# wzf2000/GAMER

Hardware: AMD Instinct MI355X
Metric: train-step sequences/sec, Qwen3Multi SMB decoder, his_len=100 (higher is better)
Workload: dtype f32 tensors/accumulators, products = 3 x fp16 pieces (split3)

## Files before the change

### gamer_amd/_lib.py

```python
from __future__ import annotations

import ctypes as C
import os
import re
from typing import Optional

import torch

_HERE = os.path.dirname(os.path.abspath(__file__))
LIB_PATH = os.path.join(_HERE, "lib", "libgamer_hip.so")
if os.environ.get("GAMER_LIB_PATH"):
    LIB_PATH = os.path.abspath(os.environ["GAMER_LIB_PATH"])
HEADER_PATH = os.path.join(os.path.dirname(_HERE), "include", "gamer_hip.h")

_lib: Optional[C.CDLL] = None

c_void_p, c_int, c_float, c_int64, c_uint64 = C.c_void_p, C.c_int, C.c_float, C.c_int64, C.c_uint64


class GemmDesc(C.Structure):
    _fields_ = [
        ("A", c_void_p), ("a_rs", c_int64), ("a_ks", c_int64),
        ("B", c_void_p), ("b_rs", c_int64), ("b_ks", c_int64),
        ("C", c_void_p), ("ldc", c_int64),
        ("M", c_int), ("N", c_int), ("K", c_int),
        ("alpha", c_float),
        ("accumulate", c_int),
        ("groups", c_int),
        ("group_mode", c_int),
        ("group_offsets", c_void_p),
        ("strideB", c_int64), ("strideC", c_int64),
        ("kchunk", c_int),
        ("resid", c_void_p),
        ("row_map", c_void_p),
        ("p_drop", c_float),
        ("seed", c_uint64),
        ("rowdot_other", c_void_p),
        ("rowdot_out", c_void_p),
        ("rowdot_S", c_int),
        ("qk_wq", c_void_p), ("qk_wk", c_void_p),
        ("qk_eps", c_float),
        ("qk_cos", c_void_p), ("qk_sin", c_void_p),
        ("qk_bias_q", c_void_p), ("qk_bias_k", c_void_p), ("qk_bias_v", c_void_p),
        ("qk_act_idx", c_void_p),
        ("qk_pos_ids", c_void_p),
        ("qk_q_rot", c_void_p), ("qk_k_rot", c_void_p),
        ("qk_S", c_int), ("qk_nq", c_int), ("qk_nkv", c_int),
        ("b_planes", c_void_p), ("b_plane_stride", c_int64),
        ("amax_a", c_void_p), ("amax_b", c_void_p),
        ("amax_c", c_void_p), ("amax_c_col0", c_int),
        ("wgrad_ws", c_void_p), ("wgrad_ws_floats", c_int64),
        ("sw_gu", c_void_p), ("sw_ld", c_int64),
        ("group_div", c_int), ("sw_tbl", c_void_p), ("b_planes_t", c_void_p),
        ("sw_hm", c_void_p), ("sw_row_group", c_void_p),
        ("norm_x", c_void_p), ("norm_w", c_void_p), ("norm_eps", c_float),
        ("norm_dst_rows", c_void_p), ("norm_src_rows", c_void_p),
        ("bias_idx", c_void_p), ("bias_q", c_void_p), ("bias_k", c_void_p), ("bias_v", c_void_p),
        ("bias_rows", c_int), ("bias_nq", c_int), ("bias_nkv", c_int),
    ]


class GemmBf16Desc(C.Structure):
    _fields_ = [
        ("A", c_void_p), ("lda", c_int64),
        ("B", c_void_p), ("ldb", c_int64),
        ("C", c_void_p), ("ldc", c_int64),
        ("M", c_int), ("N", c_int), ("K", c_int),
        ("accumulate", c_int),
        ("groups", c_int),
        ("group_mode", c_int),
        ("group_offsets", c_void_p),
        ("strideB", c_int64), ("strideC", c_int64),
        ("kchunk", c_int),
        ("resid", c_void_p),
        ("row_map", c_void_p),
        ("p_drop", c_float),
        ("seed", c_uint64),
        ("rowdot_other", c_void_p),
        ("rowdot_out", c_void_p),
        ("rowdot_S", c_int),
        ("qk_wq", c_void_p), ("qk_wk", c_void_p), ("qk_eps", c_float),
        ("qk_cos", c_void_p), ("qk_sin", c_void_p),
        ("qk_bias_q", c_void_p), ("qk_bias_k", c_void_p), ("qk_bias_v", c_void_p),
        ("qk_act_idx", c_void_p), ("qk_pos_ids", c_void_p),
        ("qk_q_rot", c_void_p), ("qk_k_rot", c_void_p),
        ("qk_S", c_int), ("qk_nq", c_int), ("qk_nkv", c_int),
        ("sw_gu", c_void_p), ("sw_ld", c_int64),
        ("wgrad_ws", c_void_p), ("wgrad_ws_floats", c_int64),
    ]


P, I, F, L, U = c_void_p, c_int, c_float, c_int64, c_uint64

_SIGNATURES = {
    "gamer_router_fwd": [P, P, P, P, I, I, I, I, I, I, P, P, P, P, P, P, P, P, P, P, P, P],
    "gamer_expert_lists": [P, I, I, I, P, P, P, P, P],
    "gamer_causal_prep": [P, I, I, P, P, P, P, P, P],
    "gamer_session_prep": [P, P, P, I, I, I, I, P, P, P, P, P, P, P],
    "gamer_moe_router_prep": [P, P, P, I, P, I, I, I, I, I, I, I, P, P, P, P, P, P, P, P, P],
    "gamer_moe_action_router_prep": [P, P, P, I, P, I, I, I, I, I, I, I, I, I, P, P, P, P, P, P, P, P, P, P],
    "gamer_session_moe_prep": [P, P, P, P, P, I, P, I, I, I, I, I, I, I, I, P, P, P, P, P, P, P, P, P, P],
    "gamer_embedding_fwd": [P, P, I, I, I, P, P],
    "gamer_embedding_bwd": [P, P, I, I, I, I, P, P],
    "gamer_embedding_bwd_ordered": [P, P, I, I, I, I, P, P, L, P],
    "gamer_embedding_bwd_ordered_ws_bytes": [I, I, I],
    "gamer_rmsnorm_fwd": [P, P, I, I, F, P, P, I, P],
    "gamer_rmsnorm_bwd": [P, P, P, I, P, I, I, F, I, P, P, I, P, P, F, U, P],
    "gamer_colsum_reduce": [P, I, I, I, P, P],
    "gamer_colsum_reduce_batched": [P, L, I, I, I, P, I, P],
    "gamer_rowtable_fwd": [P, P, P, I, I, P, I, I, P],
    "gamer_rowtable_bwd": [P, I, I, P, P, I, I, I, P, P, L, P],
    "gamer_gemm_f32": [C.POINTER(GemmDesc), P],
    "gamer_gemm_f32_split": [C.POINTER(GemmDesc), c_int, P],
    "gamer_split3_guard": [I],
    "gamer_gemm_bf16": [C.POINTER(GemmBf16Desc), P],
    "gamer_cast_params_bf16": [P, P, P, P, I, I, P],
    "gamer_attn_fwd_bf16": [P, I, P, I, P, I, P, P, I, I, I, I, F, F, U, P, P, P, P, P, P, P],
    "gamer_attn_bwd_bf16": [P, I, P, I, P, I, P, P, P, P, P, I, I, I, I, F, F, U, P, P, I, P, I, P, I, P, I, P, P, P, P],
    "gamer_session_spans": [P, P, P, P, P, I, I, I, I, P, P, P, P, P, P, P, P, P],
    "gamer_qknorm_rope_fwd": [P, I, I, I, I, P, P, F, P, P, P, P, P, P, P, P, P, P],
    "gamer_qknorm_rope_bwd": [P, P, P, I, I, I, I, P, P, F, P, P, P, P, P, I, P, P, P, P, P, P, P, P, L, P],
    "gamer_attn_row_order": [P, I, I, P, P, P, P],
    "gamer_attn_fwd": [P, I, P, I, P, I, P, P, P, P, I, I, I, I, F, F, U, P, P, P, P, P, I, P, P],
    "gamer_attn_bwd": [P, I, P, I, P, I, P, P, P, P, P, P, P, I, I, I, I, F, F, U, P, P, I, P, I, P, I, P, P, P, P, P, I, P],
    "gamer_split3_planes": [P, P, L, L, P],
    "gamer_absmax_f32": [P, I, L, I, I, L, P, P],
    "gamer_absmax_multi_f32": [P, P, I, P, P],
    "gamer_split2h_planes_multi": [P, P, I, P, P, P],
    "gamer_amax_sink": [P, P],
    "gamer_amax_sink3": [P, P, P],
    "gamer_attn_split_amax": [P, P, P, P],
    "gamer_attn_fwd_split": [P, I, P, I, P, I, P, P, P, I, I, I, I, F, F, U, P, P, P, P, P, I, P, P],
    "gamer_attn_bwd_split": [P, I, P, I, P, I, P, P, P, P, P, P, P, I, I, I, I, F, F, U, P, P, I, P, I, P, I, P, P, P, I, P, P, P],
    "gamer_residual_dropout_fwd": [P, P, P, I, I, F, U, P, P],
    "gamer_residual_dropout_bwd": [P, P, I, I, F, U, P, P],
    "gamer_swiglu_fwd": [P, P, L, F, U, P, P],
    "gamer_swiglu_bwd": [P, P, P, L, F, U, P],
    "gamer_swiglu_fwd_ld": [P, L, I, I, F, U, P, P],
    "gamer_swiglu_bwd_ld": [P, L, I, I, P, F, U, P],
    "gamer_swiglu_fwd_ld_tbl": [P, L, I, I, F, U, P, P, P, P],
    "gamer_pba_router": [P, I, I, I, I, I, I, I, P, I, I, I, I, I, P, P, P, P, P],
# ... 158 lines not shown
```

### gamer_amd/csrc/common.h

```cpp
#pragma once
#include <hip/hip_runtime.h>
#include <stdint.h>
#include <stdio.h>
#include <stdarg.h>
#include <stdlib.h>
#include <atomic>
#include <type_traits>

#include "../../include/gamer_hip.h"

namespace gamer {

void set_error(const char* fmt, ...);

#define GAMER_CHECK_ARG(cond, ...)                       \
    do {                                                 \
        if (!(cond)) {                                   \
            gamer::set_error(__VA_ARGS__);               \
            return -1;                                   \
        }                                                \
    } while (0)

#define GAMER_CHECK_LAUNCH(name)                                                        \
    do {                                                                                \
// ... 222 lines not shown
    __device__ __forceinline__ float mult(uint64_t idx) const {
        if (!on) return 1.f;
        uint32_t h = mix32((uint32_t)idx ^ k0);
        h = mix32(h + (uint32_t)(idx >> 32) * 0x9e3779b1U + k1);
        return h >= thr ? scale : 0.f;
    }
};

struct AttnDropout {
    uint32_t k0, k1, thr;
    float scale;
    __device__ __forceinline__ AttnDropout(float p, uint64_t seed) {
        k0 = mix32((uint32_t)seed ^ 0x9e3779b9U) ^ mix32((uint32_t)(seed >> 32) + 0x7f4a7c15U);
        k1 = mix32(k0 + 0x632be5abU);
        const float t = p * 4294967296.f;
        thr = t >= 4294967040.f ? 0xffffffffU : (uint32_t)t;
        scale = p > 0.f ? 1.f / (1.f - p) : 1.f;
    }
    __device__ __forceinline__ uint32_t row_word(uint32_t row) const {
        return (mix32(row * 0x9e3779b1U + k0) & 0xffffffU) | 0x800001U;
    }
    __device__ __forceinline__ uint32_t key_word(uint32_t j) const { return mix32(j * 0x85ebca6bU + k1) & 0xffffffU; }
    __device__ __forceinline__ bool keep(uint32_t a, uint32_t b) const { return __umul24(a, b) >= thr; }
};

__device__ __forceinline__ float xor32_max(float v) {
    const auto sw = __builtin_amdgcn_permlane32_swap(__float_as_uint(v), __float_as_uint(v), false, false);
    return fmaxf(__uint_as_float(sw[0]), __uint_as_float(sw[1]));
}
__device__ __forceinline__ float xor32_sum(float v) {
    const auto sw = __builtin_amdgcn_permlane32_swap(__float_as_uint(v), __float_as_uint(v), false, false);
    return __uint_as_float(sw[0]) + __uint_as_float(sw[1]);
}

__device__ __forceinline__ int wave_sum_i32(int v) {
#pragma unroll
    for (int o = 32; o > 0; o >>= 1) v += __shfl_xor(v, o, 64);
    return v;
}
__device__ __forceinline__ int wave_max_i32(int v) {
#pragma unroll
    for (int o = 32; o > 0; o >>= 1) v = max(v, __shfl_xor(v, o, 64));
    return v;
}
__device__ __forceinline__ int wave_min_i32(int v) {
#pragma unroll
    for (int o = 32; o > 0; o >>= 1) v = min(v, __shfl_xor(v, o, 64));
    return v;
}

#define GAMER_DPP_ROW_REDUCE(OP, v)                                                                   \
    v = OP(v, __builtin_amdgcn_update_dpp(v, v, 0xB1, 0xf, 0xf, false));      \
    v = OP(v, __builtin_amdgcn_update_dpp(v, v, 0x4E, 0xf, 0xf, false));      \
    v = OP(v, __builtin_amdgcn_update_dpp(v, v, 0x141, 0xf, 0xf, false));         \
    v = OP(v, __builtin_amdgcn_update_dpp(v, v, 0x140, 0xf, 0xf, false));
__device__ __forceinline__ int wave_min_i32_dpp(int v) {
    GAMER_DPP_ROW_REDUCE(min, v)
    return min(min(__builtin_amdgcn_readlane(v, 0), __builtin_amdgcn_readlane(v, 16)),
               min(__builtin_amdgcn_readlane(v, 32), __builtin_amdgcn_readlane(v, 48)));
}
__device__ __forceinline__ int wave_max_i32_dpp(int v) {
    GAMER_DPP_ROW_REDUCE(max, v)
    return max(max(__builtin_amdgcn_readlane(v, 0), __builtin_amdgcn_readlane(v, 16)),
               max(__builtin_amdgcn_readlane(v, 32), __builtin_amdgcn_readlane(v, 48)));
}

__device__ __forceinline__ float row16_sum_dpp(float v) {
#define GAMER_DPP_F(ctrl) __int_as_float(__builtin_amdgcn_update_dpp(__float_as_int(v), __float_as_int(v), ctrl, 0xf, 0xf, false))
    v += GAMER_DPP_F(0xB1);
    v += GAMER_DPP_F(0x4E);
    v += GAMER_DPP_F(0x141);
    v += GAMER_DPP_F(0x140);
#undef GAMER_DPP_F
    return v;
}

__device__ __forceinline__ float sigmoid_f(float x) { return __builtin_amdgcn_rcpf(1.f + __expf(-x)); }
__device__ __forceinline__ float silu_f(float x) { return x * sigmoid_f(x); }
__device__ __forceinline__ float dsilu_f(float x) {
    const float s = sigmoid_f(x);
    return s * (1.f + x * (1.f - s));
}

struct SwigluRule {
    static constexpr int NIN = 2;
    static __device__ __forceinline__ float fwd(float a, float b, float m) { return m * (silu_f(a) * b); }
    static __device__ __forceinline__ float bwd_a(float a, float b, float d) { return d * b * dsilu_f(a); }
    static __device__ __forceinline__ float bwd_b(float a, float, float d) { return d * silu_f(a); }
};
struct SiluRule {
    static constexpr int NIN = 1;
    static __device__ __forceinline__ float fwd(float a, float, float m) { return m * silu_f(a); }
    static __device__ __forceinline__ float bwd_a(float a, float, float d) { return d * dsilu_f(a); }
};
struct ReluRule {
    static constexpr int NIN = 1;
    static __device__ __forceinline__ float fwd(float a, float, float m) { return a > 0.f ? m * a : 0.f; }
    static __device__ __forceinline__ float bwd_a(float a, float, float d) { return a > 0.f ? d : 0.f; }
};
template <class R>
__device__ __forceinline__ float4 act_fwd4(const float4 a, const float4 b, const float (&m)[4]) {
    return make_float4(R::fwd(a.x, b.x, m[0]), R::fwd(a.y, b.y, m[1]), R::fwd(a.z, b.z, m[2]), R::fwd(a.w, b.w, m[3]));
}
template <class R>
__device__ __forceinline__ void act_bwd4(const float4 a, const float4 b, const float4 dout, const float (&m)[4], float4& da, float4& db) {
    const float d0 = m[0] * dout.x, d1 = m[1] * dout.y, d2 = m[2] * dout.z, d3 = m[3] * dout.w;
    da = make_float4(R::bwd_a(a.x, b.x, d0), R::bwd_a(a.y, b.y, d1), R::bwd_a(a.z, b.z, d2), R::bwd_a(a.w, b.w, d3));
    if constexpr (R::NIN == 2) db = make_float4(R::bwd_b(a.x, b.x, d0), R::bwd_b(a.y, b.y, d1), R::bwd_b(a.z, b.z, d2), R::bwd_b(a.w, b.w, d3));
}

bool gemm_as_eligible(const gamer_gemm_desc* d, bool a_kc, bool b_kc, const uint16_t* b_planes);
int launch_gemm_as(const gamer_gemm_desc* d, const uint16_t* b_planes, bool b_kc, hipStream_t st);
int launch_gemm_bias_rows(const gamer_gemm_desc* d, hipStream_t st);
bool gemm_os_eligible(const gamer_gemm_desc* d, bool a_kc, bool b_kc, const uint16_t* b_planes);
int launch_gemm_os(const gamer_gemm_desc* d, const uint16_t* b_planes, int guard, hipStream_t st, bool fwd_t = false);
bool gemm_os_fwd_eligible(const gamer_gemm_desc* d, bool a_kc, bool b_kc);
bool gemm_wg_eligible(const gamer_gemm_desc* d, bool a_kc, bool b_kc);
int launch_gemm_wg(const gamer_gemm_desc* d, hipStream_t st);

int launch_wgrad_reduce(const float* ws, float* C, int64_t ldc, int M, int N, int groups, const int32_t* group_offsets, int K,
                        int kchunk, int64_t strideC, hipStream_t st);

}
```

### gamer_amd/csrc/elementwise.hip

```cpp
#include "common.h"

namespace gamer {

__global__ void __launch_bounds__(EW_THREADS)
embedding_fwd_kernel(const int64_t* __restrict__ ids, const float4* __restrict__ W, int V, int T, int H4,
                     float4* __restrict__ x) {
    const int lane = threadIdx.x & 63;
    const int wave = (blockIdx.x * EW_THREADS + threadIdx.x) >> 6;
    const int nwaves = (gridDim.x * EW_THREADS) >> 6;
    for (int t = wave; t < T; t += nwaves) {
        const int64_t id = ids[t];
        const bool ok = id >= 0 && id < V;
        for (int c = lane; c < H4; c += 64) {
            float4 v = ok ? W[id * H4 + c] : make_float4(0.f, 0.f, 0.f, 0.f);
            x[(int64_t)t * H4 + c] = v;
        }
    }
}

constexpr int EMB_CACHE = 8;
constexpr int EMB_CHUNK = 1024;
__global__ void __launch_bounds__(EW_THREADS)
embedding_bwd_kernel(const int64_t* __restrict__ ids, const float* __restrict__ dx, int V, int T, int H,
                     int pad_id, float* __restrict__ dW, const int chunk) {
// ... 436 lines not shown
    for (int a = 0; a < TBL_MAXROWS; ++a) acc[a] = make_float4(0.f, 0.f, 0.f, 0.f);
    if (rl < rows_per_block) {
        for (int64_t t = (int64_t)blockIdx.x * rows_per_block + rl; t < T; t += (int64_t)gridDim.x * rows_per_block) {
            const int64_t r = dy_rows ? dy_rows[t] : t;
            const float4 g = ld4(dy + r * lddy + col0 + 4 * c);
            const int a_t = idx[t];
#pragma unroll
            for (int a = 0; a < TBL_MAXROWS; ++a) {
                const float m = (a_t == a) ? 1.f : 0.f;
                acc[a].x += m * g.x; acc[a].y += m * g.y; acc[a].z += m * g.z; acc[a].w += m * g.w;
            }
        }
#pragma unroll
        for (int a = 0; a < TBL_MAXROWS; ++a) {
            if (a < nrows) {
                if (DET) {
                    *reinterpret_cast<float4*>(&lds_tbl[(rl * nrows + a) * E + c * 4]) = acc[a];
                } else {
                    atomicAdd(&lds_tbl[a * E + c * 4 + 0], acc[a].x);
                    atomicAdd(&lds_tbl[a * E + c * 4 + 1], acc[a].y);
                    atomicAdd(&lds_tbl[a * E + c * 4 + 2], acc[a].z);
                    atomicAdd(&lds_tbl[a * E + c * 4 + 3], acc[a].w);
                }
            }
        }
    }
    __syncthreads();
    if (DET) {
        for (int i = threadIdx.x; i < nrows * E; i += EW_THREADS) {
            float t = 0.f;
            for (int g = 0; g < rows_per_block; ++g) t += lds_tbl[g * nrows * E + i];
            partial[(int64_t)blockIdx.x * nrows * E + i] = t;
        }
    } else {
        for (int i = threadIdx.x; i < nrows * E; i += EW_THREADS) atomicAdd(&dtable[i], lds_tbl[i]);
    }
}

__global__ void __launch_bounds__(EW_THREADS)
residual_dropout_fwd_kernel(const float4* x_in, const float4* __restrict__ delta,
                            const int32_t* __restrict__ src_rows, int T, int H4, float p, uint64_t seed,
                            float4* x_out) {
    const DropoutRng rng(p, seed);
    const int64_t total = (int64_t)T * H4;
    for (int64_t i = (int64_t)blockIdx.x * EW_THREADS + threadIdx.x; i < total; i += (int64_t)gridDim.x * EW_THREADS) {
        const int t = (int)(i / H4);
        const int c = (int)(i % H4);
        const int64_t r = src_rows ? src_rows[t] : t;
        const float4 d = delta[r * H4 + c];
        float4 v = x_in[i];
        float m[4];
        rng.mult4((uint32_t)i, m);
        v.x += m[0] * d.x; v.y += m[1] * d.y; v.z += m[2] * d.z; v.w += m[3] * d.w;
        x_out[i] = v;
    }
}

__global__ void __launch_bounds__(EW_THREADS)
residual_dropout_bwd_kernel(const float4* __restrict__ dx, const int32_t* __restrict__ src_rows, int T, int H4,
                            float p, uint64_t seed, float4* __restrict__ ddelta) {
    const DropoutRng rng(p, seed);
    const int64_t total = (int64_t)T * H4;
    for (int64_t i = (int64_t)blockIdx.x * EW_THREADS + threadIdx.x; i < total; i += (int64_t)gridDim.x * EW_THREADS) {
        const int t = (int)(i / H4);
        const int c = (int)(i % H4);
        const int64_t r = src_rows ? src_rows[t] : t;
        const float4 g = dx[i];
        float m[4];
        rng.mult4((uint32_t)i, m);
        float4 o;
        o.x = m[0] * g.x; o.y = m[1] * g.y; o.z = m[2] * g.z; o.w = m[3] * g.w;
        ddelta[r * H4 + c] = o;
    }
}

template <typename TA, typename TO>
__global__ void __launch_bounds__(EW_THREADS)
silu_gate_fwd_kernel(const TA* __restrict__ a, const TA* __restrict__ gate, int64_t n4,
                     TO* __restrict__ out, const float4* __restrict__ resid, float p, uint64_t seed) {
    const DropoutRng rng(resid ? p : 0.f, seed);
    for (int64_t i = (int64_t)blockIdx.x * EW_THREADS + threadIdx.x; i < n4; i += (int64_t)gridDim.x * EW_THREADS) {
        const float4 x = ld4(a + 4 * i), g = ld4(gate + 4 * i);
        float4 o;
        o.x = x.x * silu_f(g.x); o.y = x.y * silu_f(g.y); o.z = x.z * silu_f(g.z); o.w = x.w * silu_f(g.w);
        if (resid) {
            const float4 r = resid[i];
            float m[4];
            rng.mult4((uint32_t)i, m);
            o.x = r.x + m[0] * o.x; o.y = r.y + m[1] * o.y; o.z = r.z + m[2] * o.z; o.w = r.w + m[3] * o.w;
        }
        st4(out + 4 * i, o);
    }
}

template <typename TA>
__global__ void __launch_bounds__(EW_THREADS)
silu_gate_bwd_kernel(const TA* __restrict__ a, const TA* __restrict__ gate, const float4* __restrict__ dout,
                     int64_t n4, TA* __restrict__ da, TA* __restrict__ dgate, float p, uint64_t seed,
                     uint32_t* __restrict__ amax_a, uint32_t* __restrict__ amax_gate) {
    __shared__ uint32_t amax_lds[2][4];
    uint32_t ama = 0, amg = 0;
    const DropoutRng rng(p, seed);
    for (int64_t i = (int64_t)blockIdx.x * EW_THREADS + threadIdx.x; i < n4; i += (int64_t)gridDim.x * EW_THREADS) {
        const float4 x = ld4(a + 4 * i), g = ld4(gate + 4 * i);
        float4 d = dout[i];
        float m[4];
        rng.mult4((uint32_t)i, m);
        d.x *= m[0]; d.y *= m[1]; d.z *= m[2]; d.w *= m[3];
        float4 oa, og;
        oa.x = d.x * silu_f(g.x); og.x = d.x * x.x * dsilu_f(g.x);
        oa.y = d.y * silu_f(g.y); og.y = d.y * x.y * dsilu_f(g.y);
        oa.z = d.z * silu_f(g.z); og.z = d.z * x.z * dsilu_f(g.z);
        oa.w = d.w * silu_f(g.w); og.w = d.w * x.w * dsilu_f(g.w);
        st4(da + 4 * i, oa);
        st4(dgate + 4 * i, og);
        ama = amax_f4(ama, oa);
        amg = amax_f4(amg, og);
    }
    amax_block_commit(ama, amax_a, amax_lds[0]);
    amax_block_commit(amg, amax_gate, amax_lds[1]);
}

constexpr int CE_MAXC = 20;
template <typename T> constexpr int CE_EPL = 16 / (int)sizeof(T);
template <typename T> constexpr int CE_MAXQ = sizeof(T) == 2 ? 3 : 5;
__device__ __forceinline__ void ce_load16(const float* p, float (&x)[4]) {
    const float4 v = *reinterpret_cast<const float4*>(p);
    x[0] = v.x; x[1] = v.y; x[2] = v.z; x[3] = v.w;
}
__device__ __forceinline__ void ce_store16(float* p, const float (&x)[4]) { *reinterpret_cast<float4*>(p) = make_float4(x[0], x[1], x[2], x[3]); }
__device__ __forceinline__ void ce_load16(const bf16_t* p, float (&x)[8]) {
    const bf16x8 v = *reinterpret_cast<const bf16x8*>(p);
#pragma unroll
    for (int e = 0; e < 8; ++e) x[e] = (float)v[e];
}
__device__ __forceinline__ void ce_store16(bf16_t* p, const float (&x)[8]) {
    bf16x8 v;
#pragma unroll
    for (int e = 0; e < 8; ++e) v[e] = (bf16_t)x[e];
    *reinterpret_cast<bf16x8*>(p) = v;
}
template <typename TL>
__global__ void __launch_bounds__(EW_THREADS)
ce_fwd_kernel(TL* __restrict__ logits, int ldl, const int64_t* __restrict__ labels, int T, int S, int V,
              float inv_temp, int ignore_index, float* __restrict__ lse_out, float* __restrict__ row_loss, int vec4) {
    const int lane = threadIdx.x & 63;
    const int wave = (blockIdx.x * EW_THREADS + threadIdx.x) >> 6;
    const int nwaves = (gridDim.x * EW_THREADS) >> 6;
    for (int t = wave; t < T; t += nwaves) {
        TL* row = logits + (int64_t)t * ldl;
        const int s = t % S;
        const int64_t tgt = (s + 1 < S) ? labels[t + 1] : (int64_t)ignore_index;
        const bool valid = tgt != ignore_index && tgt >= 0 && tgt < V;
        float mx = -INFINITY;
        float zt = 0.f;
        if (vec4 && V <= 64 * CE_EPL<TL> * CE_MAXQ<TL>) {
            constexpr int EPL = CE_EPL<TL>;
            float z[CE_MAXQ<TL>][EPL];
            const int c_last = ((V - 1) / EPL) * EPL;
#pragma unroll
            for (int i = 0; i < CE_MAXQ<TL>; ++i) {
                const int c = EPL * (lane + 64 * i);
                float x[EPL];
                ce_load16(row + min(c, c_last), x);
#pragma unroll
                for (int e = 0; e < EPL; ++e) z[i][e] = c + e < V ? round_as<TL>(x[e] * inv_temp) : -INFINITY;
            }
#pragma unroll
            for (int i = 0; i < CE_MAXQ<TL>; ++i) {
                const int c = EPL * (lane + 64 * i);
                if (inv_temp == 1.f) {
                } else if (c + EPL <= V) {
// ... 551 lines not shown
```

### gamer_amd/csrc/gemm.hip

```cpp
#include "common.h"
#include <stdlib.h>

namespace gamer {

constexpr int BM = 128, BN = 128, BK = 32;
constexpr int GEMM_THREADS = 256;
constexpr int KC_LD = BK + 4;
constexpr int TILE_FLOATS = BM * KC_LD;
constexpr int GEMM_LDS_BYTES = 4 * TILE_FLOATS * (int)sizeof(float);

typedef float f32x16 __attribute__((ext_vector_type(16)));

constexpr int SP_KC_ROW = 80;
constexpr int SP_KC_IMG = BM * SP_KC_ROW;
constexpr int SP_RC_IMG = BK * 256;
constexpr int SP_OPERAND = 3 * SP_KC_IMG;
constexpr int SP_LDS_BYTES = 2 * SP_OPERAND;

#ifndef SP_ABLATE
#define SP_ABLATE 0
#endif
__device__ __forceinline__ uint32_t pack_hi16(uint32_t w0, uint32_t w1) { return __builtin_amdgcn_perm(w1, w0, 0x07060302u); }
__device__ __forceinline__ void split3(float x, uint32_t (&w)[3]) {
    if (SP_ABLATE & 1) { w[0] = w[1] = w[2] = __float_as_uint(x); return; }
    w[0] = __float_as_uint(x);
    const float r1 = x - __uint_as_float(w[0] & 0xffff0000u);
    w[1] = __float_as_uint(r1);
    const float r2 = r1 - __uint_as_float(w[1] & 0xffff0000u);
    w[2] = __float_as_uint(r2);
}
__device__ __forceinline__ void split3_quad(const float4& v, uint2 (&img)[3]) {
    uint32_t a[3], b[3], c[3], d[3];
    split3(v.x, a); split3(v.y, b); split3(v.z, c); split3(v.w, d);
#pragma unroll
    for (int s = 0; s < 3; ++s) img[s] = make_uint2(pack_hi16(a[s], b[s]), pack_hi16(c[s], d[s]));
}
__device__ __forceinline__ int sp_rc_off(int k, int row) { return k * 256 + ((((row >> 3) ^ ((k & 3) << 2))) << 4) + ((row & 7) << 1); }
__device__ __forceinline__ void store_kc_split(unsigned char* __restrict__ lds, int tid, const float4 (&r)[4]) {
#pragma unroll
    for (int j = 0; j < 4; ++j) {
        const int f = tid + GEMM_THREADS * j;
        uint2 img[3];
        split3_quad(r[j], img);
        unsigned char* dst = lds + (f >> 3) * SP_KC_ROW + ((f & 7) << 3);
        if (SP_ABLATE & 2) { asm volatile("" :: "v"(img[0].x), "v"(img[1].x), "v"(img[2].x), "v"(img[0].y), "v"(img[1].y), "v"(img[2].y)); continue; }
#pragma unroll
        for (int s = 0; s < 3; ++s) *reinterpret_cast<uint2*>(dst + s * SP_KC_IMG) = img[s];
    }
}
__device__ __forceinline__ void store_rc_split(unsigned char* __restrict__ lds, int tid, const float4 (&r)[4]) {
#pragma unroll
    for (int j = 0; j < 4; ++j) {
        const int f = tid + GEMM_THREADS * j;
        uint2 img[3];
        split3_quad(r[j], img);
        unsigned char* dst = lds + sp_rc_off(f >> 5, (f & 31) << 2);
        if (SP_ABLATE & 2) { asm volatile("" :: "v"(img[0].x), "v"(img[1].x), "v"(img[2].x), "v"(img[0].y), "v"(img[1].y), "v"(img[2].y)); continue; }
#pragma unroll
        for (int s = 0; s < 3; ++s) *reinterpret_cast<uint2*>(dst + s * SP_RC_IMG) = img[s];
    }
}
__device__ __forceinline__ void split2h_quad(const float4& v, float s, uint2 (&img)[2]) {
    uint32_t a0, a1, b0, b1;
    cut2h_quad(v.x, v.y, v.z, v.w, s, a0, a1, b0, b1);
    img[0] = make_uint2(a0, b0);
    img[1] = make_uint2(a1, b1);
}
__device__ __forceinline__ void store_kc_h2(unsigned char* __restrict__ lds, int tid, const float4 (&r)[4], float s) {
#pragma unroll
    for (int j = 0; j < 4; ++j) {
        const int f = tid + GEMM_THREADS * j;
        uint2 img[2];
        split2h_quad(r[j], s, img);
        unsigned char* dst = lds + (f >> 3) * SP_KC_ROW + ((f & 7) << 3);
#pragma unroll
        for (int q = 0; q < 2; ++q) *reinterpret_cast<uint2*>(dst + q * SP_KC_IMG) = img[q];
    }
}
__device__ __forceinline__ void store_rc_h2(unsigned char* __restrict__ lds, int tid, const float4 (&r)[4], float s) {
#pragma unroll
    for (int j = 0; j < 4; ++j) {
        const int f = tid + GEMM_THREADS * j;
        uint2 img[2];
        split2h_quad(r[j], s, img);
// ... 45 lines not shown
__device__ __forceinline__ bf16x8 read_frag_half(const unsigned char* __restrict__ img, int rbase, int lane) {
    const int r32 = lane & 31, h = lane >> 5;
    if (KC) {
        return *reinterpret_cast<const bf16x8*>(img + (rbase + r32) * SPH_KC_ROW + (h << 4));
    } else {
        const int q = (lane >> 2) & 3, pp = lane & 3, gsel = (lane >> 4) & 1;
        const int row = rbase + 16 * gsel + 4 * pp;
        bf16x8 out;
#pragma unroll
        for (int c = 0; c < 2; ++c) {
            const int k = 8 * h + 4 * c + q;
            const bf16x4 v = __builtin_amdgcn_ds_read_tr16_b64_v4bf16(
                (bf16x4 __attribute__((address_space(3)))*)(img + sp_rc_off(k, row)));
            out[4 * c + 0] = v[0]; out[4 * c + 1] = v[1]; out[4 * c + 2] = v[2]; out[4 * c + 3] = v[3];
        }
        return out;
    }
}

template <bool KC>
__device__ __forceinline__ bf16x8 read_frag_split(const unsigned char* __restrict__ img, int rbase, int sub, int lane) {
    const int r32 = lane & 31, h = lane >> 5;
    if (KC) {
        return *reinterpret_cast<const bf16x8*>(img + (rbase + r32) * SP_KC_ROW + ((2 * sub + h) << 4));
    } else {
        const int q = (lane >> 2) & 3, pp = lane & 3, gsel = (lane >> 4) & 1;
        const int row = rbase + 16 * gsel + 4 * pp;
        bf16x8 out;
#pragma unroll
        for (int c = 0; c < 2; ++c) {
            const int k = 16 * sub + 8 * h + 4 * c + q;
            const bf16x4 v = __builtin_amdgcn_ds_read_tr16_b64_v4bf16(
                (bf16x4 __attribute__((address_space(3)))*)(img + sp_rc_off(k, row)));
            out[4 * c + 0] = v[0]; out[4 * c + 1] = v[1]; out[4 * c + 2] = v[2]; out[4 * c + 3] = v[3];
        }
        return out;
    }
}

__device__ unsigned long long* g_gemm_stamp = nullptr;
__device__ __forceinline__ unsigned long long stamp_now() {
    unsigned long long t;
    asm volatile("s_memtime %0\n\ts_waitcnt lgkmcnt(0)" : "=s"(t) :: "memory");
    return t;
}

struct GemmParams {
    const float* A; int64_t a_rs, a_ks;
    const float* B; int64_t b_rs, b_ks;
    float* C; int64_t ldc;
    int M, N, K;
    float alpha;
    int accumulate;
    int groups;
    const int32_t* group_offsets;
    int64_t strideB, strideC;
    int kchunk;
    int m_tiles, n_tiles;
    const float* resid;
    const int32_t* row_map;
    float p_drop;
    uint64_t seed;
    const float* rowdot_other;
    float* rowdot_out;
    int rowdot_S;
    const float* qk_wq; const float* qk_wk;
    float qk_eps;
    const float* qk_cos; const float* qk_sin;
    const float* qk_bias_q; const float* qk_bias_k; const float* qk_bias_v;
    const int32_t* qk_act_idx;
    const int32_t* qk_pos_ids;
    float* qk_q_rot; float* qk_k_rot;
    int qk_S, qk_nq, qk_nkv;
    const uint32_t* amax_a; const uint32_t* amax_b;
    const uint16_t* b_planes;
    int64_t b_plane_stride;
    int guard;
    uint32_t* amax_c;
    int amax_c_col0;
    float* wgrad_ws;
    float* sw_gu; int64_t sw_ld;
    int group_div;
    const float* sw_tbl;
};

constexpr float SPLIT3_GUARD_RATIO = 1.f / 65536.f;
#ifndef GAMER_GEMM_CAMAX_BUILD
#define GAMER_GEMM_CAMAX_BUILD 1
#endif
#ifndef GAMER_SPLIT3_GUARD_BUILD
#define GAMER_SPLIT3_GUARD_BUILD 1
#endif
static int g_split3_guard = 1;

__device__ __forceinline__ int xcd_remap(int id, int n) {
    const int q = n >> 3, r = n & 7;
    const int xcd = id & 7, idx = id >> 3;
    const int base = xcd < r ? xcd * (q + 1) : r * (q + 1) + (xcd - r) * q;
    return base + idx;
}

template <bool INTERIOR>
__device__ __forceinline__ void load_kc(const float* __restrict__ p, int64_t rs, int row0, int row_end, int k0,
                                        int k_end, int tid, float4 (&r)[4]) {
#pragma unroll
    for (int j = 0; j < 4; ++j) {
        const int f = tid + GEMM_THREADS * j;
        const int row = row0 + (f >> 3);
        const int k = k0 + ((f & 7) << 2);
        if (INTERIOR) {
            r[j] = *reinterpret_cast<const float4*>(p + (int64_t)row * rs + k);
            continue;
        }
        float4 v = make_float4(0.f, 0.f, 0.f, 0.f);
        if (row < row_end && k < k_end) {
            v = *reinterpret_cast<const float4*>(p + (int64_t)row * rs + k);
            if (k + 3 >= k_end) {
                if (k + 1 >= k_end) v.y = 0.f;
                if (k + 2 >= k_end) v.z = 0.f;
                v.w = 0.f;
            }
        }
        r[j] = v;
    }
}
template <bool INTERIOR>
__device__ __forceinline__ void load_rc(const float* __restrict__ p, int64_t ks, int row0, int row_end, int k0,
                                        int k_end, int tid, float4 (&r)[4]) {
#pragma unroll
    for (int j = 0; j < 4; ++j) {
        const int f = tid + GEMM_THREADS * j;
        const int k = k0 + (f >> 5);
        const int row = row0 + ((f & 31) << 2);
        if (INTERIOR) {
            r[j] = *reinterpret_cast<const float4*>(p + (int64_t)k * ks + row);
            continue;
        }
        float4 v = make_float4(0.f, 0.f, 0.f, 0.f);
        if (k < k_end && row < row_end) {
            v = *reinterpret_cast<const float4*>(p + (int64_t)k * ks + row);
            if (row + 3 >= row_end) {
                if (row + 1 >= row_end) v.y = 0.f;
                if (row + 2 >= row_end) v.z = 0.f;
                v.w = 0.f;
            }
        }
        r[j] = v;
    }
}
__device__ __forceinline__ void store_kc(float* __restrict__ lds, int tid, const float4 (&r)[4]) {
#pragma unroll
    for (int j = 0; j < 4; ++j) {
        const int f = tid + GEMM_THREADS * j;
        *reinterpret_cast<float4*>(lds + (f >> 3) * KC_LD + ((f & 7) << 2)) = r[j];
    }
}
__device__ __forceinline__ void store_rc(float* __restrict__ lds, int tid, const float4 (&r)[4]) {
#pragma unroll
    for (int j = 0; j < 4; ++j) {
        const int f = tid + GEMM_THREADS * j;
        *reinterpret_cast<float4*>(lds + (f >> 5) * BM + ((f & 31) << 2)) = r[j];
    }
}

template <bool KC>
__device__ __forceinline__ void read_frag(const float* __restrict__ lds, int row, int kk, int h, float (&f)[4]) {
// ... 510 lines not shown
        }
    }
    if (PP && grp == 0) __syncthreads();
    const unsigned long long t_loop_end = STAMP ? stamp_now() : 0;

    bool redo = false;
    if (GUARD && p.guard) {
        const float thr = __uint_as_float(amax_a_bits) * SPLIT3_GUARD_RATIO;
        bool bad = false;
#pragma unroll
        for (int j = 0; j < 4; ++j) {
            float m = rmax[j];
            m = fmaxf(m, __shfl_xor(m, 1, 64)); m = fmaxf(m, __shfl_xor(m, 2, 64)); m = fmaxf(m, __shfl_xor(m, 4, 64));
            bad |= (m > 0.f) & !(m >= thr);
        }
        int* flags = reinterpret_cast<int*>(smem + 4 * 64 * 68);
        const bool wave_bad = __any(bad ? 1 : 0) != 0;
        if (lane == 0) flags[wid] = wave_bad ? 1 : 0;
        __syncthreads();
        redo = (flags[0] | flags[1] | flags[2] | flags[3]) != 0;
        if (redo) {
#pragma unroll
            for (int i = 0; i < 2; ++i)
#pragma unroll
                for (int j = 0; j < 2; ++j)
#pragma unroll
                    for (int r = 0; r < 16; ++r) acc[i][j][r] = 0.f;
            if (wave_live) {
                const int ar0 = row0 + wm * 64 + r32, bc0 = col0 + wn * 64 + r32;
#pragma unroll 1
                for (int k = kbeg; k < kend; k += 2) {
                    const int kk = k + h;
                    const bool kin = kk < kend;
                    float av[2], bv[2];
#pragma unroll
                    for (int i = 0; i < 2; ++i) {
                        const int row = ar0 + i * 32;
                        av[i] = (kin && row < row_end) ? p.A[(int64_t)row * p.a_rs + kk] : 0.f;
                    }
#pragma unroll
                    for (int j = 0; j < 2; ++j) {
                        const int col = bc0 + j * 32;
                        bv[j] = (kin && col < col_end) ? (B_KC ? Bsrc[(int64_t)col * p.b_rs + kk] : Bsrc[(int64_t)kk * p.b_ks + col]) : 0.f;
                    }
#pragma unroll
                    for (int i = 0; i < 2; ++i)
#pragma unroll
                        for (int j = 0; j < 2; ++j)
                            acc[i][j] = __builtin_amdgcn_mfma_f32_32x32x2f32(av[i], bv[j], acc[i][j], 0, 0, 0);
                }
            }
        }
    }

    const bool interior = a_in && b_in;
    const float alpha_eff = (SPLIT == 3 && !redo) ? p.alpha * unscale : p.alpha;
    if (MODE == 0 && (NBUF == 2 || SPLIT) && interior && (p.ldc & 3) == 0) {
        float* patch = smem + wid * (64 * 68);
        float4 oth[EPI == 2 ? 16 : 1];
        if (EPI == 2) {
            const float* ob = p.rowdot_other + (int64_t)(row0 + wm * 64 + (lane >> 4)) * p.ldc + col0 + wn * 64 + ((lane & 15) << 2);
#pragma unroll
            for (int it = 0; it < 16; ++it) oth[it] = *reinterpret_cast<const float4*>(ob + (int64_t)it * 4 * p.ldc);
        }
        if (SPLIT != 3 && p.alpha == 1.f) {
#pragma unroll
            for (int i = 0; i < 2; ++i)
#pragma unroll
                for (int j = 0; j < 2; ++j)
#pragma unroll
                    for (int r = 0; r < 16; ++r)
                        patch[(i * 32 + (r & 3) + 8 * (r >> 2) + 4 * h) * 68 + j * 32 + r32] = acc[i][j][r];
        } else {
#pragma unroll
            for (int i = 0; i < 2; ++i)
#pragma unroll
                for (int j = 0; j < 2; ++j)
#pragma unroll
                    for (int r = 0; r < 16; ++r)
                        patch[(i * 32 + (r & 3) + 8 * (r >> 2) + 4 * h) * 68 + j * 32 + r32] = alpha_eff * acc[i][j][r];
        }
        __builtin_amdgcn_s_waitcnt(0xc07f);
        const int c4 = (lane & 15) << 2;
        const DropoutRng rng((EPI == 1 || EPI == 4) ? p.p_drop : 0.f, p.seed);
        const int row_first = row0 + wm * 64 + (lane >> 4);
        const int col = col0 + wn * 64 + c4;
        float* dst0 = Cp + (int64_t)row_first * p.ldc + col;
        const int64_t step = 4 * p.ldc;
        const int qk_pos0 = EPI == 3 ? row_first % max(p.qk_S, 1) : 0;
        const bool amax_on = GAMER_GEMM_CAMAX_BUILD && p.amax_c != nullptr && !ACCUM && col0 + wn * 64 >= p.amax_c_col0;
        float cmax = 0.f;
        int pre_rc[EPI == 1 ? 16 : 1];
        float4 pre_x[EPI == 1 ? 16 : (EPI == 4 ? 8 : 1)], pre_b[EPI == 4 ? 8 : 1];
        if (EPI == 1) {
            if (p.row_map) {
#pragma unroll
                for (int it = 0; it < 16; ++it) pre_rc[it] = p.row_map[row_first + 4 * it];
            } else {
#pragma unroll
                for (int it = 0; it < 16; ++it) pre_rc[it] = row_first + 4 * it;
            }
#pragma unroll
            for (int it = 0; it < 16; ++it) pre_x[it] = *reinterpret_cast<const float4*>(p.resid + (int64_t)pre_rc[it] * p.ldc + col);
        }
        float4 tb_g = make_float4(0.f, 0.f, 0.f, 0.f), tb_u = tb_g;
        if (EPI == 4 && p.sw_tbl) {
            const float* tb = p.sw_tbl + (int64_t)tile_group * 2 * p.N + col;
            tb_g = *reinterpret_cast<const float4*>(tb);
            tb_u = *reinterpret_cast<const float4*>(tb + p.N);
        }
        auto pre_sw = [&](int it0) {
#pragma unroll
            for (int it = 0; it < 8; ++it) {
                const float* ga = p.sw_gu + (int64_t)(row_first + 4 * (it0 + it)) * p.sw_ld + col;
                pre_x[EPI == 4 ? it : 0] = *reinterpret_cast<const float4*>(ga);
                pre_b[EPI == 4 ? it : 0] = *reinterpret_cast<const float4*>(ga + p.N);
            }
        };
        if (EPI == 4) pre_sw(0);
#pragma unroll
        for (int it = 0; it < 16; ++it) {
            if (EPI == 4 && it == 8) pre_sw(8);
            const int lr = (lane >> 4) + 4 * it;
            const float4 v = *reinterpret_cast<const float4*>(patch + lr * 68 + c4);
            if (EPI == 3) {
                const int row = row_first + 4 * it;
                const int hd = (col0 + wn * 64) >> 6;
                const int g = lane & 15;
                float4 x = v;
                const bool cross = p.qk_bias_q != nullptr;
                const int a = cross ? p.qk_act_idx[row] : 0;
                if (hd < p.qk_nq + p.qk_nkv) {
                    const bool isq = hd < p.qk_nq;
                    if (cross) {
                        const float4 b4 = isq ? reinterpret_cast<const float4*>(p.qk_bias_q + (int64_t)a * p.qk_nq * 64 + hd * 64)[g]
                                              : reinterpret_cast<const float4*>(p.qk_bias_k + (int64_t)a * p.qk_nkv * 64 + (hd - p.qk_nq) * 64)[g];
                        x.x += b4.x; x.y += b4.y; x.z += b4.z; x.w += b4.w;
                    }
                    *reinterpret_cast<float4*>(dst0 + it * step) = x;
                    float ss = x.x * x.x + x.y * x.y + x.z * x.z + x.w * x.w;
                    ss = row16_sum_dpp(ss);
                    const float rstd = rsqrtf(ss * (1.f / 64.f) + p.qk_eps);
                    const float4 w4 = reinterpret_cast<const float4*>(isq ? p.qk_wq : p.qk_wk)[g];
                    float4 y;
                    y.x = w4.x * (x.x * rstd); y.y = w4.y * (x.y * rstd); y.z = w4.z * (x.z * rstd); y.w = w4.w * (x.w * rstd);
                    float4 pr;
                    pr.x = __shfl_xor(y.x, 8, 64); pr.y = __shfl_xor(y.y, 8, 64); pr.z = __shfl_xor(y.z, 8, 64); pr.w = __shfl_xor(y.w, 8, 64);
                    int pos = qk_pos0 + 4 * it;
                    if (p.qk_S >= 64) pos = pos >= p.qk_S ? pos - p.qk_S : pos;
                    else pos %= p.qk_S;
                    if (p.qk_pos_ids) pos = p.qk_pos_ids[row];
                    const float4 cc = reinterpret_cast<const float4*>(p.qk_cos + pos * 64)[g];
                    const float4 sn = reinterpret_cast<const float4*>(p.qk_sin + pos * 64)[g];
                    const float sgn = g < 8 ? -1.f : 1.f;
                    float4 o;
                    o.x = y.x * cc.x + sgn * pr.x * sn.x; o.y = y.y * cc.y + sgn * pr.y * sn.y;
                    o.z = y.z * cc.z + sgn * pr.z * sn.z; o.w = y.w * cc.w + sgn * pr.w * sn.w;
                    float* rot = isq ? p.qk_q_rot + (int64_t)row * p.qk_nq * 64 + hd * 64
                                     : p.qk_k_rot + (int64_t)row * p.qk_nkv * 64 + (hd - p.qk_nq) * 64;
                    *reinterpret_cast<float4*>(rot + 4 * g) = o;
                } else {
                    if (cross) {
                        const float4 b4 = reinterpret_cast<const float4*>(p.qk_bias_v + (int64_t)a * p.qk_nkv * 64 +
                                                                          (hd - p.qk_nq - p.qk_nkv) * 64)[g];
                        x.x += b4.x; x.y += b4.y; x.z += b4.z; x.w += b4.w;
                    }
                    *reinterpret_cast<float4*>(dst0 + it * step) = x;
                }
            } else if (EPI == 4) {
                const int row = row_first + 4 * it;
                float* ga = p.sw_gu + (int64_t)row * p.sw_ld + col;
                float* ua = ga + p.N;
                float4 a = pre_x[EPI == 4 ? (it & 7) : 0], b = pre_b[EPI == 4 ? (it & 7) : 0];
                a.x += tb_g.x; a.y += tb_g.y; a.z += tb_g.z; a.w += tb_g.w;
                b.x += tb_u.x; b.y += tb_u.y; b.z += tb_u.z; b.w += tb_u.w;
                float m[4];
                rng.mult4((uint32_t)(((int64_t)row * p.N + col) >> 2), m);
                const float d0 = m[0] * v.x, d1 = m[1] * v.y, d2 = m[2] * v.z, d3 = m[3] * v.w;
                float4 dg, du;
                dg.x = SwigluRule::bwd_a(a.x, b.x, d0); du.x = SwigluRule::bwd_b(a.x, b.x, d0);
                dg.y = SwigluRule::bwd_a(a.y, b.y, d1); du.y = SwigluRule::bwd_b(a.y, b.y, d1);
                dg.z = SwigluRule::bwd_a(a.z, b.z, d2); du.z = SwigluRule::bwd_b(a.z, b.z, d2);
                dg.w = SwigluRule::bwd_a(a.w, b.w, d3); du.w = SwigluRule::bwd_b(a.w, b.w, d3);
                *reinterpret_cast<float4*>(ga) = dg;
                *reinterpret_cast<float4*>(ua) = du;
                if (amax_on) {
                    asm("v_max3_f32 %0, %0, |%1|, |%2|\n\tv_max3_f32 %0, %0, |%3|, |%4|" : "+v"(cmax) : "v"(dg.x), "v"(dg.y), "v"(dg.z), "v"(dg.w));
                    asm("v_max3_f32 %0, %0, |%1|, |%2|\n\tv_max3_f32 %0, %0, |%3|, |%4|" : "+v"(cmax) : "v"(du.x), "v"(du.y), "v"(du.z), "v"(du.w));
                }
            } else if (EPI == 1) {
                const int64_t e = (int64_t)pre_rc[EPI == 1 ? it : 0] * p.ldc + col;
                float* dst = Cp + e;
                const float4 x = pre_x[EPI == 1 ? it : 0];
                float m[4];
                rng.mult4((uint32_t)(e >> 2), m);
                float4 o;
                o.x = x.x + m[0] * v.x; o.y = x.y + m[1] * v.y; o.z = x.z + m[2] * v.z; o.w = x.w + m[3] * v.w;
                *reinterpret_cast<float4*>(dst) = o;
            } else {
                float* dst = dst0 + it * step;
                if (EPI != 1 && EPI != 3 && amax_on)
                    asm("v_max3_f32 %0, %0, |%1|, |%2|\n\tv_max3_f32 %0, %0, |%3|, |%4|" : "+v"(cmax) : "v"(v.x), "v"(v.y), "v"(v.z), "v"(v.w));
                if (EPI == 2) {
                    const float4 o4 = oth[EPI == 2 ? it : 0];
                    float d = v.x * o4.x + v.y * o4.y + v.z * o4.z + v.w * o4.w;
                    d = row16_sum_dpp(d);
                    if ((lane & 15) == 0) {
                        const int row = row_first + 4 * it;
                        const int heads = p.N >> 6, head = (col0 + wn * 64) >> 6;
                        p.rowdot_out[((int64_t)(row / p.rowdot_S) * heads + head) * p.rowdot_S + row % p.rowdot_S] = d;
                    }
                }
                if (ACCUM) {
                    float4 o = *reinterpret_cast<const float4*>(dst);
                    o.x += v.x; o.y += v.y; o.z += v.z; o.w += v.w;
                    *reinterpret_cast<float4*>(dst) = o;
                } else {
                    *reinterpret_cast<float4*>(dst) = v;
                }
            }
        }
        if (EPI != 1 && EPI != 3 && amax_on) {
            uint32_t mw = __float_as_uint(cmax);
#pragma unroll
            for (int o2 = 32; o2 > 0; o2 >>= 1) mw = max(mw, (uint32_t)__shfl_xor((int)mw, o2, 64));
            if (lane == 0 && mw) amax_publish(mw, p.amax_c, (uint32_t)(vblock * 4 + wid));
        }
    } else if (MODE == 1 && p.wgrad_ws != nullptr) {
        float* blk = p.wgrad_ws + ws_block * (int64_t)(BM * BN);
#pragma unroll
        for (int i = 0; i < 2; ++i)
#pragma unroll
            for (int j = 0; j < 2; ++j) {
                const int lc = wn * 64 + j * 32 + r32;
                const int lr0 = wm * 64 + i * 32 + 4 * h;
#pragma unroll
                for (int r = 0; r < 16; ++r) blk[(lr0 + (r & 3) + 8 * (r >> 2)) * BN + lc] = alpha_eff * acc[i][j][r];
            }
    } else {
        float emax = 0.f;
        if (EPI == 4 && p.sw_tbl != nullptr) {
            const float* tb0 = p.sw_tbl + (int64_t)tile_group * 2 * p.N;
            const int nr = min(BM, row_end - row0), nc = min(BN, p.N - col0);
            for (int i = threadIdx.x; i < nr * nc; i += GEMM_THREADS) {
                const int rr = row0 + i / nc, cc = col0 + i % nc;
                float* ga = p.sw_gu + (int64_t)rr * p.sw_ld + cc;
                ga[0] += tb0[cc];
                ga[p.N] += tb0[p.N + cc];
            }
            __syncthreads();
        }
        auto emit = [&](int row, int col, float v) {
            if (EPI == 4) {
                float* ga = p.sw_gu + (int64_t)row * p.sw_ld + col;
                float a = ga[0], b = ga[p.N];
                const int64_t e = (int64_t)row * p.N + col;
                const DropoutRng rng(p.p_drop, p.seed);
                float m[4];
                rng.mult4((uint32_t)(e >> 2), m);
                const float d = m[e & 3] * v;
                const float dg = SwigluRule::bwd_a(a, b, d), du = SwigluRule::bwd_b(a, b, d);
                ga[0] = dg; ga[p.N] = du;
                if (GAMER_GEMM_CAMAX_BUILD && p.amax_c != nullptr) emax = fmaxf(emax, fmaxf(fabsf(dg), fabsf(du)));
                return;
            }
            if (GAMER_GEMM_CAMAX_BUILD && EPI != 1 && MODE == 0 && !ACCUM && p.amax_c != nullptr && col >= p.amax_c_col0) emax = fmaxf(emax, fabsf(v));
            if (EPI == 1) {
                const int64_t rc = p.row_map ? p.row_map[row] : row;
                const int64_t e = rc * p.ldc + col;
                const DropoutRng rng(p.p_drop, p.seed);
                float m[4];
                rng.mult4((uint32_t)(e >> 2), m);
                Cp[e] = p.resid[e] + m[e & 3] * v;
            } else {
                float* dst = Cp + (int64_t)row * p.ldc + col;
                if (MODE == 1) atomicAdd(dst, v);
                else if (ACCUM) *dst += v;
                else *dst = v;
            }
        };
#pragma unroll
        for (int i = 0; i < 2; ++i) {
#pragma unroll
            for (int j = 0; j < 2; ++j) {
                const int col = col0 + wn * 64 + j * 32 + r32;
                const int rbase = row0 + wm * 64 + i * 32 + 4 * h;
                if (interior) {
#pragma unroll
                    for (int r = 0; r < 16; ++r) emit(rbase + (r & 3) + 8 * (r >> 2), col, alpha_eff * acc[i][j][r]);
                } else {
#pragma unroll
                    for (int r = 0; r < 16; ++r) {
                        const int rr = (r & 3) + 8 * (r >> 2);
                        if (rbase + rr < row_end && col < col_end) emit(rbase + rr, col, alpha_eff * acc[i][j][r]);
                    }
                }
            }
        }
        if (GAMER_GEMM_CAMAX_BUILD && MODE == 0 && !ACCUM && p.amax_c != nullptr) {
            uint32_t mw = __float_as_uint(emax);
#pragma unroll
            for (int o2 = 32; o2 > 0; o2 >>= 1) mw = max(mw, (uint32_t)__shfl_xor((int)mw, o2, 64));
            if (lane == 0 && mw) amax_publish(mw, p.amax_c, (uint32_t)(vblock * 4 + wid));
        }
    }
    if (STAMP) {
        unsigned long long* st = g_gemm_stamp;
        if (st && threadIdx.x == 0) {
            const unsigned long long t_end = stamp_now();
            unsigned long long* rec = st + 8ull * vblock;
            rec[0] = t_ph[0]; rec[1] = t_ph[1]; rec[2] = t_ph[2]; rec[3] = t_ph[3];
            rec[4] = t_loop_end - t_begin;
            rec[5] = t_end - t_loop_end;
            rec[6] = t_begin;
            rec[7] = t_end;
        }
    }
}

template <bool A_KC, bool B_KC, int MODE, bool ACCUM, bool STAMP, int NBUF, int EPI, int SPLIT = 0, bool PP = false>
__global__ void __launch_bounds__(PP ? 2 * GEMM_THREADS : GEMM_THREADS, (NBUF == 1 && SPLIT == 0) ? 3 : 2)
gemm_f32_kernel(const GemmParams p, const int vgrid) {
    extern __shared__ __attribute__((aligned(16))) float smem_all[];
    for (int v = blockIdx.x; v < vgrid; v += gridDim.x) {
        gemm_f32_tile<A_KC, B_KC, MODE, ACCUM, STAMP, NBUF, EPI, SPLIT, PP>(p, smem_all, v, vgrid);
        if (v + (int)gridDim.x < vgrid) __syncthreads();
    }
}

template <bool A_KC, bool B_KC, int MODE, bool ACCUM, bool STAMP, int NBUF, int EPI = 0, int SPLIT = 0, bool PP = false>
static int launch_gemm_t(const GemmParams& p, int blocks, hipStream_t st, int lds) {
    static int persist = -1;
    if (persist < 0) { const char* e = getenv("GAMER_GEMM_PERSIST"); persist = e ? atoi(e) : 0; }
    const int grid = (persist > 0 && SPLIT != 0 && !PP && !STAMP && blocks > persist) ? persist : blocks;
    return launch<gemm_f32_kernel<A_KC, B_KC, MODE, ACCUM, STAMP, NBUF, EPI, SPLIT, PP>>("gamer_gemm_f32", dim3(grid), dim3(PP ? 2 * GEMM_THREADS : GEMM_THREADS),
                                                                                        lds, st, p, blocks);
}

template <bool A_KC, bool B_KC, int MODE, int SPLIT>
static int launch_gemm_split(const GemmParams& p, int blocks, hipStream_t st) {
    constexpr int h2_stage = 2 * ((A_KC ? SP_KC_IMG : SP_RC_IMG) + (B_KC ? SP_KC_IMG : SP_RC_IMG));
    const int lds = (SPLIT == 3 && SP_WIDE3 && A_KC && B_KC && 2 * h2_stage > GEMM_LDS_BYTES) ? 2 * h2_stage : GEMM_LDS_BYTES;
    static_assert(SP_LDS_BYTES <= GEMM_LDS_BYTES, "split images must fit the fp32 kernel's LDS allocation");
    const bool acc = MODE == 0 && p.accumulate;
    static int stamp = -1, pp = 0;
    if (stamp < 0) {
        const char* e = getenv("GAMER_GEMM_STAMP");
        stamp = (e && e[0] == '1') ? 1 : 0;
        const char* e2 = getenv("GAMER_GEMM_PP");
        pp = (SP_PINGPONG && e2 && e2[0] == '1') ? 1 : 0;
    }
    (void)pp;
#if SP_PINGPONG
    if ((SPLIT == 6 || SPLIT == 3) && pp && !(MODE == 0 && p.b_planes)) {
        int pblocks;
        if (MODE == 0) pblocks = (blocks + 1) / 2;
        else {
            const int tiles_mn = p.m_tiles * p.n_tiles;
            pblocks = blocks / tiles_mn * ((tiles_mn + 1) / 2);
        }
        const int plds = 2 * GEMM_LDS_BYTES;
        if (stamp) return launch_gemm_t<A_KC, B_KC, MODE, false, true, 2, 0, SPLIT, true>(p, pblocks, st, plds);
        if (MODE == 0 && p.resid) return launch_gemm_t<A_KC, B_KC, MODE, false, false, 2, 1, SPLIT, true>(p, pblocks, st, plds);
        if (MODE == 0 && p.rowdot_out) return launch_gemm_t<A_KC, B_KC, MODE, false, false, 2, 2, SPLIT, true>(p, pblocks, st, plds);
        if (MODE == 0 && A_KC && B_KC && p.qk_q_rot) return launch_gemm_t<A_KC, B_KC, MODE, false, false, 2, 3, SPLIT, true>(p, pblocks, st, plds);
        if (acc) return launch_gemm_t<A_KC, B_KC, MODE, true, false, 2, 0, SPLIT, true>(p, pblocks, st, plds);
        return launch_gemm_t<A_KC, B_KC, MODE, false, false, 2, 0, SPLIT, true>(p, pblocks, st, plds);
    }
#endif
    if (stamp && SPLIT == 6) return launch_gemm_t<A_KC, B_KC, MODE, false, true, 2, 0, SPLIT>(p, blocks, st, lds);
    if constexpr (SPLIT == 3 && MODE == 0 && A_KC) {
        if (p.sw_gu) return launch_gemm_t<A_KC, B_KC, MODE, false, false, 2, 4, SPLIT>(p, blocks, st, lds);
    }
    if (MODE == 0 && p.resid) return launch_gemm_t<A_KC, B_KC, MODE, false, false, 2, 1, SPLIT>(p, blocks, st, lds);
    if (MODE == 0 && p.rowdot_out) return launch_gemm_t<A_KC, B_KC, MODE, false, false, 2, 2, SPLIT>(p, blocks, st, lds);
    if (MODE == 0 && A_KC && B_KC && p.qk_q_rot) return launch_gemm_t<A_KC, B_KC, MODE, false, false, 2, 3, SPLIT>(p, blocks, st, lds);
    if (acc) return launch_gemm_t<A_KC, B_KC, MODE, true, false, 2, 0, SPLIT>(p, blocks, st, lds);
    return launch_gemm_t<A_KC, B_KC, MODE, false, false, 2, 0, SPLIT>(p, blocks, st, lds);
}

template <bool A_KC, bool B_KC, int MODE>
static int launch_gemm(const GemmParams& p, int blocks, hipStream_t st, int split = 0) {
    if (split == 6) return launch_gemm_split<A_KC, B_KC, MODE, 6>(p, blocks, st);
    if (split == 9) return launch_gemm_split<A_KC, B_KC, MODE, 9>(p, blocks, st);
    if (split == 3) return launch_gemm_split<A_KC, B_KC, MODE, 3>(p, blocks, st);
    static int stamp = -1, solo = 0, nbuf = 2;
    if (stamp < 0) {
        const char* e = getenv("GAMER_GEMM_STAMP");
        stamp = (e && e[0] == '1') ? 1 : 0;
        const char* s2 = getenv("GAMER_GEMM_SOLO");
        solo = (s2 && s2[0] == '1') ? 1 : 0;
        const char* s3 = getenv("GAMER_GEMM_NBUF");
        nbuf = (s3 && s3[0] == '1') ? 1 : 2;
    }
    const int lds = solo ? 150 * 1024 : GEMM_LDS_BYTES;
    const bool acc = MODE == 0 && p.accumulate;
    if (stamp) return launch_gemm_t<A_KC, B_KC, MODE, false, true, 2>(p, blocks, st, lds);
    if (MODE == 0 && p.resid) return launch_gemm_t<A_KC, B_KC, MODE, false, false, 2, 1>(p, blocks, st, lds);
    if (MODE == 0 && p.rowdot_out) return launch_gemm_t<A_KC, B_KC, MODE, false, false, 2, 2>(p, blocks, st, lds);
    if (MODE == 0 && A_KC && B_KC && p.qk_q_rot) return launch_gemm_t<A_KC, B_KC, MODE, false, false, 2, 3>(p, blocks, st, lds);
    if (nbuf == 1) {
        const int lds1 = 2 * TILE_FLOATS * (int)sizeof(float);
        if (acc) return launch_gemm_t<A_KC, B_KC, MODE, true, false, 1>(p, blocks, st, lds1);
        return launch_gemm_t<A_KC, B_KC, MODE, false, false, 1>(p, blocks, st, lds1);
    }
    if (acc) return launch_gemm_t<A_KC, B_KC, MODE, true, false, 2>(p, blocks, st, lds);
    return launch_gemm_t<A_KC, B_KC, MODE, false, false, 2>(p, blocks, st, lds);
}

__global__ void __launch_bounds__(256)
wgrad_reduce_kernel(const float* __restrict__ ws, float* __restrict__ C, int64_t ldc, int M, int N, int m_tiles, int n_tiles,
                    int groups, const int32_t* __restrict__ group_offsets, int K, int kchunk, int64_t strideC) {
    const int tiles_mn = m_tiles * n_tiles;
    int id = blockIdx.x;
    const int strip = id & 15; id >>= 4;
    const int tile = id % tiles_mn, g = id / tiles_mn;
    int c_beg = 0, c_n;
    if (group_offsets) {
        int prev = group_offsets[0];
        c_n = 0;
        for (int gi = 0; gi <= g; ++gi) {
            const int nxt = group_offsets[gi + 1];
            const int chunks = (nxt - prev + kchunk - 1) / kchunk;
            if (gi < g) c_beg += chunks; else c_n = chunks;
            prev = nxt;
        }
    } else {
        c_n = (K + kchunk - 1) / kchunk;
    }
    const int lr = strip * 8 + (threadIdx.x >> 5), lc = (threadIdx.x & 31) << 2;
    const float4* src = reinterpret_cast<const float4*>(ws + ((int64_t)c_beg * tiles_mn + tile) * (int64_t)(BM * BN) + lr * BN + lc);
    const int64_t step4 = (int64_t)tiles_mn * (BM * BN) / 4;
    float4 s = make_float4(0.f, 0.f, 0.f, 0.f);
    int c = 0;
    for (; c + 4 <= c_n; c += 4) {
        const float4 a0 = src[(int64_t)c * step4], a1 = src[(int64_t)(c + 1) * step4], a2 = src[(int64_t)(c + 2) * step4],
                     a3 = src[(int64_t)(c + 3) * step4];
        s.x = (((s.x + a0.x) + a1.x) + a2.x) + a3.x; s.y = (((s.y + a0.y) + a1.y) + a2.y) + a3.y;
        s.z = (((s.z + a0.z) + a1.z) + a2.z) + a3.z; s.w = (((s.w + a0.w) + a1.w) + a2.w) + a3.w;
    }
    for (; c < c_n; ++c) {
        const float4 a0 = src[(int64_t)c * step4];
        s.x += a0.x; s.y += a0.y; s.z += a0.z; s.w += a0.w;
    }
    const int row = (tile / n_tiles) * BM + lr, col = (tile % n_tiles) * BN + lc;
    if (row < M && c_n > 0) {
        float* dst = C + (int64_t)g * strideC + (int64_t)row * ldc + col;
        const float v[4] = {s.x, s.y, s.z, s.w};
#pragma unroll
        for (int e = 0; e < 4; ++e)
            if (col + e < N) dst[e] += v[e];
    }
}

int launch_wgrad_reduce(const float* ws, float* C, int64_t ldc, int M, int N, int groups, const int32_t* group_offsets, int K,
                        int kchunk, int64_t strideC, hipStream_t st) {
    const int m_tiles = (M + BM - 1) / BM, n_tiles = (N + BN - 1) / BN;
    const int64_t rblocks = (int64_t)groups * m_tiles * n_tiles * 16;
    hipLaunchKernelGGL(wgrad_reduce_kernel, dim3((int)rblocks), dim3(256), 0, st, ws, C, ldc, M, N, m_tiles, n_tiles, groups,
                       group_offsets, K, kchunk, strideC);
    return (int)hipGetLastError();
}

__global__ void __launch_bounds__(256)
split3_planes_kernel(const float4* __restrict__ x, uint16_t* __restrict__ planes, int64_t n4, int64_t stride) {
    for (int64_t i = (int64_t)blockIdx.x * 256 + threadIdx.x; i < n4; i += (int64_t)gridDim.x * 256) {
        uint2 img[3];
        split3_quad(x[i], img);
#pragma unroll
        for (int s = 0; s < 3; ++s) *reinterpret_cast<uint2*>(planes + s * stride + 4 * i) = img[s];
    }
}

}

using namespace gamer;

extern "C" int gamer_split3_planes(const float* x, gamer_bf16* planes, int64_t n, int64_t plane_stride, void* stream) {
    GAMER_CHECK_ARG(x && planes && n > 0 && n % 4 == 0 && plane_stride >= n && plane_stride % 4 == 0 && aligned16(x) &&
                    (reinterpret_cast<uintptr_t>(planes) & 7u) == 0,
                    "gamer_split3_planes: n=%lld and plane_stride=%lld must be multiples of 4 (stride >= n), x 16-byte and planes 8-byte aligned",
                    (long long)n, (long long)plane_stride);
    const int64_t n4 = n / 4;
    int blocks = (int)((n4 + 255) / 256);
    if (blocks > 4096) blocks = 4096;
    hipLaunchKernelGGL(split3_planes_kernel, dim3(blocks), dim3(256), 0, (hipStream_t)stream, reinterpret_cast<const float4*>(x),
                       reinterpret_cast<uint16_t*>(planes), n4, plane_stride);
    GAMER_CHECK_LAUNCH("gamer_split3_planes");
    return 0;
}

extern "C" int gamer_debug_gemm_stamp(void* p) {
    unsigned long long* v = (unsigned long long*)p;
    return (int)hipMemcpyToSymbol(HIP_SYMBOL(g_gemm_stamp), &v, sizeof(v));
}

static inline bool diag_build_switches() {
    static EnvSwitch stamp("GAMER_GEMM_STAMP"), nbuf("GAMER_GEMM_NBUF");
    return stamp.is_set() || nbuf.is_set();
}
static inline bool diag_pp_switch() { static EnvSwitch pp("GAMER_GEMM_PP"); return pp.is_set(); }
static int gemm_entry(const gamer_gemm_desc* d, void* stream, int split) {
    GAMER_CHECK_ARG(d, "gamer_gemm_f32: null descriptor");
    GAMER_CHECK_ARG(d->A && d->B && d->C, "gamer_gemm_f32: null matrix pointer");
    GAMER_CHECK_ARG(d->M > 0 && d->N > 0 && d->K > 0, "gamer_gemm_f32: bad shape M=%d N=%d K=%d", d->M, d->N, d->K);
    GAMER_CHECK_ARG((d->a_rs == 1) != (d->a_ks == 1) || (d->a_rs == 1 && d->a_ks == 1 && (d->M == 1 || d->K == 1)),
                    "gamer_gemm_f32: exactly one of a_rs/a_ks must be 1 (rs=%lld ks=%lld)", (long long)d->a_rs, (long long)d->a_ks);
    GAMER_CHECK_ARG((d->b_rs == 1) != (d->b_ks == 1) || (d->b_rs == 1 && d->b_ks == 1 && (d->N == 1 || d->K == 1)),
                    "gamer_gemm_f32: exactly one of b_rs/b_ks must be 1 (rs=%lld ks=%lld)", (long long)d->b_rs, (long long)d->b_ks);
    const bool a_kc = d->a_ks == 1, b_kc = d->b_ks == 1;
    const int64_t a_ld = a_kc ? d->a_rs : d->a_ks, b_ld = b_kc ? d->b_rs : d->b_ks;
    GAMER_CHECK_ARG(a_ld % 4 == 0 && b_ld % 4 == 0 && d->ldc >= d->N,
                    "gamer_gemm_f32: leading dims must be multiples of 4 (lda=%lld ldb=%lld ldc=%lld)",
                    (long long)a_ld, (long long)b_ld, (long long)d->ldc);
    GAMER_CHECK_ARG(aligned16(d->A) && aligned16(d->B), "gamer_gemm_f32: A and B must be 16-byte aligned");
    GAMER_CHECK_ARG(d->groups >= 1 && (d->groups == 1 || d->group_offsets), "gamer_gemm_f32: groups=%d needs group_offsets", d->groups);
    GAMER_CHECK_ARG(d->strideB % 4 == 0, "gamer_gemm_f32: strideB must be a multiple of 4");
    GAMER_CHECK_ARG(d->group_mode == 0 || d->group_mode == 1, "gamer_gemm_f32: group_mode=%d", d->group_mode);

    GemmParams p;
    p.A = d->A; p.a_rs = d->a_rs; p.a_ks = d->a_ks;
    p.B = d->B; p.b_rs = d->b_rs; p.b_ks = d->b_ks;
    p.C = d->C; p.ldc = d->ldc;
    p.M = d->M; p.N = d->N; p.K = d->K;
    p.alpha = d->alpha; p.accumulate = d->accumulate;
    p.groups = d->groups; p.group_offsets = d->group_offsets;
    p.strideB = d->strideB; p.strideC = d->strideC;
    p.kchunk = d->kchunk;
    p.resid = d->resid; p.row_map = d->row_map; p.p_drop = d->p_drop; p.seed = d->seed;
    p.rowdot_other = d->rowdot_other; p.rowdot_out = d->rowdot_out; p.rowdot_S = d->rowdot_S;
    p.qk_wq = d->qk_wq; p.qk_wk = d->qk_wk; p.qk_eps = d->qk_eps; p.qk_cos = d->qk_cos; p.qk_sin = d->qk_sin;
    p.qk_bias_q = d->qk_bias_q; p.qk_bias_k = d->qk_bias_k; p.qk_bias_v = d->qk_bias_v;
    p.qk_act_idx = d->qk_act_idx; p.qk_pos_ids = d->qk_pos_ids; p.qk_q_rot = d->qk_q_rot; p.qk_k_rot = d->qk_k_rot;
    p.qk_S = d->qk_S; p.qk_nq = d->qk_nq; p.qk_nkv = d->qk_nkv;
    p.amax_a = d->amax_a; p.amax_b = d->amax_b;
    p.guard = g_split3_guard;
    p.amax_c = d->amax_c; p.amax_c_col0 = d->amax_c_col0;
    p.wgrad_ws = nullptr;
    p.sw_gu = d->sw_gu; p.sw_ld = d->sw_ld;
    p.group_div = d->group_div > 1 ? d->group_div : 1; p.sw_tbl = d->sw_tbl;
    GAMER_CHECK_ARG(d->group_div <= 1 || (d->group_mode == 0 && d->group_offsets && d->groups % d->group_div == 0),
                    "gamer_gemm_f32: group_div = %d needs group_mode 0, group_offsets and groups (%d) a multiple of it", d->group_div, d->groups);
    GAMER_CHECK_ARG(!d->sw_tbl || ((d->sw_gu || d->sw_hm) && aligned16(d->sw_tbl)),
                    "gamer_gemm_f32: sw_tbl is an option of the SwiGLU epilogues (sw_gu, sw_hm)");
    GAMER_CHECK_ARG(!d->sw_gu || (split == 3 && d->group_mode == 0 && !d->accumulate && !d->resid && !d->rowdot_out && !d->qk_q_rot &&
                                  d->alpha == 1.f && d->N % 4 == 0 && d->sw_ld >= 2 * (int64_t)d->N && d->sw_ld % 4 == 0 &&
                                  aligned16(d->sw_gu) && d->p_drop >= 0.f && d->p_drop < 1.f),
                    "gamer_gemm_f32: the SwiGLU-backward epilogue (sw_gu) is built for gamer_gemm_f32_split(terms = 3), a plain input-"
                    "gradient GEMM with alpha = 1, N %% 4 == 0, sw_ld >= 2 N (N=%d sw_ld=%lld)", d->N, (long long)d->sw_ld);
    GAMER_CHECK_ARG(!d->amax_c || (d->group_mode == 0 && !d->accumulate && !d->resid && !d->qk_q_rot && d->amax_c_col0 >= 0 &&
                                   d->amax_c_col0 % 64 == 0),
                    "gamer_gemm_f32: amax_c needs a plain or row-dot Linear-forward / input-gradient GEMM (no accumulate, residual or "
                    "q|k|v epilogue) and amax_c_col0 a multiple of 64 (amax_c_col0=%d)", d->amax_c_col0);
    GAMER_CHECK_ARG(split != 3 || (d->amax_a && d->amax_b), "gamer_gemm_f32_split: terms = 3 needs amax_a and amax_b (gamer_absmax_f32)");
    p.b_planes = (split && d->group_mode == 0) ? (const uint16_t*)d->b_planes : nullptr;
    p.b_plane_stride = d->b_plane_stride;
    GAMER_CHECK_ARG(!p.b_planes || split == 3 || ((reinterpret_cast<uintptr_t>(p.b_planes) & 7u) == 0 && d->b_plane_stride % 4 == 0 && d->b_plane_stride > 0),
                    "gamer_gemm_f32_split: b_planes must be 8-byte aligned with b_plane_stride %% 4 == 0");
    GAMER_CHECK_ARG(!p.b_planes || split != 3 || (reinterpret_cast<uintptr_t>(p.b_planes) & 15u) == 0,
                    "gamer_gemm_f32_split: terms = 3 takes b_planes as packed pieces at B's offsets (16-byte aligned)");
    if (split == 3 && p.b_planes && ((b_kc ? d->K : d->N) % 4) != 0) p.b_planes = nullptr;
    GAMER_CHECK_ARG(!d->qk_q_rot || (d->qk_k_rot && d->qk_wq && d->qk_wk && d->qk_cos && d->qk_sin && d->group_mode == 0 &&
                                     d->groups == 1 && a_kc && b_kc && !d->resid && !d->rowdot_out && !d->accumulate &&
                                     d->alpha == 1.f && d->M % BM == 0 && d->qk_nq > 0 && d->qk_nkv > 0 && d->qk_S > 0 &&
                                     d->N == (d->qk_nq + 2 * d->qk_nkv) * 64 && d->N % BN == 0 && d->ldc % 4 == 0 &&
                                     aligned16(d->C) && aligned16(d->qk_q_rot) && aligned16(d->qk_k_rot) &&
                                     (!d->qk_bias_q || (d->qk_bias_k && d->qk_bias_v && d->qk_act_idx)) &&
                                     !diag_build_switches()),
                    "gamer_gemm_f32: the q|k|v epilogue needs a Linear-forward layout, one group, M %% 128 == 0 (M=%d), "
                    "N = (nq + 2 nkv) * 64 a multiple of 128 (N=%d), alpha = 1 and no other epilogue", d->M, d->N);
    GAMER_CHECK_ARG(!d->rowdot_out || (d->rowdot_other && d->rowdot_S > 0 && d->group_mode == 0 && d->groups == 1 &&
                                       !d->resid && !d->accumulate && d->M % BM == 0 && d->N % BN == 0 &&
                                       d->M % d->rowdot_S == 0 && d->ldc % 4 == 0 && aligned16(d->rowdot_other) &&
                                       aligned16(d->C) && !diag_build_switches()),
                    "gamer_gemm_f32: the row-dot epilogue needs full 128 x 128 tiles (M=%d N=%d), one group, ldc %% 4 == 0",
                    d->M, d->N);
    GAMER_CHECK_ARG(!d->resid || (d->group_mode == 0 && !d->accumulate && a_kc && b_kc && d->ldc % 4 == 0 &&
                                  aligned16(d->resid) && aligned16(d->C) && d->p_drop >= 0.f && d->p_drop < 1.f),
                    "gamer_gemm_f32: the fused residual epilogue needs a Linear-forward layout, ldc %% 4 == 0, no accumulate");
    GAMER_CHECK_ARG(!d->sw_hm || (d->group_mode == 0 && a_kc && b_kc && !d->accumulate && !d->resid && !d->rowdot_out && !d->qk_q_rot &&
                                  !d->sw_gu && d->alpha == 1.f && d->N % 8 == 0 && d->ldc >= d->N && d->ldc % 4 == 0 && aligned16(d->sw_hm) &&
                                  aligned16(d->C) && (!d->sw_tbl || d->sw_row_group) && d->p_drop >= 0.f && d->p_drop < 1.f),
                    "gamer_gemm_f32: the SwiGLU-forward epilogue (sw_hm) needs a Linear-forward layout with N = 2 I (N=%d), alpha = 1, no other "
                    "epilogue, and sw_row_group with sw_tbl", d->N);
    GAMER_CHECK_ARG(!d->norm_x || (d->norm_w && d->group_mode == 0 && a_kc && b_kc && d->norm_eps > 0.f && d->K % 4 == 0 && d->K <= 1024 &&
                                   aligned16(d->norm_x) && aligned16(d->norm_w) &&
                                   (d->norm_dst_rows != nullptr) == (d->norm_src_rows != nullptr)),
                    "gamer_gemm_f32: the RMSNorm prologue (norm_x) needs a Linear-forward layout, norm_w, norm_eps > 0, K %% 4 == 0 (K=%d) "
                    "and norm_dst_rows / norm_src_rows both or neither", d->K);
    GAMER_CHECK_ARG(!d->bias_idx || (d->bias_q && d->bias_k && d->bias_v && d->group_mode == 0 && d->groups == 1 && a_kc && b_kc &&
                                     !d->accumulate && !d->resid && !d->rowdot_out && !d->qk_q_rot && !d->sw_gu && !d->sw_hm &&
                                     d->bias_rows >= 1 && d->bias_nq > 0 && d->bias_nkv > 0 && d->bias_nq % 4 == 0 && d->bias_nkv % 4 == 0 &&
                                     d->N == d->bias_nq + 2 * d->bias_nkv && d->ldc % 4 == 0 && aligned16(d->C) && aligned16(d->bias_q) &&
                                     aligned16(d->bias_k) && aligned16(d->bias_v)),
                    "gamer_gemm_f32: the bias-row epilogue (bias_idx) needs a plain Linear-forward GEMM with one group, three tables and "
                    "N = bias_nq + 2 bias_nkv in multiples of 4 (N=%d)", d->N);
    if (split == 3 && gemm_as_eligible(d, a_kc, b_kc, p.b_planes)) return launch_gemm_as(d, p.b_planes, b_kc, (hipStream_t)stream);
    if (d->norm_x || d->bias_idx) {
        gamer_gemm_desc d2 = *d;
        if (d->norm_x) {
            if (d->amax_a) gamer_amax_sink(const_cast<uint32_t*>(d->amax_a), nullptr);
            GAMER_TRY(gamer_rmsnorm_fwd(d->norm_x, d->norm_w, d->M, d->K, d->norm_eps, d->norm_dst_rows, const_cast<float*>(d->A), (int)d->a_rs,
                                        stream));
            d2.norm_x = nullptr; d2.norm_w = nullptr; d2.norm_dst_rows = nullptr; d2.norm_src_rows = nullptr;
        }
        if (d->bias_idx) { d2.bias_idx = nullptr; d2.amax_c = nullptr; }
        GAMER_TRY(gemm_entry(&d2, stream, split));
        return d->bias_idx ? launch_gemm_bias_rows(d, (hipStream_t)stream) : 0;
    }
    if (d->sw_hm) {
        gamer_gemm_desc d2 = *d;
        d2.sw_hm = nullptr; d2.sw_row_group = nullptr; d2.sw_tbl = nullptr; d2.amax_c = nullptr;
        const int rc = gemm_entry(&d2, stream, split);
        if (rc) return rc;
        if (d->amax_c) gamer_amax_sink(d->amax_c, nullptr);
        return d->sw_tbl ? gamer_swiglu_fwd_ld_tbl(d->C, d->ldc, d->M, d->N / 2, d->p_drop, d->seed, d->sw_hm, d->sw_tbl, d->sw_row_group, stream)
                         : gamer_swiglu_fwd_ld(d->C, d->ldc, d->M, d->N / 2, d->p_drop, d->seed, d->sw_hm, stream);
    }
    if (split == 3 && gemm_os_eligible(d, a_kc, b_kc, p.b_planes)) return launch_gemm_os(d, p.b_planes, g_split3_guard, (hipStream_t)stream);
    if (split == 3 && gemm_os_fwd_eligible(d, a_kc, b_kc))
        return launch_gemm_os(d, reinterpret_cast<const uint16_t*>(d->b_planes_t), g_split3_guard, (hipStream_t)stream, true);
    p.n_tiles = (d->N + BN - 1) / BN;
    hipStream_t st = (hipStream_t)stream;

    if (d->group_mode == 0) {
        p.m_tiles = (d->M + BM - 1) / BM + (d->group_offsets ? d->groups : 0);
        const int64_t blocks = (int64_t)p.m_tiles * p.n_tiles;
        GAMER_CHECK_ARG(blocks < (1LL << 31), "gamer_gemm_f32: grid too large");
        if (a_kc && b_kc) return launch_gemm<true, true, 0>(p, (int)blocks, st, split);
        if (a_kc && !b_kc) return launch_gemm<true, false, 0>(p, (int)blocks, st, split);
        if (!a_kc && !b_kc) return launch_gemm<false, false, 0>(p, (int)blocks, st, split);
        GAMER_CHECK_ARG(false, "gamer_gemm_f32: layout (A row-contiguous, B k-contiguous) is not built");
    } else {
        GAMER_CHECK_ARG(!a_kc && !b_kc, "gamer_gemm_f32: group_mode 1 (wgrad) needs row-contiguous A and B");
        GAMER_CHECK_ARG(d->kchunk >= BK && d->kchunk % BK == 0, "gamer_gemm_f32: kchunk=%d must be a positive multiple of 32", d->kchunk);
        p.m_tiles = (d->M + BM - 1) / BM;
        const int64_t chunks = (d->K + d->kchunk - 1) / d->kchunk + (d->group_offsets ? d->groups : 0);
        const int64_t blocks = chunks * p.m_tiles * p.n_tiles;
        GAMER_CHECK_ARG(blocks < (1LL << 31), "gamer_gemm_f32: grid too large");
        p.wgrad_ws = d->wgrad_ws;
        if (p.wgrad_ws) {
            const int64_t need = chunks * p.m_tiles * p.n_tiles * (int64_t)(BM * BN);
            GAMER_CHECK_ARG(d->wgrad_ws_floats >= need && aligned16(d->wgrad_ws),
                            "gamer_gemm_f32: wgrad_ws holds %lld floats, this weight gradient needs %lld (chunks x tiles x 16384)",
                            (long long)d->wgrad_ws_floats, (long long)need);
            GAMER_CHECK_ARG(!diag_pp_switch(), "gamer_gemm_f32: the deterministic weight gradient is not built for the ping-pong form");
        }
        const int rc = (split == 3 && p.wgrad_ws && gemm_wg_eligible(d, a_kc, b_kc)) ? launch_gemm_wg(d, st)
                                                                                     : launch_gemm<false, false, 1>(p, (int)blocks, st, split);
        if (rc || !p.wgrad_ws) return rc;
        const int64_t rblocks = (int64_t)d->groups * p.m_tiles * p.n_tiles * 16;
        hipLaunchKernelGGL(wgrad_reduce_kernel, dim3((int)rblocks), dim3(256), 0, st, p.wgrad_ws, d->C, d->ldc, d->M, d->N, p.m_tiles,
                           p.n_tiles, d->groups, d->group_offsets, d->K, d->kchunk, d->strideC);
        GAMER_CHECK_LAUNCH("gamer_gemm_f32/wgrad_reduce");
        return 0;
    }
    return 0;
}

__device__ __forceinline__ uint32_t amax4(uint32_t m, const uint4 v) {
    return max(max(m, v.x & 0x7fffffffu), max(max(v.y & 0x7fffffffu, v.z & 0x7fffffffu), v.w & 0x7fffffffu));
}
__device__ __forceinline__ void amax_commit(uint32_t m, uint32_t* __restrict__ out) {
    __shared__ uint32_t part[4];
#pragma unroll
    for (int o = 32; o > 0; o >>= 1) m = max(m, (uint32_t)__shfl_xor((int)m, o, 64));
    if ((threadIdx.x & 63) == 0) part[threadIdx.x >> 6] = m;
    __syncthreads();
    if (threadIdx.x == 0) {
        m = max(max(part[0], part[1]), max(part[2], part[3]));
        if (m) amax_publish(m, out, blockIdx.x);
    }
}
__global__ void __launch_bounds__(256)
absmax_flat_kernel(const uint4* __restrict__ x, int64_t n4, uint32_t* __restrict__ out) {
    uint32_t m = 0;
    const int64_t step = (int64_t)gridDim.x * 256;
    int64_t i = (int64_t)blockIdx.x * 256 + threadIdx.x;
    for (; i + step < n4; i += 2 * step) {
        const uint4 a = x[i], b = x[i + step];
        m = amax4(amax4(m, a), b);
    }
    if (i < n4) m = amax4(m, x[i]);
    amax_commit(m, out);
}
__global__ void __launch_bounds__(256)
absmax_rows_kernel(const float* __restrict__ x, int batch, int64_t stride, int rows, int cols, int64_t ld, uint32_t* __restrict__ out) {
    const int lane = threadIdx.x & 63;
    const int64_t waves = (int64_t)gridDim.x * 4, nrows = (int64_t)batch * rows;
    uint32_t m = 0;
    for (int64_t w = (int64_t)blockIdx.x * 4 + (threadIdx.x >> 6); w < nrows; w += waves) {
        const int64_t b = w / rows, r = w - b * rows;
        const float* src = x + b * stride + r * ld;
        for (int c = lane << 2; c < cols; c += 256) {
            if (c + 3 < cols) m = amax4(m, *reinterpret_cast<const uint4*>(src + c));
            else for (int q = 0; c + q < cols; ++q) m = max(m, __float_as_uint(src[c + q]) & 0x7fffffffu);
        }
    }
    amax_commit(m, out);
}
extern "C" int gamer_absmax_f32(const float* x, int batch, int64_t stride, int rows, int cols, int64_t ld, uint32_t* out, void* stream) {
    GAMER_CHECK_ARG(x && out && batch >= 1 && rows >= 1 && cols >= 1 && ld >= cols && ld % 4 == 0 && stride % 4 == 0 &&
                    (reinterpret_cast<uintptr_t>(x) & 15u) == 0, "gamer_absmax_f32: bad arguments (rows=%d cols=%d ld=%lld)",
// ... 14 lines not shown
    return 0;
}

__global__ void __launch_bounds__(256)
absmax_multi_kernel(const float* __restrict__ base, const int64_t* __restrict__ table, int bpe, uint32_t* __restrict__ out) {
    const int e = blockIdx.x / bpe, part = blockIdx.x % bpe;
    const uint4* x = reinterpret_cast<const uint4*>(base + table[2 * e]);
    const int64_t n4 = table[2 * e + 1] >> 2;
    uint32_t m = 0;
    for (int64_t i = (int64_t)part * 256 + threadIdx.x; i < n4; i += (int64_t)bpe * 256) m = amax4(m, x[i]);
    __shared__ uint32_t part4[4];
#pragma unroll
    for (int o = 32; o > 0; o >>= 1) m = max(m, (uint32_t)__shfl_xor((int)m, o, 64));
    if ((threadIdx.x & 63) == 0) part4[threadIdx.x >> 6] = m;
    __syncthreads();
    if (threadIdx.x == 0) {
        m = max(max(part4[0], part4[1]), max(part4[2], part4[3]));
        if (m) amax_publish(m, out + (int64_t)e * 256, (uint32_t)part);
    }
}
extern "C" int gamer_absmax_multi_f32(const float* base, const int64_t* table, int n, uint32_t* out, void* stream) {
    GAMER_CHECK_ARG(base && table && out && n >= 1 && (reinterpret_cast<uintptr_t>(base) & 15u) == 0, "gamer_absmax_multi_f32: bad arguments");
    const int bpe = 16;
    hipLaunchKernelGGL(absmax_multi_kernel, dim3(n * bpe), dim3(256), 0, (hipStream_t)stream, base, table, bpe, out);
    GAMER_CHECK_LAUNCH("gamer_absmax_multi_f32");
    return 0;
}

__global__ void __launch_bounds__(256)
split2h_planes_multi_kernel(const float* __restrict__ base, const int64_t* __restrict__ table, int bpe,
                            const uint32_t* __restrict__ slots, uint16_t* __restrict__ planes) {
    const int e = blockIdx.x / bpe, part = blockIdx.x % bpe;
    const int64_t off = table[2 * e], n4 = table[2 * e + 1] >> 2;
    float s, inv;
    scale_from_amax(amax_read(slots + (int64_t)e * 256), s, inv);
    const float4* x = reinterpret_cast<const float4*>(base + off);
    for (int64_t i = (int64_t)part * 256 + threadIdx.x; i < n4; i += (int64_t)bpe * 256) {
        uint2 img[2];
        split2h_quad(x[i], s, img);
        reinterpret_cast<uint4*>(planes)[(off >> 2) + i] = make_uint4(img[0].x, img[0].y, img[1].x, img[1].y);
    }
}
extern "C" int gamer_split2h_planes_multi(const float* base, const int64_t* table, int n, const uint32_t* slots, gamer_bf16* planes,
                                          void* stream) {
    GAMER_CHECK_ARG(base && table && slots && planes && n >= 1 && (reinterpret_cast<uintptr_t>(base) & 15u) == 0 &&
                    (reinterpret_cast<uintptr_t>(planes) & 15u) == 0, "gamer_split2h_planes_multi: bad arguments");
    const int bpe = 16;
    hipLaunchKernelGGL(split2h_planes_multi_kernel, dim3(n * bpe), dim3(256), 0, (hipStream_t)stream, base, table, bpe, slots,
                       reinterpret_cast<uint16_t*>(planes));
    GAMER_CHECK_LAUNCH("gamer_split2h_planes_multi");
    return 0;
}

__global__ void __launch_bounds__(256)
split2h_transpose_multi_kernel(const uint4* __restrict__ planes, const int64_t* __restrict__ table, int bpe, uint4* __restrict__ planes_t) {
    const int e = blockIdx.x / bpe, part = blockIdx.x % bpe;
    const int64_t off4 = table[3 * e] >> 2;
    const int rows = (int)table[3 * e + 1], cols = (int)table[3 * e + 2];
    const int r4n = rows >> 2, c4n = cols >> 2;
    const int64_t units = (int64_t)r4n * cols;
    for (int64_t u = (int64_t)part * 256 + threadIdx.x; u < units; u += (int64_t)bpe * 256) {
        const int r4 = (int)(u / cols), c = (int)(u % cols);
        uint32_t h0[4], h1[4];
#pragma unroll
        for (int i = 0; i < 4; ++i) {
            const uint4 s = planes[off4 + (int64_t)(4 * r4 + i) * c4n + (c >> 2)];
            const uint32_t w0 = (c & 2) ? s.y : s.x, w1 = (c & 2) ? s.w : s.z;
            h0[i] = (c & 1) ? (w0 >> 16) : (w0 & 0xffffu);
            h1[i] = (c & 1) ? (w1 >> 16) : (w1 & 0xffffu);
        }
        planes_t[off4 + (int64_t)c * r4n + r4] = make_uint4(h0[0] | (h0[1] << 16), h0[2] | (h0[3] << 16), h1[0] | (h1[1] << 16), h1[2] | (h1[3] << 16));
    }
}
extern "C" int gamer_split2h_transpose_multi(const gamer_bf16* planes, const int64_t* table, int n, gamer_bf16* planes_t, void* stream) {
    GAMER_CHECK_ARG(planes && table && planes_t && n >= 1 && aligned16(planes) && aligned16(planes_t), "gamer_split2h_transpose_multi: bad arguments");
    const int bpe = 16;
    hipLaunchKernelGGL(split2h_transpose_multi_kernel, dim3(n * bpe), dim3(256), 0, (hipStream_t)stream, reinterpret_cast<const uint4*>(planes),
                       table, bpe, reinterpret_cast<uint4*>(planes_t));
    GAMER_CHECK_LAUNCH("gamer_split2h_transpose_multi");
    return 0;
}

extern "C" int gamer_gemm_f32(const gamer_gemm_desc* d, void* stream) { return gemm_entry(d, stream, 0); }

extern "C" int gamer_split3_guard(int on) {
    const int prev = g_split3_guard;
    if (on >= 0) g_split3_guard = on ? 1 : 0;
    return prev;
}

extern "C" int gamer_gemm_f32_split(const gamer_gemm_desc* d, int terms, void* stream) {
    GAMER_CHECK_ARG(terms == 3 || terms == 6 || terms == 9, "gamer_gemm_f32_split: terms=%d (3, 6 or 9)", terms);
    return gemm_entry(d, stream, terms);
}
```

### gamer_amd/csrc/qknorm_rope.hip

```cpp
#include "common.h"

#pragma clang fp contract(off)

namespace gamer {

__device__ __forceinline__ void ld8(const bf16_t* p, float (&f)[8]) {
    const bf16x8 v = *reinterpret_cast<const bf16x8*>(p);
#pragma unroll
    for (int e = 0; e < 8; ++e) f[e] = (float)v[e];
}
__device__ __forceinline__ void st8(bf16_t* p, const float (&f)[8]) {
    f32x8v v;
#pragma unroll
    for (int e = 0; e < 8; ++e) v[e] = f[e];
    *reinterpret_cast<bf16x8*>(p) = __builtin_convertvector(v, bf16x8);
}
template <typename TA> struct RowLanes;
template <> struct RowLanes<float> {
    static constexpr int LANES = 16, E = 4;
    static __device__ __forceinline__ void ld(const float* p, float (&f)[4]) {
        const float4 v = ld4(p);
        f[0] = v.x; f[1] = v.y; f[2] = v.z; f[3] = v.w;
    }
    static __device__ __forceinline__ void st(float* p, const float (&f)[4]) { st4(p, make_float4(f[0], f[1], f[2], f[3])); }
// ... 326 lines not shown
    if (cross) {
#pragma unroll
        for (int a = 0; a < NBR; ++a) {
#pragma unroll
            for (int e = 0; e < E; ++e) dbacc[a][e] = rows_sum<L>(dbacc[a][e]);
            if (a < nb1 && sub == 0) st_f32(prow + (1 + a) * 64, dbacc[a]);
        }
    }
}

template <typename TA>
__global__ void __launch_bounds__(EW_THREADS)
qknorm_rope_bwd_tok_kernel(const TA* __restrict__ qkv, const TA* __restrict__ dq_rot, const TA* __restrict__ dk_rot,
                           int T, int S, int nq, int nkv, const float* __restrict__ wq, const float* __restrict__ wk, float eps,
                           const float* __restrict__ cos_t, const float* __restrict__ sin_t, TA* __restrict__ dqkv,
                           float* __restrict__ partial, int n_waves, const int32_t* __restrict__ pos_ids,
                           uint32_t* __restrict__ amax_out) {
    using L = RowLanes<TA>;
    constexpr int E = L::E, ROWS = 64 / L::LANES;
    constexpr bool F32 = sizeof(TA) == 4;
    const int lane = threadIdx.x & 63;
    const int g = lane % L::LANES, sub = lane / L::LANES;
    const int wave = (int)(((int64_t)blockIdx.x * EW_THREADS + threadIdx.x) >> 6);
    if (wave >= n_waves) return;
    float am = 0.f;
    const int nqk = nq + nkv;
    const int ldqkv = (nq + 2 * nkv) * 64;
    float wqv[E], wkv[E], dwq[E], dwk[E];
    ld_f32(wq + E * g, wqv);
    ld_f32(wk + E * g, wkv);
#pragma unroll
    for (int e = 0; e < E; ++e) { dwq[e] = 0.f; dwk[e] = 0.f; }
    const float sgn = g < L::LANES / 2 ? 1.f : -1.f;
    for (int tb = wave * ROWS; tb < T; tb += n_waves * ROWS) {
        const int t = tb + sub;
        const bool live = t < T;
        const int tc = live ? t : T - 1;
        const int pos = pos_ids ? pos_ids[tc] : tc % S;
        float cs[E], sn[E];
        ld_f32(cos_t + pos * 64 + E * g, cs);
        ld_f32(sin_t + pos * 64 + E * g, sn);
        const TA* xrow = qkv + (int64_t)tc * ldqkv + E * g;
        const TA* dqrow = dq_rot + (int64_t)tc * nq * 64 + E * g;
        const TA* dkrow = dk_rot + (int64_t)tc * nkv * 64 + E * g;
        for (int h0 = 0; h0 < nqk; h0 += 3) {
            float xs[3][E], ds[3][E];
#pragma unroll
            for (int u = 0; u < 3; ++u) {
                const int hd = min(h0 + u, nqk - 1);
                L::ld(xrow + hd * 64, xs[u]);
                L::ld(hd < nq ? dqrow + hd * 64 : dkrow + (hd - nq) * 64, ds[u]);
            }
#pragma unroll
            for (int u = 0; u < 3; ++u) {
                const int hd = h0 + u;
                if (hd >= nqk) break;
                const bool isq = hd < nq;
                float dx[E], dwr[E];
#pragma unroll
                for (int e = 0; e < E; ++e) dwr[e] = F32 ? -0.f : (isq ? dwq[e] : dwk[e]);
                bwd_row<TA>(xs[u], ds[u], isq ? wqv : wkv, cs, sn, eps, sgn, false, live ? 1.f : 0.f, dx, dwr);
#pragma unroll
                for (int e = 0; e < E; ++e) {
                    if (isq) dwq[e] = F32 ? dwq[e] + dwr[e] : dwr[e];
                    else dwk[e] = F32 ? dwk[e] + dwr[e] : dwr[e];
                }
                if (live) {
                    L::st(dqkv + (int64_t)t * ldqkv + hd * 64 + E * g, dx);
                    if (F32) am = amax_row(am, dx);
                }
            }
        }
    }
    if (F32) bwd_amax_commit(am, amax_out, lane, (uint32_t)wave);
    float* prow = partial + (int64_t)wave * 128 + E * g;
#pragma unroll
    for (int e = 0; e < E; ++e) { dwq[e] = rows_sum<L>(dwq[e]); dwk[e] = rows_sum<L>(dwk[e]); }
    if (sub == 0) {
        st_f32(prow, dwq);
        st_f32(prow + 64, dwk);
    }
}

constexpr int QKR_CW = 8;
constexpr int QKR_RG = 1024 / QKR_CW;
__global__ void __launch_bounds__(1024)
qknorm_partial_reduce_kernel(const float* __restrict__ partial, int n_rows, int nq, int nkv, int cross, int nb1,
                             float* __restrict__ dwq, float* __restrict__ dwk, float* __restrict__ dbias_q,
                             float* __restrict__ dbias_k, float* __restrict__ dbias_v) {
    __shared__ float sh[16][QKR_CW];
    const int cl = threadIdx.x & (QKR_CW - 1), rg = threadIdx.x / QKR_CW;
    const int NH = nq + nkv + (cross ? nkv : 0);
    const int SL = 1 + (cross ? nb1 : 0);
    const int64_t row_stride = (int64_t)NH * SL * 64;
    const int col = blockIdx.x * QKR_CW + cl;
    int h0, h1, slot, c;
    float* dst;
    if (col < 64) { h0 = 0; h1 = nq; slot = 0; c = col; dst = dwq + c; }
    else if (col < 128) { h0 = nq; h1 = nq + nkv; slot = 0; c = col - 64; dst = dwk + c; }
    else {
        const int b = col - 128;
        const int hd = b / (nb1 * 64), a = (b / 64) % nb1;
        c = b % 64; h0 = hd; h1 = hd + 1; slot = 1 + a;
        if (hd < nq) dst = dbias_q + (int64_t)a * nq * 64 + hd * 64 + c;
        else if (hd < nq + nkv) dst = dbias_k + (int64_t)a * nkv * 64 + (hd - nq) * 64 + c;
        else dst = dbias_v + (int64_t)a * nkv * 64 + (hd - nq - nkv) * 64 + c;
    }
    const int nh = h1 - h0;
    const int64_t n_items = (int64_t)n_rows * nh;
    float s0 = 0.f, s1 = 0.f, s2 = 0.f, s3 = 0.f;
    auto at = [&](int64_t it) { return partial[(it / nh) * row_stride + ((int64_t)(h0 + it % nh) * SL + slot) * 64 + c]; };
    int64_t it = rg;
    for (; it + 3 * QKR_RG < n_items; it += 4 * QKR_RG) {
        s0 += at(it); s1 += at(it + QKR_RG); s2 += at(it + 2 * QKR_RG); s3 += at(it + 3 * QKR_RG);
    }
    for (; it < n_items; it += QKR_RG) s0 += at(it);
    float t = (s0 + s1) + (s2 + s3);
    t += __shfl_xor(t, 8, 64); t += __shfl_xor(t, 16, 64); t += __shfl_xor(t, 32, 64);
    const int lane = threadIdx.x & 63, w = threadIdx.x >> 6;
    if (lane < QKR_CW) sh[w][lane] = t;
    __syncthreads();
    if (threadIdx.x < QKR_CW) {
        float tot = 0.f;
#pragma unroll
        for (int gi = 0; gi < 16; ++gi) tot += sh[gi][threadIdx.x];
        *dst += tot;
    }
}

static bool qknorm_row_major() {
    static EnvSwitch sw("GAMER_QKNORM_ROW_MAJOR");
    return sw.is_set();
}

template <typename TA>
static int qknorm_rope_fwd_impl(const char* name, TA* qkv, int T, int S, int nq, int nkv, const float* wq,
                                const float* wk, float eps, const float* cos_t, const float* sin_t, const float* bias_q,
                                const float* bias_k, const float* bias_v, const int32_t* act_idx, TA* q_rot, TA* k_rot,
                                const int32_t* pos_ids, void* stream) {
    GAMER_CHECK_ARG(qkv && wq && wk && cos_t && sin_t && q_rot && k_rot, "%s: null pointer", name);
    GAMER_CHECK_ARG(T > 0 && S > 0 && nq > 0 && nkv > 0 && T % S == 0, "%s: bad shape T=%d S=%d nq=%d nkv=%d", name, T, S, nq, nkv);
    const bool cross = bias_q != nullptr;
    GAMER_CHECK_ARG(!cross || (bias_k && bias_v && act_idx), "%s: cross needs bias_k, bias_v, act_idx", name);
    const int NH = nq + nkv + (cross ? nkv : 0);
    constexpr int ROWS = 64 / RowLanes<TA>::LANES;
    AmaxSink sink = {};
    if constexpr (sizeof(TA) == 4) sink = take_amax_sink();
    const bool row_major = qknorm_row_major();
    const dim3 grid(grid_for_waves(((int64_t)T * (row_major ? NH : 1) + ROWS - 1) / ROWS));
    return with_flags([&](auto rm) {
        return launch<rm() ? qknorm_rope_fwd_row_kernel<TA> : qknorm_rope_fwd_tok_kernel<TA>>(
            name, grid, dim3(EW_THREADS), 0, ST(stream), qkv, T, S, nq, nkv, wq, wk, eps, cos_t, sin_t, bias_q, bias_k, bias_v, act_idx, q_rot,
            k_rot, pos_ids, sink.out[0], sink.out[1], sink.out[2]);
    }, row_major);
}
extern "C" int gamer_qknorm_rope_fwd(float* qkv, int T, int S, int nq, int nkv, const float* wq, const float* wk,
                                     float eps, const float* cos_t, const float* sin_t, const float* bias_q,
                                     const float* bias_k, const float* bias_v, const int32_t* act_idx, float* q_rot,
                                     float* k_rot, const int32_t* pos_ids, void* stream) {
    return qknorm_rope_fwd_impl<float>("gamer_qknorm_rope_fwd", qkv, T, S, nq, nkv, wq, wk, eps, cos_t, sin_t, bias_q,
                                       bias_k, bias_v, act_idx, q_rot, k_rot, pos_ids, stream);
}
extern "C" int gamer_qknorm_rope_fwd_bf16(gamer_bf16* qkv, int T, int S, int nq, int nkv, const float* wq,
                                          const float* wk, float eps, const float* cos_t, const float* sin_t,
                                          const float* bias_q, const float* bias_k, const float* bias_v,
                                          const int32_t* act_idx, gamer_bf16* q_rot, gamer_bf16* k_rot,
                                          const int32_t* pos_ids, void* stream) {
    return qknorm_rope_fwd_impl<bf16_t>("gamer_qknorm_rope_fwd_bf16", (bf16_t*)qkv, T, S, nq, nkv, wq, wk, eps, cos_t,
                                        sin_t, bias_q, bias_k, bias_v, act_idx, (bf16_t*)q_rot, (bf16_t*)k_rot, pos_ids,
                                        stream);
}

template <typename TA>
static int qknorm_rope_bwd_impl(const char* name, const TA* qkv, const TA* dq_rot, const TA* dk_rot, int T, int S,
                                int nq, int nkv, const float* wq, const float* wk, float eps, const float* cos_t,
                                const float* sin_t, const float* bias_q, const float* bias_k, const int32_t* act_idx,
                                int nb1, TA* dqkv, float* dwq, float* dwk, float* dbias_q, float* dbias_k,
                                float* dbias_v, const int32_t* pos_ids, float* partial, int64_t partial_numel,
                                void* stream) {
    GAMER_CHECK_ARG(qkv && dq_rot && dk_rot && wq && wk && cos_t && sin_t && dqkv && dwq && dwk && partial,
                    "%s: null pointer", name);
    GAMER_CHECK_ARG(T > 0 && S > 0 && nq > 0 && nkv > 0 && T % S == 0, "%s: bad shape", name);
    const int cross = bias_q != nullptr ? 1 : 0;
    GAMER_CHECK_ARG(!cross || (bias_k && act_idx && dbias_q && dbias_k && dbias_v && nb1 > 0 && nb1 <= TBL_MAXROWS),
                    "%s: cross needs bias_k, act_idx, dbias_*, 0<nb1<=8 (nb1=%d)", name, nb1);
    const int NH = nq + nkv + (cross ? nkv : 0);
    const int SL = 1 + (cross ? nb1 : 0);
    constexpr bool F32 = sizeof(TA) == 4;
    constexpr int ROWS = 64 / RowLanes<TA>::LANES;
    int waves_per_head = 8192 / NH;
    if (waves_per_head > (T + ROWS - 1) / ROWS) waves_per_head = (T + ROWS - 1) / ROWS;
    const int64_t cap = partial_numel / ((int64_t)NH * SL * 64);
    if (waves_per_head > cap) waves_per_head = (int)cap;
    GAMER_CHECK_ARG(waves_per_head >= 1 && aligned16(partial),
                    "%s: partial needs at least %d floats, 16-byte aligned (got %lld)", name, NH * SL * 64,
                    (long long)partial_numel);
    int n_waves = (T + ROWS - 1) / ROWS;
    if (n_waves > 8192) n_waves = 8192;
    if ((int64_t)n_waves * 128 > partial_numel) n_waves = (int)(partial_numel / 128);
    auto reduce = [&](int n_rows, int rq, int rkv, int rcross, int rnb1, int cols) {
        return launch<qknorm_partial_reduce_kernel>(name, dim3(cols / QKR_CW), dim3(1024), 0, ST(stream), (const float*)partial, n_rows, rq, rkv,
                                                    rcross, rnb1, dwq, dwk, dbias_q, dbias_k, dbias_v);
    };
    uint32_t* amax_out = nullptr;
    if (!cross && !qknorm_row_major() && n_waves >= 1) {
        if constexpr (F32) amax_out = take_amax_sink().out[0];
        GAMER_TRY(launch<qknorm_rope_bwd_tok_kernel<TA>>(name, dim3((n_waves + EW_WAVES - 1) / EW_WAVES), dim3(EW_THREADS), 0, ST(stream), qkv,
                                                         dq_rot, dk_rot, T, S, nq, nkv, wq, wk, eps, cos_t, sin_t, dqkv, partial, n_waves,
                                                         pos_ids, amax_out));
        return reduce(n_waves, 1, 1, 0, 0, 128);
    }
    const int64_t total_waves = (int64_t)NH * waves_per_head;
    const dim3 grid((int)((total_waves + EW_WAVES - 1) / EW_WAVES));
    if constexpr (F32) amax_out = take_amax_sink().out[0];
    GAMER_TRY(with_flags([&](auto four) {
        return launch<qknorm_rope_bwd_head_kernel<TA, (!F32 && four()) ? 4 : TBL_MAXROWS>>(
            name, grid, dim3(EW_THREADS), 0, ST(stream), qkv, dq_rot, dk_rot, T, S, nq, nkv, wq, wk, eps, cos_t, sin_t, cross, bias_q, bias_k,
            act_idx, nb1, dqkv, partial, waves_per_head, pos_ids, amax_out);
    }, !cross || nb1 <= 4));
    return reduce(waves_per_head, nq, nkv, cross, nb1, 128 + (cross ? NH * nb1 * 64 : 0));
}
extern "C" int gamer_qknorm_rope_bwd(const float* qkv, const float* dq_rot, const float* dk_rot, int T, int S, int nq,
                                     int nkv, const float* wq, const float* wk, float eps, const float* cos_t,
                                     const float* sin_t, const float* bias_q, const float* bias_k,
                                     const int32_t* act_idx, int nb1, float* dqkv, float* dwq, float* dwk,
                                     float* dbias_q, float* dbias_k, float* dbias_v, const int32_t* pos_ids,
                                     float* partial, int64_t partial_numel, void* stream) {
    return qknorm_rope_bwd_impl<float>("gamer_qknorm_rope_bwd", qkv, dq_rot, dk_rot, T, S, nq, nkv, wq, wk, eps, cos_t,
                                       sin_t, bias_q, bias_k, act_idx, nb1, dqkv, dwq, dwk, dbias_q, dbias_k, dbias_v,
                                       pos_ids, partial, partial_numel, stream);
}
extern "C" int gamer_qknorm_rope_bwd_bf16(const gamer_bf16* qkv, const gamer_bf16* dq_rot, const gamer_bf16* dk_rot,
                                          int T, int S, int nq, int nkv, const float* wq, const float* wk, float eps,
                                          const float* cos_t, const float* sin_t, const float* bias_q,
                                          const float* bias_k, const int32_t* act_idx, int nb1, gamer_bf16* dqkv,
                                          float* dwq, float* dwk, float* dbias_q, float* dbias_k, float* dbias_v,
                                          const int32_t* pos_ids, float* partial, int64_t partial_numel, void* stream) {
    return qknorm_rope_bwd_impl<bf16_t>("gamer_qknorm_rope_bwd_bf16", (const bf16_t*)qkv, (const bf16_t*)dq_rot,
                                        (const bf16_t*)dk_rot, T, S, nq, nkv, wq, wk, eps, cos_t, sin_t, bias_q, bias_k,
                                        act_idx, nb1, (bf16_t*)dqkv, dwq, dwk, dbias_q, dbias_k, dbias_v, pos_ids,
                                        partial, partial_numel, stream);
}

}
```

### gamer_amd/engine.py

```python
from __future__ import annotations

import contextlib
import functools
import math
import os
from types import SimpleNamespace
from typing import Dict, List, Optional, Tuple

import torch

from . import ops
from .config import Qwen3MultiConfig

IGNORE_INDEX = -100


def _round_up(x: int, m: int) -> int:
    return (x + m - 1) // m * m


class _FlatLayout:

    def __init__(self, decay: List[Tuple[str, tuple]], nodecay: List[Tuple[str, tuple]]):
        self.entries: Dict[str, Tuple[int, tuple]] = {}
# ... 515 lines not shown
                    self._amax.register_transposed(Wl.cross_attn["o"], 1, H, NQ)
        span_self = span_cross = None
        if self.variant == "session":
            if session_ids is None:
                raise ValueError("Session IDs must be provided to generate session-wise causal mask.")
            sid = session_ids.to(self.device, torch.int64).contiguous()
            ext = (extended_session_ids.to(self.device, torch.int64).contiguous()
                   if extended_session_ids is not None else None)
            if ws.session is None:
                i32 = torch.int32
                if "s_violations" not in ws._store:
                    ws._store["s_violations"] = torch.zeros(1, dtype=i32, device=self.device)
                ws.session = {"span_self": ws._buf("s_span_self", (B, S, 4), i32),
                              "span_cross": ws._buf("s_span_cross", (B, S, 4), i32),
                              "pos_ids": ws._buf("s_pos_ids", (B, S), i32), "violations": ws._store["s_violations"]}
            ws.session["violations"].zero_()
            ops.session_spans(sid, ext, am, cfg.num_positions, S, r, ws.session)
            span_self, span_cross, pos_ids = (ws.session["span_self"], ws.session["span_cross"],
                                              ws.session["pos_ids"])
        elif self.key_spans:
            span_self = ws.session["span_self"]
        if cfg.cross_attention_decoder:
            ops.attn_row_order(r["empty_cross"], *ws.cross_order)
        ops.embedding_fwd(ids, self.params["model.embed_tokens.weight"], ws.x[0][0])

        fuse_qkv = ((self.fuse_qkv_bf16 if bf16 else self.fuse_qkv) and ops.qkv_fused_ok(ws.layers[0]["h1"], T, QKV)
                    and cfg.head_dim == 64)
        attention = functools.partial(self._attention, c)

        for l in range(cfg.num_hidden_layers):
            W, A, xs = self.W[l], ws.layers[l], ws.x[l]
            Wm = self.Wm[l]
            if hidden_sink is not None:
                hidden_sink.append(xs[0].view(B, S, H).clone())
            self._self_attention(c, l, r, span_self, pos_ids, fuse_qkv, kv_dest, kv_sink)
            xcur = xs[1]
            if W.cross:
                C, Cm = W.cross_attn, Wm.cross_attn
                nrm = dict(norm=dict(x=xs[1], w=W.ln2, eps=eps)) if (c.fuse_norm and not fuse_qkv) else {}
                fuse_bias = c.fuse_bias and not fuse_qkv
                if not nrm:
                    ops.rmsnorm_fwd(xs[1], W.ln2, eps, A["h2"])
                qkv_x, k_x = kv_dest(l, "cross") if kv_dest is not None else (A["qkv_c"], A["k_c"])
                h2_hold = self._amax.hold(A["h2"]) if (self._amax is not None and not train) else None
                if h2_hold is not None:
                    h2_hold.__enter__()
                if fuse_qkv:
                    ops.gemm(A["h2"], H, 1, Cm["qkv"], H, 1, qkv_x, QKV, T, QKV, H,
                             qknorm=dict(wq=C["qn"], wk=C["kn"], eps=eps, cos=cos, sin=sin, q_rot=A["q_c"], k_rot=k_x,
                                         bias_q=C["bq"], bias_k=C["bk"], bias_v=C["bv"], act_idx=r["act_idx"],
                                         pos_ids=pos_ids, S=S, nq=nq, nkv=nkv))
                elif fuse_bias:
                    ops.linear_fwd(A["h2"], H, Cm["qkv"], H, qkv_x, QKV, T, QKV, H,
                                   bias=dict(idx=r["act_idx"], q=C["bq"], k=C["bk"], v=C["bv"]),
                                   c_amax=(qkv_x[:, NQ + NKV:], NQ + NKV), **nrm)
                    ops.qknorm_rope_fwd(qkv_x, S, nq, nkv, C["qn"], C["kn"], eps, cos, sin, A["q_c"], k_x, pos_ids=pos_ids)
                else:
                    ops.linear_fwd(A["h2"], H, Cm["qkv"], H, qkv_x, QKV, T, QKV, H, **nrm)
                    ops.qknorm_rope_fwd(qkv_x, S, nq, nkv, C["qn"], C["kn"], eps, cos, sin, A["q_c"], k_x,
                                        bias_q=C["bq"], bias_k=C["bk"], bias_v=C["bv"], act_idx=r["act_idx"],
                                        pos_ids=pos_ids)
                if kv_sink is not None:
                    kv_sink(l, "cross", k_x, qkv_x[:, NQ + NKV:])
                if (last_row_logits and l == cfg.num_hidden_layers - 1 and span_cross is None and not bf16 and
                        os.environ.get("GAMER_PREFILL_LAST_ROW", "1") != "0"):
                    rows = torch.arange(B, device=self.device) * S + (S - 1)
                    f32 = dict(dtype=torch.float32, device=self.device)
                    q_l = A["q_c"].index_select(0, rows).contiguous()
                    key_ok = (r["kl_cross"].view(B, S) < r["ql_cross"].view(B, S)[:, S - 1:S]).to(torch.int32).contiguous()
                    uni = (r["empty_cross"].view(B, S)[:, S - 1] != 0).to(torch.int32).contiguous()
                    kg0 = torch.zeros(B, 1, NKV, **f32)
                    ao_l = torch.empty(B, NQ, **f32)
                    ops.attn_decode(q_l, k_x, qkv_x[:, NQ + NKV:], key_ok, kg0, kg0, 0, False, uni, B, 1, S, nq, nkv, scale, ao_l)
                    op_l, gate_l, x_cross_last = torch.empty(B, H, **f32), torch.empty(B, H, **f32), torch.empty(B, H, **f32)
                    ops.linear_fwd(ao_l, NQ, Cm["o"], NQ, op_l, H, B, H, NQ)
                    ops.linear_fwd(A["h2"].index_select(0, rows).contiguous(), H, Cm["gate"], H, gate_l, H, B, H, H)
                    ops.silu_gate_fwd(op_l, gate_l, x_cross_last, resid=xs[1].index_select(0, rows).contiguous())
                    xcur = None
                else:
                    x_cross_last = None
                    attention(A["q_c"], k_x, qkv_x[:, NQ + NKV:], r["kl_cross"], r["ql_cross"], r["empty_cross"],
                              r["tile_empty_cross"], self._seed(l, 2), A["ao_c"], A["lse_c"], ws.cross_order, span_cross)
                if x_cross_last is None:
                    ops.linear_fwd(A["ao_c"], NQ, Cm["o"], NQ, A["op_c"], H, T, H, NQ)
                    ops.linear_fwd(A["h2"], H, Cm["gate"], H, A["gate_c"], H, T, H, H)
                if h2_hold is not None:
                    h2_hold.__exit__(None, None, None)
                if x_cross_last is None:
                    ops.silu_gate_fwd(A["op_c"], A["gate_c"], xs[2], resid=xs[1], p=p_res, seed=self._seed(l, 3))
                    xcur = xs[2]
            din = W.din
            if last_row_logits and l == cfg.num_hidden_layers - 1:
                rows = torch.arange(B, device=self.device) * S + (S - 1)
                xl = x_cross_last if (W.cross and x_cross_last is not None) else xcur.index_select(0, rows).contiguous()
                f32 = dict(dtype=torch.float32, device=self.device)
                beh = r["beh_idx"].view(-1).index_select(0, rows).contiguous() if W.inject else None
                x_last = torch.empty(B, H, **f32)
                self._ffn_last_rows(W, S, rows, xl, beh, x_last, Wm)
                break
            xnext = ws.x[l + 1][0] if l + 1 < cfg.num_hidden_layers else ws.x_final
            if not self._shipped_ffn_layer(W):
                self._ffn_fwd_plain(c, l, xcur, xnext)
                continue
            grp = dict(groups=E, group_offsets=ws.offsets)
            nrm = dict(norm=dict(x=xcur, w=W.ln3, eps=eps, dst_rows=ws.slot, src_rows=ws.perm)) if c.fuse_norm else {}
            if W.inject and self.split_inject:
                hin = A["hin"].view(-1)[:T * H].view(T, H)
                if not nrm:
                    ops.rmsnorm_fwd(xcur, W.ln3, eps, hin, H, ws.slot)
                tb = ws._buf((f"l{l}_" if train else "l_") + "inject_tbl", (E * NB1, 2 * I))
                ops.inject_table_fwd(W.beh, W.gu, din, H, E, 2 * I, tb)
                if c.fuse_swiglu_fwd:
                    ops.gemm(hin, H, 1, Wm.gu, din, 1, A["gu"], 2 * I, T, 2 * I, H, strideB=2 * I * din, groups=E * NB1,
                             group_offsets=ws.grp_offsets, group_div=NB1, p_drop=p_res, seed=self._seed(l, 4),
                             swiglu_fwd=(A["hm"], tb, ws.row_group), **nrm)
                else:
                    ops.linear_fwd(hin, H, Wm.gu, din, A["gu"], 2 * I, T, 2 * I, H, strideB=2 * I * din, **grp, **nrm)
                    ops.swiglu_fwd_ld_tbl(A["gu"], 2 * I, T, I, p_res, self._seed(l, 4), A["hm"], tb, ws.row_group)
            else:
                if din != H:
                    nrm = {}
                if not nrm:
                    ops.rmsnorm_fwd(xcur, W.ln3, eps, A["hin"], din, ws.slot)
                if W.inject:
                    ops.rowtable_fwd(W.beh, r["beh_idx"], A["hin"], din, H, ws.slot)
                if c.fuse_swiglu_fwd and din == H:
                    ops.gemm(A["hin"], din, 1, Wm.gu, din, 1, A["gu"], 2 * I, T, 2 * I, din, strideB=2 * I * din, p_drop=p_res,
                             seed=self._seed(l, 4), swiglu_fwd=(A["hm"], None, None), **grp, **nrm)
                else:
                    ops.linear_fwd(A["hin"], din, Wm.gu, din, A["gu"], 2 * I, T, 2 * I, din, strideB=2 * I * din, **grp, **nrm)
                    ops.swiglu_fwd_ld(A["gu"], 2 * I, T, I, p_res, self._seed(l, 4), A["hm"])
            ops.gemm(A["hm"], I, 1, Wm.down, I, 1, xnext, H, T, H, I, strideB=H * I, resid=xcur, row_map=ws.perm,
                     p_drop=p_res, seed=self._seed(l, 5), **grp)
        return self._head(c, x_last if last_row_logits else None, num_items_in_batch, hidden_sink)

    def _route(self, c, actions, act_zero_col, rope_from_mask: bool):
        if rope_from_mask:
            raise ValueError("rope_from_mask is an option of the models without behaviour levels")
        cfg, r, S = self.cfg, c.ws.router, c.S
        act = actions.to(self.device, torch.int64).contiguous() if actions is not None else None
        ops.router_fwd(c.ids, c.am, act, self.lut, cfg.num_positions, cfg.pad_token_id, cfg.eos_token_id, r)
        if self.position_table is not None:
            ops.router_position_table(r["expert"], self.position_table)
        if act_zero_col is None and S % cfg.num_positions == 1:
            act_zero_col = S - 1
        if act_zero_col is not None:
            r["act_idx"][:, act_zero_col] = 0
        return None

    def _bf16_refusal(self, kv_dest, generation: bool) -> Optional[str]:
        if kv_dest is not None:
            return "kv_dest is built for dtype='f32' only (a bf16 generation copies its caches through kv_sink)"
        if generation and self.variant != "multi":
            return f"generation on a dtype='bf16' engine is built for the default variant (Qwen3Multi), not for variant {self.variant!r}"
        return None

    def _shipped_ffn_layer(self, W) -> bool:
        return W.sparse and W.gated and not self.cfg.Moe_behavior_only

    def _ffn_rows(self, l: int):
        return self.ws.slot if self.W[l].sparse else None

    def _ffn_fwd_plain(self, c, l: int, xcur, xnext):
        ws, W, Wm, A = c.ws, self.W[l], self.Wm[l], c.ws.layers[l]
        T, H, I, din, nI = c.T, c.H, c.I, W.din, W.nI
        slot = ws.slot if W.sparse else None
        grp = dict(groups=W.ne, group_offsets=ws.offsets) if W.sparse else {}
        phantom = W.sparse and self.cfg.Moe_behavior_only
        ops.rmsnorm_fwd(xcur, W.ln3, c.eps, A["hin"], din, slot)
        if W.inject:
            ops.rowtable_fwd(W.beh, ws.router["beh_idx"], A["hin"], din, H, slot)
        gu = A["gu"].view(-1)[:T * nI].view(T, nI)
        if phantom:
            gu.zero_()
        ops.linear_fwd(A["hin"], din, Wm.gu, din, gu, nI, T, nI, din, **(dict(strideB=nI * din) if W.sparse else {}), **grp)
        if W.gated:
            ops.swiglu_fwd_ld(gu, nI, T, I, c.p_res, self._seed(l, 4), A["hm"])
        else:
            ops.silu_fwd_ld(gu, nI, T, I, c.p_res, self._seed(l, 4), A["hm"])
        if phantom:
            xnext.copy_(xcur)
        ops.gemm(A["hm"], I, 1, Wm.down, I, 1, xnext, H, T, H, I, resid=xcur, p_drop=c.p_res, seed=self._seed(l, 5),
                 **(dict(strideB=H * I, row_map=ws.perm) if W.sparse else {}), **grp)

    def _ffn_bwd_plain(self, c, l: int, xlast):
        ws, W, G, A = c.ws, self.W[l], self.G[l], c.ws.layers[l]
        WT = self.WT[l] if c.bf16 else None
        T, H, I, din, nI = c.T, c.H, c.I, W.din, W.nI
        t0 = ws.tmpH[0]
        slot = ws.slot if W.sparse else None
        grp = dict(groups=W.ne, group_offsets=ws.offsets) if W.sparse else {}
        sB = (lambda n: dict(strideB=n)) if W.sparse else (lambda n: {})
        sC = (lambda n: dict(strideC=n)) if W.sparse else (lambda n: {})
        if W.sparse and self.cfg.Moe_behavior_only:
            ws.dhm.zero_()
            ws.dhin.zero_()
        with c.hold(t0):
            ops.linear_wgrad(t0, H, A["hm"], I, G.down, I, T, H, I, **sC(H * I), **grp)
            self._dgrad(c, t0, H, W.down, WT.down if c.bf16 else None, I, ws.dhm, I, H, I, **sB(H * I), **grp)
        gu = A["gu"].view(-1)[:T * nI].view(T, nI)
        if W.gated:
            ops.swiglu_bwd_ld(gu, nI, T, I, ws.dhm, c.p_res, self._seed(l, 4))
        else:
            ops.silu_bwd_ld(gu, nI, T, I, ws.dhm, c.p_res, self._seed(l, 4))
        with c.hold(gu):
            ops.linear_wgrad(gu, nI, A["hin"], din, G.gu, din, T, nI, din, **sC(nI * din), **grp)
            self._dgrad(c, gu, nI, W.gu, WT.gu if c.bf16 else None, din, ws.dhin, din, nI, din, **sB(nI * din), **grp)
        if W.inject:
            ops.rowtable_bwd(ws.dhin, din, H, ws.router["beh_idx"], G.beh, slot, partial=ws.norm_partial[-1])
        self._norm_bwd(c, xlast, W.ln3, ws.dhin, din, G.ln3, True, slot,
                       branch=None if W.cross else (self._seed(l, 1), None))

    def ffn_rows(self, W, pos: int, x, beh, out, Wm=None):
        cfg = self.cfg
        Wm = W if Wm is None else Wm
        B, H, I, din, nI = x.shape[0], cfg.hidden_size, cfg.intermediate_size, W.din, W.nI
        e = cfg.position_experts()[pos] if W.sparse else 0
        if e >= W.ne:
            out.copy_(x)
            return
        act = dict(dtype=Wm.gu.dtype, device=self.device)
        hin = torch.empty(B, din, **act)
        ops.rmsnorm_fwd(x, W.ln3, float(cfg.rms_norm_eps), hin, din)
        if W.inject:
            ops.rowtable_fwd(W.beh, beh, hin, din, H)
        gu, hm = torch.empty(B, nI, **act), torch.empty(B, I, **act)
        ops.linear_fwd(hin, din, Wm.gu[e * nI:(e + 1) * nI], din, gu, nI, B, nI, din)
        if W.gated:
            ops.swiglu_fwd_ld(gu, nI, B, I, 0.0, 0, hm)
        else:
            ops.silu_fwd_ld(gu, nI, B, I, 0.0, 0, hm)
        ops.gemm(hm, I, 1, Wm.down[e * H:(e + 1) * H], I, 1, out, H, B, H, I, resid=x)

    def _ffn_last_rows(self, W, S: int, rows, x, beh, out, Wm):
        self.ffn_rows(W, (S - 1) % self.cfg.num_positions, x, beh, out, Wm)

    def _pass(self, B: int, S: int, p_res: float, p_att: float) -> SimpleNamespace:
        cfg = self.cfg
        c = SimpleNamespace(B=B, S=S, T=B * S, H=cfg.hidden_size, nq=cfg.num_attention_heads, nkv=cfg.num_key_value_heads,
                            dh=cfg.head_dim, I=cfg.intermediate_size, eps=float(cfg.rms_norm_eps), p_res=p_res, p_att=p_att,
                            bf16=self.dtype == "bf16")
        c.NQ, c.NKV = c.nq * c.dh, c.nkv * c.dh
        c.QKV = c.NQ + 2 * c.NKV
        c.scale = float(c.dh) ** -0.5
        c.cos, c.sin = self.rope(S)
        c.split_attn = self.split_attention and self.matmul != "f32" and not c.bf16
        c.h2 = c.split_attn and self.h2_attention and self.matmul == "split3" and p_att < 0.75
        c.fuse_swiglu_fwd = not c.bf16 and self.matmul == "split3" and os.environ.get("GAMER_FUSE_SWIGLU_FWD", "1") != "0"
        c.fuse_swiglu_bwd = (c.bf16 or self.matmul == "split3") and self.fuse_swiglu_bwd
        c.fuse_norm = not c.bf16 and self.matmul == "split3" and os.environ.get("GAMER_GEMM_AS_NORM", "1") != "0"
        c.fuse_bias = not c.bf16 and self.matmul == "split3" and os.environ.get("GAMER_GEMM_AS_BIAS", "1") != "0"
        return c

    def _prologue(self, input_ids, attention_mask, labels, train, dropout, dropout_rate, kv_dest, hidden_sink,
                  last_row_logits, uniform_len, eval_only: Optional[str], f32_only: Optional[str]) -> SimpleNamespace:
        B, S = input_ids.shape
        if kv_dest is not None and train:
            raise ValueError("kv_dest is an evaluation-only option (the backward reads the workspace's q|k|v and keys)")
        if eval_only and (train or labels is not None):
            raise ValueError(eval_only)
        if hidden_sink is not None and last_row_logits:
            raise ValueError("hidden_sink needs the full-sequence forward")
        if self.dtype == "bf16":
            if f32_only:
                raise NotImplementedError(f32_only)
            self.shadow.refresh()
        if self.weight_planes is not None:
            ops.split3_planes(self.flat_p, self.weight_planes)
        use_drop = train if dropout is None else dropout
        c = self._pass(B, S, float(dropout_rate) if use_drop else 0.0,
                       float(self.cfg.attention_dropout) if use_drop else 0.0)
        if use_drop:
            self.dropout_step += 1
        ws = c.ws = self.ws = self.workspace(B, S, train)
        if self._amax is not None:
            self._amax.reset()
            if train:
                self._amax.stable(ws.xn, *[A[k] for A in ws.layers for k in ("h1", "h2", "ao", "ao_c", "hin", "hm") if k in A])
                if self.h2_attention:
                    self._amax.stable(*[A[k] for A in ws.layers for k in ("q", "k", "q_c", "k_c") if k in A],
                                      *[A[k][:, c.NQ + c.NKV:] for A in ws.layers for k in ("qkv", "qkv_c") if k in A])
        c.ids = input_ids.to(self.device, torch.int64).contiguous()
        c.am = attention_mask.to(self.device, torch.int64).contiguous() if attention_mask is not None else None
        c.lab = labels.to(self.device, torch.int64).contiguous() if labels is not None else None
        c.uniform_len, c.train = uniform_len, train
        if c.lab is not None:
            ws.bad_label.zero_()
            ops.check_labels(c.lab, self.cfg.vocab_size, IGNORE_INDEX, ws.bad_label)
        return c

    def _attention(self, c, qb, kb, vb, kl_, ql_, empty_, tile_empty_, seed_, ob, lseb, order_, span_):
        B, S, nq, nkv, NQ, NKV, QKV = c.B, c.S, c.nq, c.nkv, c.NQ, c.NKV, c.QKV
        if c.split_attn and (span_ is None or c.h2):
            ops.attn_fwd_split(qb, NQ, kb, NKV, vb, QKV, kl_, ql_, empty_, B, S, nq, nkv, c.scale, c.p_att, seed_, ob, lseb,
                               order=order_, h2=c.h2, uniform_len=c.uniform_len, q_span=span_)
        elif c.bf16:
            ord16 = (order_[0], order_[2], empty_) if (order_ is not None and span_ is None) else None
            ops.attn_fwd_bf16(qb, NQ, kb, NKV, vb, QKV, kl_, ql_, B, S, nq, nkv, c.scale, c.p_att, seed_, ob, lseb,
                              q_span=span_, order=ord16)
        else:
            ops.attn_fwd(qb, NQ, kb, NKV, vb, QKV, kl_, ql_, empty_, tile_empty_, B, S, nq, nkv, c.scale, c.p_att, seed_,
                         ob, lseb, order=order_, uniform_len=c.uniform_len, q_span=span_)

    def _self_attention(self, c, l: int, masks: dict, span, pos_ids, fuse_qkv: bool, kv_dest, kv_sink):
        W, Wm, A, xs = self.W[l], self.Wm[l], c.ws.layers[l], c.ws.x[l]
        T, H, NQ, NKV, QKV, eps = c.T, c.H, c.NQ, c.NKV, c.QKV, c.eps
        nrm = dict(norm=dict(x=xs[0], w=W.ln1, eps=eps)) if (c.fuse_norm and not fuse_qkv) else {}
        if not nrm:
            ops.rmsnorm_fwd(xs[0], W.ln1, eps, A["h1"])
        qkv_s, k_s = kv_dest(l, "self") if kv_dest is not None else (A["qkv"], A["k"])
        if fuse_qkv:
            ops.gemm(A["h1"], H, 1, Wm.self_attn["qkv"], H, 1, qkv_s, QKV, T, QKV, H,
                     qknorm=dict(wq=W.self_attn["qn"], wk=W.self_attn["kn"], eps=eps, cos=c.cos, sin=c.sin, q_rot=A["q"],
                                 k_rot=k_s, pos_ids=pos_ids, S=c.S, nq=c.nq, nkv=c.nkv))
        else:
            v_amax = dict(c_amax=(qkv_s[:, NQ + NKV:], NQ + NKV)) if (c.h2 and self.gemm_c_amax) else {}
            ops.linear_fwd(A["h1"], H, Wm.self_attn["qkv"], H, qkv_s, QKV, T, QKV, H, **v_amax, **nrm)
            ops.qknorm_rope_fwd(qkv_s, c.S, c.nq, c.nkv, W.self_attn["qn"], W.self_attn["kn"], eps, c.cos, c.sin, A["q"], k_s,
                                pos_ids=pos_ids)
        if kv_sink is not None:
            kv_sink(l, "self", k_s, qkv_s[:, NQ + NKV:])
        self._attention(c, A["q"], k_s, qkv_s[:, NQ + NKV:], masks["kl_self"], None, masks["empty_self"],
                        masks["tile_empty_self"], self._seed(l, 0), A["ao"], A["lse"], None, span)
        ops.gemm(A["ao"], NQ, 1, Wm.self_attn["o"], NQ, 1, xs[1], H, T, H, NQ, resid=xs[0], p_drop=c.p_res,
                 seed=self._seed(l, 1))

    def _head(self, c, x_last: Optional[torch.Tensor], num_items_in_batch, hidden_sink):
        ws, B, S, H, eps = c.ws, c.B, c.S, c.H, c.eps
        V = self.cfg.vocab_size
        if x_last is not None:
            xn = torch.empty_like(x_last, dtype=self.act_dtype)
            ops.rmsnorm_fwd(x_last, self.params["model.norm.weight"], eps, xn)
            small = torch.empty(B, ws.ldl, dtype=torch.float32, device=self.device)
            if c.bf16:
# ... 57 lines not shown
        with ops.deterministic(True if self.deterministic else ops.DETERMINISTIC_WGRAD, bf16=True if self.deterministic else None):
            return self._backward(dloss, layer_done, dloss_dev)

    def _backward(self, dloss: float = 1.0, layer_done=None, dloss_dev: Optional[torch.Tensor] = None):
        cfg = self.cfg
        c = self._backward_head(dloss, dloss_dev, rows=self._ffn_rows(cfg.num_hidden_layers - 1))
        ws, B, S, T, H, I, E = c.ws, c.B, c.S, c.T, c.H, c.I, cfg.num_ffn_experts
        nq, nkv, NQ, NKV, QKV, eps, cos, sin, p_res = c.nq, c.nkv, c.NQ, c.NKV, c.QKV, c.eps, c.cos, c.sin, c.p_res
        NB1 = cfg.num_behavior + 1
        span_self = span_cross = pos_ids = None
        if self.key_spans:
            span_self, span_cross, pos_ids = ws.session["span_self"], ws.session["span_cross"], ws.session["pos_ids"]
        r = ws.router
        NP = ws.norm_partial[-1]
        hold, fuse_delta, do_amax, fuse_swiglu_bwd = c.hold, c.fuse_delta, c.do_amax, c.fuse_swiglu_bwd
        dgrad, norm_bwd = functools.partial(self._dgrad, c), functools.partial(self._norm_bwd, c)
        attention_bwd = functools.partial(self._attention_bwd, c)
        t0, t1, t2, t3 = ws.tmpH
        bf16 = c.bf16
        for l in reversed(range(cfg.num_hidden_layers)):
            W, G, A, xs = self.W[l], self.G[l], ws.layers[l], ws.x[l]
            WT = self.WT[l] if bf16 else None
            din = W.din
            grp = dict(groups=E, group_offsets=ws.offsets)
            xlast = xs[2] if W.cross else xs[1]
            if not self._shipped_ffn_layer(W):
                self._ffn_bwd_plain(c, l, xlast)
            else:
                split_inj = W.inject and self.split_inject
                tb = ws._buf(f"l{l}_inject_tbl", (E * NB1, 2 * I)) if split_inj else None
                with hold(t0):
                    ops.linear_wgrad(t0, H, A["hm"], I, G.down, I, T, H, I, strideC=H * I, **grp)
                    if fuse_swiglu_bwd and split_inj:
                        ops.gemm(t0, H, 1, W.down, 1, I, ws.dhm, I, T, I, H, strideB=H * I, p_drop=p_res, seed=self._seed(l, 4),
                                 swiglu_bwd=(A["gu"], 2 * I), groups=E * NB1, group_offsets=ws.grp_offsets, group_div=NB1, sw_tbl=tb)
                    elif fuse_swiglu_bwd:
                        if bf16:
                            ops.linear_dgrad_t(t0, H, WT.down, WT.down.shape[1], ws.dhm, I, T, H, I, strideB=H * I, p_drop=p_res,
                                               seed=self._seed(l, 4), swiglu_bwd=(A["gu"], 2 * I), **grp)
                        else:
                            ops.gemm(t0, H, 1, W.down, 1, I, ws.dhm, I, T, I, H, strideB=H * I, p_drop=p_res, seed=self._seed(l, 4),
                                     swiglu_bwd=(A["gu"], 2 * I), **grp)
                    else:
                        dgrad(t0, H, W.down, WT.down if bf16 else None, I, ws.dhm, I, H, I, strideB=H * I, **grp)
                if not fuse_swiglu_bwd:
                    if split_inj:
                        ops.swiglu_bwd_ld_tbl(A["gu"], 2 * I, T, I, ws.dhm, p_res, self._seed(l, 4), tb, ws.row_group)
                    else:
                        ops.swiglu_bwd_ld(A["gu"], 2 * I, T, I, ws.dhm, p_res, self._seed(l, 4))
                if split_inj:
                    hin = A["hin"].view(-1)[:T * H].view(T, H)
                    dhin = ws.dhin.view(-1)[:T * H].view(T, H)
                    with hold(A["gu"]):
                        ops.linear_wgrad(A["gu"], 2 * I, hin, H, G.gu, din, T, 2 * I, H, strideC=2 * I * din, **grp)
                        dgrad(A["gu"], 2 * I, W.gu, None, din, dhin, H, 2 * I, H, strideB=2 * I * din, **grp)
                    seg = ws._buf("inject_segsum", (E * NB1, 2 * I))
                    seg_ws = ws._buf("inject_seg_ws", (ops.segment_colsum_ws_floats(T, 2 * I, E * NB1),))
                    ops.segment_colsum(A["gu"], 2 * I, T, 2 * I, ws.grp_offsets, E * NB1, seg_ws, seg)
                    ops.inject_table_bwd(seg, W.beh, W.gu, din, H, E, 2 * I, G.gu, G.beh,
                                         ws._buf("inject_scratch", (NB1 * E * cfg.behavior_embedding_dim,)))
                    norm_bwd(xlast, W.ln3, dhin, H, G.ln3, True, ws.slot, branch=None if W.cross else (self._seed(l, 1), None))
                else:
                    with hold(A["gu"]):
                        ops.linear_wgrad(A["gu"], 2 * I, A["hin"], din, G.gu, din, T, 2 * I, din, strideC=2 * I * din, **grp)
                        dgrad(A["gu"], 2 * I, W.gu, WT.gu if bf16 else None, din, ws.dhin, din, 2 * I, din, strideB=2 * I * din, **grp)
                    if W.inject:
                        ops.rowtable_bwd(ws.dhin, din, H, r["beh_idx"], G.beh, ws.slot, partial=NP)
                    norm_bwd(xlast, W.ln3, ws.dhin, din, G.ln3, True, ws.slot,
                             branch=None if W.cross else (self._seed(l, 1), None))
            if W.cross:
                C, GC = W.cross_attn, G.cross_attn
                CT = WT.cross_attn if bf16 else dict(o=None, gate=None, qkv=None)
                ops.silu_gate_bwd(A["op_c"], A["gate_c"], ws.dx, t1, t2, p=p_res, seed=self._seed(l, 3))
                hold_t2 = hold(t2)
                hold_t2.__enter__()
                with hold(t1):
                    ops.linear_wgrad(t1, H, A["ao_c"], NQ, GC["o"], NQ, T, H, NQ)
                    ops.linear_wgrad(t2, H, A["h2"], H, GC["gate"], H, T, H, H)
                    dgrad(t1, H, C["o"], CT["o"], NQ, ws.dao, NQ, H, NQ,
                          rowdot=(A["ao_c"], ws.delta, S) if fuse_delta else None, **do_amax)
                attention_bwd(A["q_c"], A["k_c"], A["qkv_c"][:, NQ + NKV:], A["ao_c"], A["lse_c"], r["kl_cross"],
                              r["ql_cross"], r["empty_cross"], r["tile_empty_cross"], self._seed(l, 2), ws.cross_order,
                              span_cross)
                ops.qknorm_rope_bwd(A["qkv_c"], ws.dq, ws.dk, S, nq, nkv, C["qn"], C["kn"], eps, cos, sin, ws.dqkv,
                                    GC["qn"], GC["kn"], bias_q=C["bq"], bias_k=C["bk"], act_idx=r["act_idx"], nb1=NB1,
                                    dbias_q=GC["bq"], dbias_k=GC["bk"], dbias_v=GC["bv"], pos_ids=pos_ids,
                                    partial=ws.qk_partial)
                with hold(ws.dqkv):
                    ops.linear_wgrad(ws.dqkv, QKV, A["h2"], H, GC["qkv"], H, T, QKV, H)
                    dgrad(ws.dqkv, QKV, C["qkv"], CT["qkv"], H, t3, H, QKV, H)
                dgrad(t2, H, C["gate"], CT["gate"], H, t3, H, H, H, accumulate=True)
                hold_t2.__exit__(None, None, None)
                norm_bwd(xs[1], W.ln2, t3, H, G.ln2, True, branch=(self._seed(l, 1), None))
            self._self_attention_bwd(c, l, r, span_self, pos_ids, rows=self._ffn_rows(l - 1) if l > 0 else None)
            if layer_done is not None:
                layer_done(l)
        self._backward_tail(c)

    def _backward_head(self, dloss, dloss_dev, rows) -> SimpleNamespace:
        sv = self._saved
        c = self._pass(sv["B"], sv["S"], sv["p_res"], sv["p_att"])
        ws = c.ws = self.ws
        c.saved_step = self.dropout_step
        self.dropout_step = sv["dropout_step"]
        c.ids, c.norm_dws = sv["ids"], []
        c.fuse_delta = (ws.ds_work is not None or c.bf16 or c.split_attn) and c.T % 128 == 0 and c.NQ % 128 == 0
        c.do_amax = dict(c_amax=(ws.dao, 0)) if (c.h2 and self.gemm_c_amax) else {}
        c.hold = self._amax.hold if self._amax is not None else (lambda *t: contextlib.nullcontext())
        V, H, T, L = self.cfg.vocab_size, c.H, c.T, self.cfg.num_hidden_layers
        if torch.is_tensor(sv["num_items"]):
            ops.ce_bwd(ws.logits, ws.ldl, sv["labels"], V, self.temperature, IGNORE_INDEX, ws.lse_ce, sv["num_items"], 0.0,
                       dloss, dloss_dev)
        elif sv["num_items"] is not None:
            ops.ce_bwd(ws.logits, ws.ldl, sv["labels"], V, self.temperature, IGNORE_INDEX, ws.lse_ce, None,
                       float(sv["num_items"]), dloss, dloss_dev)
        else:
            ops.ce_bwd(ws.logits, ws.ldl, sv["labels"], V, self.temperature, IGNORE_INDEX, ws.lse_ce, ws.count, 0.0,
                       dloss, dloss_dev)
        t3 = ws.tmpH[3]
        with c.hold(ws.logits):
            ops.linear_wgrad(ws.logits, ws.ldl, ws.xn, H, self.grads["model.embed_tokens.weight"], H, T, V, H)
            self._dgrad(c, ws.logits, ws.ldl, self.params["model.embed_tokens.weight"],
                        self.shadow.t("model.embed_tokens.weight") if c.bf16 else None, H, t3, H, V, H)
        self._norm_bwd(c, ws.x_final, self.params["model.norm.weight"], t3, H, self.grads["model.norm.weight"], False,
                       branch=(self._seed(L - 1, 5), rows))
        return c

    def _dgrad(self, c, dy, lddy, Wf, Wt, ldw, dx, lddx, n_out, k_in, **kw):
        if c.bf16:
            ops.linear_dgrad_t(dy, lddy, Wt, Wt.shape[1], dx, lddx, c.T, n_out if Wt.shape[1] == n_out else Wt.shape[1],
                               k_in, **kw)
        else:
            ops.linear_dgrad(dy, lddy, Wf, ldw, dx, lddx, c.T, n_out, k_in, **kw)

    def _norm_bwd(self, c, xin, w, dy, lddy, dw, accumulate_dx, dy_rows=None, branch=None):
        ws = c.ws
        part = ws.norm_partial[len(c.norm_dws)]
        c.norm_dws.append(dw)
        if branch is None:
            ops.rmsnorm_bwd(xin, w, dy, lddy, c.eps, ws.dx, part, accumulate_dx, dy_rows)
        else:
            ops.rmsnorm_bwd(xin, w, dy, lddy, c.eps, ws.dx, part, accumulate_dx, dy_rows, mask_out=ws.tmpH[0],
                            mask_rows=branch[1], p=c.p_res, seed=branch[0])

    def _attention_bwd(self, c, qb, kb, vb, ob, lseb, kl_, ql_, empty_, tile_empty_, seed_, order_, span_):
        ws, B, S, nq, nkv, NQ, NKV, QKV = c.ws, c.B, c.S, c.nq, c.nkv, c.NQ, c.NKV, c.QKV
        if c.split_attn and (span_ is None or c.h2):
            ops.attn_bwd_split(qb, NQ, kb, NKV, vb, QKV, ob, ws.dao, lseb, kl_, ql_, empty_, tile_empty_, B, S, nq, nkv, c.scale,
                               c.p_att, seed_, ws.delta, ws.dq, NQ, ws.dk, NKV, ws.dqkv[:, NQ + NKV:], QKV, order=order_,
                               delta_ready=c.fuse_delta, dv_of=ws.dqkv,
                               h2=c.h2, q_span=span_)
        elif c.bf16:
            ord16 = (order_[0], order_[2], empty_) if (order_ is not None and span_ is None) else None
            ops.attn_bwd_bf16(qb, NQ, kb, NKV, vb, QKV, ob, ws.dao, lseb, kl_, ql_, B, S, nq, nkv, c.scale, c.p_att, seed_,
                              ws.delta, ws.dq, NQ, ws.dk, NKV, ws.dqkv[:, NQ + NKV:], QKV, q_span=span_,
                              delta_ready=c.fuse_delta, order=ord16)
        else:
            ops.attn_bwd(qb, NQ, kb, NKV, vb, QKV, ob, ws.dao, lseb, kl_, ql_, empty_, tile_empty_, B, S, nq, nkv, c.scale,
                         c.p_att, seed_, ws.delta, ws.dq, NQ, ws.dk, NKV, ws.dqkv[:, NQ + NKV:], QKV, order=order_,
                         ds_work=ws.ds_work, q_span=span_, delta_ready=c.fuse_delta and ws.ds_work is not None)

    def _self_attention_bwd(self, c, l: int, masks: dict, span, pos_ids, rows):
        W, G, A, xs, ws = self.W[l], self.G[l], c.ws.layers[l], c.ws.x[l], c.ws
        T, H, NQ, NKV, QKV, S = c.T, c.H, c.NQ, c.NKV, c.QKV, c.S
        SA, GS = W.self_attn, G.self_attn
        ST = self.WT[l].self_attn if c.bf16 else dict(o=None, qkv=None)
        t0, t3 = ws.tmpH[0], ws.tmpH[3]
        with c.hold(t0):
            ops.linear_wgrad(t0, H, A["ao"], NQ, GS["o"], NQ, T, H, NQ)
            self._dgrad(c, t0, H, SA["o"], ST["o"], NQ, ws.dao, NQ, H, NQ,
# ... 73 lines not shown
```

### gamer_amd/ops.py

```python
from __future__ import annotations

import ctypes as C
from typing import Optional

import os

import torch

from . import _lib
from ._lib import GemmBf16Desc, GemmDesc, call, ptr, stream_ptr


def _sfx(t: torch.Tensor) -> str:
    if t.dtype == torch.float32:
        return ""
    if t.dtype == torch.bfloat16:
        return "_bf16"
    raise RuntimeError(f"activations must be float32 or bfloat16, got {t.dtype}")


def _chk(t: torch.Tensor, dtype, name: str):
    if not t.is_cuda:
        raise RuntimeError(f"{name} must be on the HIP device (gamer_amd has no CPU path)")
    if t.dtype != dtype:
# ... 478 lines not shown


def absmax_slot(x, batch, stride, rows, cols, ld, produced=False):
    if _AMAX_REUSE is not None:
        if produced:
            _AMAX_REUSE.preset(x, (batch, stride, rows, cols, ld))
        return _AMAX_REUSE.slot(x, (batch, stride, rows, cols, ld))
    key = (x.device.index, stream_ptr())
    ring = _AMAX_RING.get(key)
    if ring is None:
        ring = _AMAX_RING[key] = [torch.zeros(_AMAX_SLOTS * AMAX_WORDS, dtype=torch.int32, device=x.device), 0]
    if ring[1] == _AMAX_SLOTS:
        ring[0].zero_()
        ring[1] = 0
    slot = ring[0].data_ptr() + 4 * AMAX_WORDS * ring[1]
    ring[1] += 1
    if not produced:
        call("gamer_absmax_f32", ptr(x), batch, stride, rows, cols, ld, slot, stream_ptr())
    return slot


def split3_planes(x, planes):
    call("gamer_split3_planes", ptr(x), ptr(planes), x.numel(), planes.stride(0), stream_ptr())


DETERMINISTIC_WGRAD = os.environ.get("GAMER_WGRAD_TWO_PASS", "1") != "0"
DETERMINISTIC_WGRAD_BF16 = os.environ.get("GAMER_WGRAD_TWO_PASS_BF16", "0") == "1"
_WGRAD_WS = {}


class deterministic:

    def __init__(self, on: bool = True, bf16=None):
        self.on, self.bf16 = bool(on), bf16

    def __enter__(self):
        global DETERMINISTIC_WGRAD, DETERMINISTIC_WGRAD_BF16
        self.prev, DETERMINISTIC_WGRAD = DETERMINISTIC_WGRAD, self.on
        self.prev16 = DETERMINISTIC_WGRAD_BF16
        if self.bf16 is not None:
            DETERMINISTIC_WGRAD_BF16 = bool(self.bf16)
        return self

    def __exit__(self, *exc):
        global DETERMINISTIC_WGRAD, DETERMINISTIC_WGRAD_BF16
        DETERMINISTIC_WGRAD, DETERMINISTIC_WGRAD_BF16 = self.prev, self.prev16
        return False


def _wgrad_workspace(device, floats: int) -> torch.Tensor:
    t = _WGRAD_WS.get(device)
    if t is None or t.numel() < floats:
        _WGRAD_WS[device] = None
        t = _WGRAD_WS[device] = torch.empty(int(floats), dtype=torch.float32, device=device)
    return t


class split3_guard:

    def __init__(self, on: bool):
        self.on = bool(on)

    def __enter__(self):
        self.prev = _lib.load().gamer_split3_guard(1 if self.on else 0)
        return self

    def __exit__(self, *exc):
        _lib.load().gamer_split3_guard(self.prev)
        return False


def set_f32_matmul(mode) -> int:
    global F32_MATMUL_TERMS
    prev = F32_MATMUL_TERMS
    terms = MATMUL_MODES[mode] if isinstance(mode, str) else int(mode)
    if terms not in (0, 3, 6, 9):
        raise ValueError(f"fp32 matmul mode {mode!r}: one of {sorted(MATMUL_MODES)}")
    F32_MATMUL_TERMS = terms
    return prev


def gemm(A, a_rs, a_ks, Bm, b_rs, b_ks, Cm, ldc, M, N, K, alpha=1.0, accumulate=False, groups=1, group_mode=0,
         group_offsets=None, strideB=0, strideC=0, kchunk=0, resid=None, row_map=None, p_drop=0.0, seed=0,
         rowdot=None, qknorm=None, c_amax=None, swiglu_bwd=None, group_div=0, sw_tbl=None, swiglu_fwd=None, norm=None, bias=None):
    if A.dtype == torch.bfloat16:
        if group_div > 1 or sw_tbl is not None or swiglu_fwd is not None or norm is not None or bias is not None:
            raise RuntimeError("group_div / sw_tbl / swiglu_fwd / norm / bias are options of the fp32 GEMM")
        return _gemm_bf16(A, a_rs, a_ks, Bm, b_rs, b_ks, Cm, ldc, M, N, K, alpha, accumulate, groups, group_mode,
                          group_offsets, strideB, strideC, kchunk, resid, row_map, p_drop, seed, rowdot, qknorm, swiglu_bwd)
    d = GemmDesc()
    d.A = ptr(A); d.a_rs = a_rs; d.a_ks = a_ks
    d.B = ptr(Bm); d.b_rs = b_rs; d.b_ks = b_ks
    d.C = ptr(Cm); d.ldc = ldc
    d.M = M; d.N = N; d.K = K
    d.alpha = alpha
    d.accumulate = 1 if accumulate else 0
    d.groups = groups
    d.group_mode = group_mode
    d.group_offsets = ptr(group_offsets)
    d.strideB = strideB; d.strideC = strideC
    d.kchunk = kchunk
    d.resid = ptr(resid)
    d.row_map = ptr(row_map)
    d.p_drop = p_drop
    d.seed = seed
    if rowdot is not None:
        d.rowdot_other, d.rowdot_out, d.rowdot_S = ptr(rowdot[0]), ptr(rowdot[1]), int(rowdot[2])
    if qknorm is not None:
        q = qknorm
        d.qk_wq, d.qk_wk, d.qk_eps = ptr(q["wq"]), ptr(q["wk"]), float(q["eps"])
        d.qk_cos, d.qk_sin = ptr(q["cos"]), ptr(q["sin"])
        d.qk_bias_q, d.qk_bias_k, d.qk_bias_v = ptr(q.get("bias_q")), ptr(q.get("bias_k")), ptr(q.get("bias_v"))
        d.qk_act_idx, d.qk_pos_ids = ptr(q.get("act_idx")), ptr(q.get("pos_ids"))
        d.qk_q_rot, d.qk_k_rot = ptr(q["q_rot"]), ptr(q["k_rot"])
        d.qk_S, d.qk_nq, d.qk_nkv = int(q["S"]), int(q["nq"]), int(q["nkv"])
    if (c_amax is not None and _AMAX_REUSE is not None and F32_MATMUL_TERMS == 3 and group_mode == 0 and not accumulate
            and resid is None and qknorm is None and c_amax[1] % 64 == 0):
        view, col0 = c_amax
        slot_c = _AMAX_REUSE.preset(view, (1, 0, M, N - col0, ldc))
        d.amax_c, d.amax_c_col0 = slot_c, int(col0)
    if swiglu_bwd is not None:
        gu, ld_gu = swiglu_bwd
        d.sw_gu, d.sw_ld = ptr(gu), int(ld_gu)
        d.sw_tbl = ptr(sw_tbl)
        if _AMAX_REUSE is not None and F32_MATMUL_TERMS == 3 and ld_gu == 2 * N:
            d.amax_c, d.amax_c_col0 = _AMAX_REUSE.preset(gu, (1, 0, 1, M * ld_gu, M * ld_gu)), 0
    d.group_div = int(group_div)
    if norm is not None:
        nx = norm["x"]
        if group_mode != 0 or a_ks != 1 or b_ks != 1 or nx.dim() != 2 or nx.shape[0] < M or nx.shape[1] != K or not nx.is_contiguous():
            raise RuntimeError("gemm(norm=...): a Linear-forward GEMM whose rows are the RMSNorm of a dense [M, K] tensor")
        d.norm_x, d.norm_w, d.norm_eps = ptr(norm["x"]), ptr(norm["w"]), float(norm["eps"])
        d.norm_dst_rows, d.norm_src_rows = ptr(norm.get("dst_rows")), ptr(norm.get("src_rows"))
    if bias is not None:
        d.bias_idx, d.bias_q, d.bias_k, d.bias_v = ptr(bias["idx"]), ptr(bias["q"]), ptr(bias["k"]), ptr(bias["v"])
        d.bias_rows, d.bias_nq, d.bias_nkv = int(bias["q"].shape[0]), int(bias["q"].shape[1]), int(bias["k"].shape[1])
    if swiglu_fwd is not None:
        hm, tbl, row_group = swiglu_fwd
        d.sw_hm, d.sw_tbl, d.sw_row_group = ptr(hm), ptr(tbl), ptr(row_group)
        if _AMAX_REUSE is not None and F32_MATMUL_TERMS == 3:
            d.amax_c, d.amax_c_col0 = _AMAX_REUSE.preset(hm, (1, 0, 1, M * (N // 2), M * (N // 2))), 0
    if group_mode == 1 and DETERMINISTIC_WGRAD:
        n_chunks = (K + kchunk - 1) // kchunk + (groups if group_offsets is not None else 0)
        need = n_chunks * ((M + 127) // 128) * ((N + 127) // 128) * 16384
        ws = _wgrad_workspace(A.device, need)
        d.wgrad_ws, d.wgrad_ws_floats = ws.data_ptr(), ws.numel()
    if F32_MATMUL_TERMS == 3:
        ga = (M, K, a_rs) if a_ks == 1 else (K, M, a_ks)
        gb = (N, K, b_rs) if b_ks == 1 else (K, N, b_ks)
        nb = (groups // max(1, int(group_div))) if (group_mode == 0 and groups > 1) else 1
        d.amax_a = absmax_slot(A, 1, 0, *ga, produced=norm is not None)
        geom_b = (nb, strideB if nb > 1 else 0) + gb
        c = _AMAX_REUSE
        parent = c.plane_parent(Bm.data_ptr(), geom_b) if (c is not None and c.planes is not None and group_mode == 0) else None
        if parent is not None:
            d.amax_b = parent
            d.b_planes = c.planes.data_ptr() + (Bm.data_ptr() - c.stable_ranges[0][0])
            call("gamer_gemm_f32_split", C.byref(d), 3, stream_ptr())
            return
        d.amax_b = absmax_slot(Bm, *geom_b)
        if c is not None and c.planes is not None and group_mode == 0 and c._key(Bm.data_ptr(), geom_b) in c._plane_keys:
            d.b_planes = c.planes.data_ptr() + (Bm.data_ptr() - c.stable_ranges[0][0])
            if a_ks == 1 and b_ks == 1 and c._key(Bm.data_ptr(), geom_b) in c._tplane_keys:
                d.b_planes_t = c.planes_t.data_ptr() + (Bm.data_ptr() - c.stable_ranges[0][0])
        call("gamer_gemm_f32_split", C.byref(d), 3, stream_ptr())
        return
    if F32_MATMUL_TERMS:
        if WEIGHT_PLANES is not None and group_mode == 0:
            base, nbytes, pl, stride = WEIGHT_PLANES
            off = Bm.data_ptr() - base
            if 0 <= off < nbytes:
                d.b_planes, d.b_plane_stride = pl + off // 2, stride
        call("gamer_gemm_f32_split", C.byref(d), F32_MATMUL_TERMS, stream_ptr())
    else:
        call("gamer_gemm_f32", C.byref(d), stream_ptr())


def _gemm_bf16(A, a_rs, a_ks, Bm, b_rs, b_ks, Cm, ldc, M, N, K, alpha, accumulate, groups, group_mode, group_offsets,
               strideB, strideC, kchunk, resid, row_map, p_drop, seed, rowdot, qknorm=None, swiglu_bwd=None):
    if Bm.dtype != torch.bfloat16 or alpha != 1.0:
        raise RuntimeError("gamer_gemm_bf16 takes two bf16 operands and alpha = 1")
    d = GemmBf16Desc()
    if group_mode == 0:
        if a_ks != 1 or b_ks != 1:
            raise RuntimeError("bf16 GEMM: both operands must be k-contiguous (dgrad runs on the transposed weight copy)")
        d.lda, d.ldb = a_rs, b_rs
        want = torch.float32 if resid is not None else torch.bfloat16
    else:
# ... 115 lines not shown
        kchunk = min(16384, max(256, -(-per_group // chunks)))
        return (kchunk + 63) // 64 * 64
    return pick_kchunk(rows, groups > 1)


def _tune_kchunk(dy, lddy, x, ldx, dW, lddw, rows, N_out, K_in, groups, group_offsets, strideC):
    rule = _rule_kchunk(dy, rows, N_out, K_in, groups)
    if dy.dtype == torch.bfloat16:
        cands = {rule, 512, 1024, 2048, 4096, 8192, 16384, 1088, 2112, 3136, 4160, 6208}
    else:
        cands = {rule, 384, 512, 768, 1024, 1280, 1536, 2048, 3072, 4096}
        tiles = ((N_out + 127) // 128) * ((K_in + 127) // 128)
        per_group = max(1, rows // max(groups, 1))
        for rounds in (1, 2, 3, 4):
            n_chunks = max(1, (512 * rounds) // (tiles * max(groups, 1)))
            c = (-(-per_group // n_chunks) + 31) // 32 * 32
            if 256 <= c <= 8192:
                cands.add(c)
        if F32_MATMUL_TERMS == 3 and N_out % 256 == 0 and K_in % 256 == 0:
            tiles2 = (N_out // 256) * (K_in // 256)
            for rounds in (1, 2, 3, 4):
                n_chunks = max(1, (256 * rounds) // (tiles2 * max(groups, 1)))
                c = (-(-per_group // n_chunks) + 31) // 32 * 32
                if 256 <= c <= 8192:
                    cands.add(c)
            cands.update({1056, 2080, 3104, 4128})
    cands = sorted(c for c in cands if c <= max(256, rows))
    scratch = torch.zeros_like(dW)
    best, best_t = rule, float("inf")
    s, e = torch.cuda.Event(enable_timing=True), torch.cuda.Event(enable_timing=True)
    for c in cands:
        ts = []
        for it in range(4):
            s.record()
            gemm(dy, 1, lddy, x, 1, ldx, scratch, lddw, N_out, K_in, rows, groups=groups, group_mode=1,
                 group_offsets=group_offsets, strideC=strideC, kchunk=c)
            e.record()
            e.synchronize()
            if it:
                ts.append(s.elapsed_time(e))
        t = min(ts)
        if t < best_t * (0.98 if c != rule else 1.0):
            best, best_t = c, t
    return best


def wgrad_rows_bucket(rows: int) -> int:
    g = 1 << max(12, int(rows).bit_length() - 3)
    return -(-int(rows) // g) * g


def linear_wgrad(dy, lddy, x, ldx, dW, lddw, rows, N_out, K_in, groups=1, group_offsets=None, strideC=0, kchunk=None, tune_rows=None):
    if kchunk is None:
        key = (tune_rows or rows, N_out, K_in, groups, dy.dtype, F32_MATMUL_TERMS)
        kchunk = _WGRAD_TUNED.get(key)
        if kchunk is None and _tune_key_str(key) in _WGRAD_FILE_CACHE:
            kchunk = _WGRAD_TUNED[key] = _WGRAD_FILE_CACHE[_tune_key_str(key)]
        if kchunk is None:
            capturing = torch.cuda.is_current_stream_capturing()
            if rows >= 4096 and not capturing and _tune_allowed():
                kchunk = _tune_kchunk(dy, lddy, x, ldx, dW, lddw, rows, N_out, K_in, groups, group_offsets, strideC)
                if _WGRAD_TUNE_FILE:
                    _WGRAD_FILE_CACHE[_tune_key_str(key)] = int(kchunk)
                    _save_tune_file()
            else:
                kchunk = _rule_kchunk(dy, rows, N_out, K_in, groups)
            if not capturing:
                _WGRAD_TUNED[key] = kchunk
    gemm(dy, 1, lddy, x, 1, ldx, dW, lddw, N_out, K_in, rows, groups=groups, group_mode=1,
         group_offsets=group_offsets, strideC=strideC, kchunk=kchunk)


def qknorm_rope_fwd(qkv, S, nq, nkv, wq, wk, eps, cos_t, sin_t, q_rot, k_rot, bias_q=None, bias_k=None, bias_v=None,
                    act_idx=None, pos_ids=None):
    T = qkv.shape[0]
    outs = [(q_rot, (1, 0, T, nq * 64, nq * 64), False), (k_rot, (1, 0, T, nkv * 64, nkv * 64), False)]
    if bias_v is not None:
        outs.append((qkv[:, (nq + nkv) * 64:], (1, 0, T, nkv * 64, qkv.stride(0)), False))
    _arm_sink(*outs)
    call("gamer_qknorm_rope_fwd" + _sfx(qkv), ptr(qkv), T, S, nq, nkv, ptr(wq), ptr(wk), eps, ptr(cos_t), ptr(sin_t),
         ptr(bias_q), ptr(bias_k), ptr(bias_v), ptr(act_idx), ptr(q_rot), ptr(k_rot), ptr(pos_ids), stream_ptr())


def qknorm_partial_numel(nb1: int = 0) -> int:
    return 8192 * (1 + nb1) * 64


def qknorm_rope_bwd(qkv, dq_rot, dk_rot, S, nq, nkv, wq, wk, eps, cos_t, sin_t, dqkv, dwq, dwk, bias_q=None,
                    bias_k=None, act_idx=None, nb1=0, dbias_q=None, dbias_k=None, dbias_v=None, pos_ids=None,
                    partial=None):
    T = qkv.shape[0]
    if partial is None:
        partial = torch.empty(qknorm_partial_numel(nb1), dtype=torch.float32, device=qkv.device)
    _arm_sink((dqkv, (1, 0, T, dqkv.shape[1], dqkv.stride(0)), "only"))
    call("gamer_qknorm_rope_bwd" + _sfx(qkv), ptr(qkv), ptr(dq_rot), ptr(dk_rot), T, S, nq, nkv, ptr(wq), ptr(wk), eps,
         ptr(cos_t), ptr(sin_t), ptr(bias_q), ptr(bias_k), ptr(act_idx), nb1, ptr(dqkv), ptr(dwq), ptr(dwk),
         ptr(dbias_q), ptr(dbias_k), ptr(dbias_v), ptr(pos_ids), ptr(partial), partial.numel(), stream_ptr())


def attn_row_order(row_empty, perm, tile_kind, tile_maxpos):
    B, S = row_empty.shape
    call("gamer_attn_row_order", ptr(row_empty), B, S, ptr(perm), ptr(tile_kind), ptr(tile_maxpos), stream_ptr())


def attn_fwd(q, ldq, k, ldk, v, ldv, kl, ql, row_empty, tile_empty, B, S, nq, nkv, scale, p_drop, seed, o, lse,
             order=None, uniform_len=0, q_span=None):
    pm, tk, tm = order if order is not None else (None, None, None)
    call("gamer_attn_fwd", ptr(q), ldq, ptr(k), ldk, ptr(v), ldv, ptr(kl), ptr(ql), ptr(row_empty), ptr(tile_empty),
         B, S, nq, nkv, scale, p_drop, seed, ptr(o), ptr(lse), ptr(pm), ptr(tk), ptr(tm), uniform_len, ptr(q_span),
         stream_ptr())


def attn_bwd(q, ldq, k, ldk, v, ldv, o, d_o, lse, kl, ql, row_empty, tile_empty, B, S, nq, nkv, scale, p_drop, seed,
             delta, dq, lddq, dk, lddk, dv, lddv, order=None, ds_work=None, q_span=None, delta_ready=False):
    pm, tk, tm = order if order is not None else (None, None, None)
    call("gamer_attn_bwd", ptr(q), ldq, ptr(k), ldk, ptr(v), ldv, ptr(o), ptr(d_o), ptr(lse), ptr(kl), ptr(ql),
         ptr(row_empty), ptr(tile_empty), B, S, nq, nkv, scale, p_drop, seed, ptr(delta), ptr(dq), lddq, ptr(dk),
         lddk, ptr(dv), lddv, ptr(pm), ptr(tk), ptr(tm), ptr(ds_work), ptr(q_span),
         1 if (delta_ready and ds_work is not None) else 0, stream_ptr())


def attn_operand_maxima(q, ldq, k, ldk, v, ldv, T, nq, nkv, d_o=None):
    sl = [absmax_slot(q, 1, 0, T, nq * 64, ldq), absmax_slot(k, 1, 0, T, nkv * 64, ldk), absmax_slot(v, 1, 0, T, nkv * 64, ldv)]
    sl.append(absmax_slot(d_o, 1, 0, T, nq * 64, nq * 64) if d_o is not None else None)
    return sl


def attn_fwd_split(q, ldq, k, ldk, v, ldv, kl, ql, row_empty, B, S, nq, nkv, scale, p_drop, seed, o, lse, order=None,
                   h2=False, uniform_len=0, q_span=None):
    pm, tk, tm = order if order is not None else (None, None, None)
    if h2:
        call("gamer_attn_split_amax", *attn_operand_maxima(q, ldq, k, ldk, v, ldv, B * S, nq, nkv))
    if _AMAX_ATTN:
        _arm_sink((o, (1, 0, 1, B * S * nq * 64, B * S * nq * 64), False))
    call("gamer_attn_fwd_split", ptr(q), ldq, ptr(k), ldk, ptr(v), ldv, ptr(kl), ptr(ql), ptr(row_empty), B, S, nq, nkv,
         scale, p_drop, seed, ptr(o), ptr(lse), ptr(pm), ptr(tk), ptr(tm), int(uniform_len), ptr(q_span), stream_ptr())


def attn_bwd_split(q, ldq, k, ldk, v, ldv, o, d_o, lse, kl, ql, row_empty, tile_empty, B, S, nq, nkv, scale, p_drop, seed,
                   delta, dq, lddq, dk, lddk, dv, lddv, order=None, delta_ready=False, ds_work=None, dv_of=None, h2=False,
                   q_span=None):
    pm, tk, tm = order if order is not None else (None, None, None)
    if h2:
        call("gamer_attn_split_amax", *attn_operand_maxima(q, ldq, k, ldk, v, ldv, B * S, nq, nkv, d_o=d_o))
    if dv_of is not None and _AMAX_ATTN:
        _arm_sink((dv_of, (1, 0, dv_of.shape[0], dv_of.shape[1], dv_of.stride(0)), False))
    call("gamer_attn_bwd_split", ptr(q), ldq, ptr(k), ldk, ptr(v), ldv, ptr(o), ptr(d_o), ptr(lse), ptr(kl), ptr(ql),
         ptr(row_empty), ptr(tile_empty), B, S, nq, nkv, scale, p_drop, seed, ptr(delta), ptr(dq), lddq, ptr(dk), lddk, ptr(dv),
         lddv, ptr(pm), ptr(tk), ptr(tm), 1 if delta_ready else 0, ptr(ds_work), ptr(q_span), stream_ptr())


def attn_fwd_bf16(q, ldq, k, ldk, v, ldv, kl, ql, B, S, nq, nkv, scale, p_drop, seed, o, lse, q_span=None, order=None):
    perm, tmax, rempty = order if order is not None else (None, None, None)
    call("gamer_attn_fwd_bf16", ptr(q), ldq, ptr(k), ldk, ptr(v), ldv, ptr(kl), ptr(ql), B, S, nq, nkv, scale, p_drop,
         seed, ptr(o), ptr(lse), ptr(q_span), ptr(perm), ptr(tmax), ptr(rempty), stream_ptr())


def attn_bwd_bf16(q, ldq, k, ldk, v, ldv, o, d_o, lse, kl, ql, B, S, nq, nkv, scale, p_drop, seed, delta, dq, lddq, dk,
                  lddk, dv, lddv, q_span=None, delta_ready=False, order=None):
    perm, tmax, rempty = order if order is not None else (None, None, None)
    call("gamer_attn_bwd_bf16", ptr(q), ldq, ptr(k), ldk, ptr(v), ldv, ptr(o), ptr(d_o), ptr(lse), ptr(kl), ptr(ql),
         B, S, nq, nkv, scale, p_drop, seed, ptr(delta), ptr(dq), lddq, ptr(dk), lddk, ptr(dv), lddv, ptr(q_span),
         1 if delta_ready else 0, ptr(perm), ptr(tmax), ptr(rempty), stream_ptr())


def cast_params_bf16(flat, out, out_t, table, n_entries, n_tiles):
    call("gamer_cast_params_bf16", ptr(flat), ptr(out), ptr(out_t), ptr(table), n_entries, n_tiles, stream_ptr())

# ... 1099 lines not shown
```

### include/gamer_hip.h

```cpp
#ifndef GAMER_HIP_H
#define GAMER_HIP_H

#include <stdint.h>

#ifdef __cplusplus
extern "C" {
#endif

#define GAMER_ABI_VERSION 9
#define GAMER_AMAX_WORDS 256

typedef uint16_t gamer_bf16;

int gamer_abi_version(void);
const char* gamer_last_error(void);
int gamer_reload_env(void);

int gamer_router_fwd(const int64_t* ids, const int64_t* attn_mask, const int64_t* actions,
                     const int32_t* behavior_lut, int vocab, int B, int S, int num_positions,
                     int pad_id, int eos_id,
                     int32_t* expert, int32_t* beh_idx, int32_t* act_idx,
                     int32_t* kl_self, int32_t* kl_cross, int32_t* ql_cross,
                     int32_t* empty_self, int32_t* empty_cross,
                     int32_t* tile_empty_self, int32_t* tile_empty_cross,
// ... 45 lines not shown
                        void* stream);
int64_t gamer_embedding_bwd_ordered_ws_bytes(int V, int T, int H);
int gamer_embedding_bwd_ordered(const int64_t* ids, const float* dx, int V, int T, int H, int pad_id, float* dW,
                                void* ws, int64_t ws_bytes, void* stream);

int gamer_rmsnorm_fwd(const float* x, const float* w, int T, int H, float eps,
                      const int32_t* dst_rows, float* y, int ldy, void* stream);
int gamer_rmsnorm_bwd(const float* x, const float* w, const float* dy, int lddy,
                      const int32_t* dy_rows, int T, int H, float eps, int accumulate_dx,
                      float* dx, float* dw_partial, int n_partial,
                      float* mask_out, const int32_t* mask_rows, float p_drop, uint64_t seed, void* stream);
int gamer_rmsnorm_fwd_bf16(const float* x, const float* w, int T, int H, float eps,
                           const int32_t* dst_rows, gamer_bf16* y, int ldy, void* stream);
int gamer_rmsnorm_bwd_bf16(const float* x, const float* w, const gamer_bf16* dy, int lddy,
                           const int32_t* dy_rows, int T, int H, float eps, int accumulate_dx,
                           float* dx, float* dw_partial, int n_partial,
                           gamer_bf16* mask_out, const int32_t* mask_rows, float p_drop, uint64_t seed, void* stream);
int gamer_colsum_reduce(const float* partial, int rows, int cols, int accumulate, float* out,
                        void* stream);
int gamer_colsum_reduce_batched(const float* partial, int64_t stride, int rows, int cols, int n, float* const* outs,
                                int accumulate, void* stream);

int gamer_rowtable_fwd(const float* table, const int32_t* idx, const int32_t* dst_rows, int T, int E,
                       float* y, int ldy, int col0, void* stream);
int gamer_rowtable_bwd(const float* dy, int lddy, int col0, const int32_t* idx,
                       const int32_t* dy_rows, int T, int E, int n_rows_table, float* dtable,
                       float* partial, int64_t partial_numel, void* stream);
int gamer_rowtable_fwd_bf16(const float* table, const int32_t* idx, const int32_t* dst_rows, int T, int E,
                            gamer_bf16* y, int ldy, int col0, void* stream);
int gamer_rowtable_bwd_bf16(const gamer_bf16* dy, int lddy, int col0, const int32_t* idx,
                            const int32_t* dy_rows, int T, int E, int n_rows_table, float* dtable,
                            float* partial, int64_t partial_numel, void* stream);

typedef struct {
    const float* A; int64_t a_rs, a_ks;
    const float* B; int64_t b_rs, b_ks;
    float* C; int64_t ldc;
    int M, N, K;
    float alpha;
    int accumulate;
    int groups;
    int group_mode;
    const int32_t* group_offsets;
    int64_t strideB, strideC;
    int kchunk;
    const float* resid;
    const int32_t* row_map;
    float p_drop;
    uint64_t seed;
    const float* rowdot_other;
    float* rowdot_out;
    int rowdot_S;
    const float* qk_wq; const float* qk_wk;
    float qk_eps;
    const float* qk_cos; const float* qk_sin;
    const float* qk_bias_q; const float* qk_bias_k; const float* qk_bias_v;
    const int32_t* qk_act_idx;
    const int32_t* qk_pos_ids;
    float* qk_q_rot; float* qk_k_rot;
    int qk_S, qk_nq, qk_nkv;
    const gamer_bf16* b_planes;
    int64_t b_plane_stride;
    const uint32_t* amax_a;
    const uint32_t* amax_b;
    uint32_t* amax_c;
    int amax_c_col0;
    float* wgrad_ws;
    int64_t wgrad_ws_floats;
    float* sw_gu;
    int64_t sw_ld;
    int group_div;
    const float* sw_tbl;
    const gamer_bf16* b_planes_t;
    float* sw_hm;
    const int32_t* sw_row_group;
    const float* norm_x;
    const float* norm_w;
    float norm_eps;
    const int32_t* norm_dst_rows;
    const int32_t* norm_src_rows;
    const int32_t* bias_idx;
    const float* bias_q; const float* bias_k; const float* bias_v;
    int bias_rows, bias_nq, bias_nkv;
} gamer_gemm_desc;

int gamer_gemm_f32(const gamer_gemm_desc* d, void* stream);
int gamer_split2h_transpose_multi(const gamer_bf16* planes, const int64_t* table, int n, gamer_bf16* planes_t, void* stream);

int gamer_gemm_f32_split(const gamer_gemm_desc* d, int terms, void* stream);
int gamer_split3_guard(int on);
int gamer_absmax_f32(const float* x, int batch, int64_t stride, int rows, int cols, int64_t ld, uint32_t* out, void* stream);
int gamer_absmax_multi_f32(const float* base, const int64_t* table, int n, uint32_t* out, void* stream);
int gamer_split2h_planes_multi(const float* base, const int64_t* table, int n, const uint32_t* slots, gamer_bf16* planes,
                               void* stream);
int gamer_amax_sink(uint32_t* out0, uint32_t* out1);
int gamer_amax_sink3(uint32_t* out0, uint32_t* out1, uint32_t* out2);
int gamer_attn_split_amax(const uint32_t* q, const uint32_t* k, const uint32_t* v, const uint32_t* d_o);
int gamer_split3_planes(const float* x, gamer_bf16* planes, int64_t n, int64_t plane_stride, void* stream);

typedef struct {
    const gamer_bf16* A; int64_t lda;
    const gamer_bf16* B; int64_t ldb;
    void* C; int64_t ldc;
    int M, N, K;
    int accumulate;
    int groups;
    int group_mode;
    const int32_t* group_offsets;
    int64_t strideB, strideC;
    int kchunk;
    const float* resid;
    const int32_t* row_map;
    float p_drop;
    uint64_t seed;
    const gamer_bf16* rowdot_other;
    float* rowdot_out;
    int rowdot_S;
    const float* qk_wq; const float* qk_wk; float qk_eps;
    const float* qk_cos; const float* qk_sin;
    const float* qk_bias_q; const float* qk_bias_k; const float* qk_bias_v;
    const int32_t* qk_act_idx; const int32_t* qk_pos_ids;
    gamer_bf16* qk_q_rot; gamer_bf16* qk_k_rot;
    int qk_S, qk_nq, qk_nkv;
    gamer_bf16* sw_gu;
    int64_t sw_ld;
    float* wgrad_ws;
    int64_t wgrad_ws_floats;
} gamer_gemm_bf16_desc;

int gamer_gemm_bf16(const gamer_gemm_bf16_desc* d, void* stream);

int gamer_cast_params_bf16(const float* flat, gamer_bf16* out, gamer_bf16* out_t, const int64_t* table,
                           int n_entries, int n_tiles, void* stream);

int gamer_qknorm_rope_fwd(float* qkv, int T, int S, int nq, int nkv,
                          const float* wq, const float* wk, float eps,
                          const float* cos_t, const float* sin_t,
                          const float* bias_q, const float* bias_k, const float* bias_v,
                          const int32_t* act_idx,
                          float* q_rot, float* k_rot, const int32_t* pos_ids, void* stream);
int gamer_qknorm_rope_bwd(const float* qkv, const float* dq_rot, const float* dk_rot,
                          int T, int S, int nq, int nkv,
                          const float* wq, const float* wk, float eps,
                          const float* cos_t, const float* sin_t,
                          const float* bias_q, const float* bias_k,
                          const int32_t* act_idx, int nb1,
                          float* dqkv, float* dwq, float* dwk,
                          float* dbias_q, float* dbias_k, float* dbias_v, const int32_t* pos_ids,
                          float* partial, int64_t partial_numel, void* stream);
int gamer_qknorm_rope_fwd_bf16(gamer_bf16* qkv, int T, int S, int nq, int nkv,
                               const float* wq, const float* wk, float eps,
                               const float* cos_t, const float* sin_t,
                               const float* bias_q, const float* bias_k, const float* bias_v,
                               const int32_t* act_idx,
                               gamer_bf16* q_rot, gamer_bf16* k_rot, const int32_t* pos_ids, void* stream);
int gamer_qknorm_rope_bwd_bf16(const gamer_bf16* qkv, const gamer_bf16* dq_rot, const gamer_bf16* dk_rot,
                               int T, int S, int nq, int nkv,
                               const float* wq, const float* wk, float eps,
                               const float* cos_t, const float* sin_t,
                               const float* bias_q, const float* bias_k,
                               const int32_t* act_idx, int nb1,
                               gamer_bf16* dqkv, float* dwq, float* dwk,
                               float* dbias_q, float* dbias_k, float* dbias_v, const int32_t* pos_ids,
                               float* partial, int64_t partial_numel, void* stream);

int gamer_attn_row_order(const int32_t* row_empty, int B, int S, int32_t* perm, int32_t* tile_kind,
// ... 304 lines not shown
```

Measured before the change: 5164.

## Fuse cross-attn gated residual into o-proj GEMM epilogue and add token-major cross qknorm bwd

Adds a GEMM epilogue (EPI 5) that computes the gated-SiLU dropout residual directly from the o-projection output tile. This removes the separate silu_gate_fwd pass and its re-read of the projection output, and the engine enables it by default for split3. It also adds a token-major qknorm/rope backward kernel for the cross path, which accumulates per-action bias gradients with permlane swaps and reduces them with a dedicated partial-reduce kernel. The partial scratch for that kernel is carved from the dao workspace. The extra loads raise epilogue register pressure, and the new code paths add complexity and aliasing risk.

```diff
diff --git a/gamer_amd/_lib.py b/gamer_amd/_lib.py
--- a/gamer_amd/_lib.py
+++ b/gamer_amd/_lib.py
@@ -57,6 +57,7 @@
         ("norm_dst_rows", c_void_p), ("norm_src_rows", c_void_p),
         ("bias_idx", c_void_p), ("bias_q", c_void_p), ("bias_k", c_void_p), ("bias_v", c_void_p),
         ("bias_rows", c_int), ("bias_nq", c_int), ("bias_nkv", c_int),
+        ("gate", c_void_p), ("gate_out", c_void_p),
     ]
 
 
diff --git a/gamer_amd/csrc/common.h b/gamer_amd/csrc/common.h
--- a/gamer_amd/csrc/common.h
+++ b/gamer_amd/csrc/common.h
@@ -328,6 +328,12 @@
     return s * (1.f + x * (1.f - s));
 }
 
+__device__ __forceinline__ float gate_resid_f(float a, float g, float r, float m) { return fmaf(m, __fmul_rn(a, silu_f(g)), r); }
+__device__ __forceinline__ float4 gate_resid4(const float4 a, const float4 g, const float4 r, const float (&m)[4]) {
+    return make_float4(gate_resid_f(a.x, g.x, r.x, m[0]), gate_resid_f(a.y, g.y, r.y, m[1]), gate_resid_f(a.z, g.z, r.z, m[2]),
+                       gate_resid_f(a.w, g.w, r.w, m[3]));
+}
+
 struct SwigluRule {
     static constexpr int NIN = 2;
     static __device__ __forceinline__ float fwd(float a, float b, float m) { return m * (silu_f(a) * b); }
diff --git a/gamer_amd/csrc/elementwise.hip b/gamer_amd/csrc/elementwise.hip
--- a/gamer_amd/csrc/elementwise.hip
+++ b/gamer_amd/csrc/elementwise.hip
@@ -542,12 +542,13 @@
     for (int64_t i = (int64_t)blockIdx.x * EW_THREADS + threadIdx.x; i < n4; i += (int64_t)gridDim.x * EW_THREADS) {
         const float4 x = ld4(a + 4 * i), g = ld4(gate + 4 * i);
         float4 o;
-        o.x = x.x * silu_f(g.x); o.y = x.y * silu_f(g.y); o.z = x.z * silu_f(g.z); o.w = x.w * silu_f(g.w);
         if (resid) {
             const float4 r = resid[i];
             float m[4];
             rng.mult4((uint32_t)i, m);
-            o.x = r.x + m[0] * o.x; o.y = r.y + m[1] * o.y; o.z = r.z + m[2] * o.z; o.w = r.w + m[3] * o.w;
+            o = gate_resid4(x, g, r, m);
+        } else {
+            o.x = x.x * silu_f(g.x); o.y = x.y * silu_f(g.y); o.z = x.z * silu_f(g.z); o.w = x.w * silu_f(g.w);
         }
         st4(out + 4 * i, o);
     }
diff --git a/gamer_amd/csrc/gemm.hip b/gamer_amd/csrc/gemm.hip
--- a/gamer_amd/csrc/gemm.hip
+++ b/gamer_amd/csrc/gemm.hip
@@ -1,5 +1,6 @@
 #include "common.h"
 #include <stdlib.h>
+#include <atomic>
 
 namespace gamer {
 
@@ -211,6 +212,8 @@
     float* sw_gu; int64_t sw_ld;
     int group_div;
     const float* sw_tbl;
+    const float* gate;
+    float* gate_out;
 };
 
 constexpr float SPLIT3_GUARD_RATIO = 1.f / 65536.f;
@@ -887,7 +890,7 @@
         }
         __builtin_amdgcn_s_waitcnt(0xc07f);
         const int c4 = (lane & 15) << 2;
-        const DropoutRng rng((EPI == 1 || EPI == 4) ? p.p_drop : 0.f, p.seed);
+        const DropoutRng rng((EPI == 1 || EPI == 4 || EPI == 5) ? p.p_drop : 0.f, p.seed);
         const int row_first = row0 + wm * 64 + (lane >> 4);
         const int col = col0 + wn * 64 + c4;
         float* dst0 = Cp + (int64_t)row_first * p.ldc + col;
@@ -896,7 +899,7 @@
         const bool amax_on = GAMER_GEMM_CAMAX_BUILD && p.amax_c != nullptr && !ACCUM && col0 + wn * 64 >= p.amax_c_col0;
         float cmax = 0.f;
         int pre_rc[EPI == 1 ? 16 : 1];
-        float4 pre_x[EPI == 1 ? 16 : (EPI == 4 ? 8 : 1)], pre_b[EPI == 4 ? 8 : 1];
+        float4 pre_x[EPI == 1 ? 16 : ((EPI == 4 || EPI == 5) ? 8 : 1)], pre_b[(EPI == 4 || EPI == 5) ? 8 : 1];
         if (EPI == 1) {
             if (p.row_map) {
 #pragma unroll
@@ -923,9 +926,19 @@
             }
         };
         if (EPI == 4) pre_sw(0);
+        auto pre_gate = [&](int it0) {
+#pragma unroll
+            for (int it = 0; it < 8; ++it) {
+                const int64_t e = (int64_t)(row_first + 4 * (it0 + it)) * p.ldc + col;
+                pre_x[EPI == 5 ? it : 0] = *reinterpret_cast<const float4*>(p.resid + e);
+                pre_b[EPI == 5 ? it : 0] = *reinterpret_cast<const float4*>(p.gate + e);
+            }
+        };
+        if (EPI == 5) pre_gate(0);
 #pragma unroll
         for (int it = 0; it < 16; ++it) {
             if (EPI == 4 && it == 8) pre_sw(8);
+            if (EPI == 5 && it == 8) pre_gate(8);
             const int lr = (lane >> 4) + 4 * it;
             const float4 v = *reinterpret_cast<const float4*>(patch + lr * 68 + c4);
             if (EPI == 3) {
@@ -993,6 +1006,12 @@
                     asm("v_max3_f32 %0, %0, |%1|, |%2|\n\tv_max3_f32 %0, %0, |%3|, |%4|" : "+v"(cmax) : "v"(dg.x), "v"(dg.y), "v"(dg.z), "v"(dg.w));
                     asm("v_max3_f32 %0, %0, |%1|, |%2|\n\tv_max3_f32 %0, %0, |%3|, |%4|" : "+v"(cmax) : "v"(du.x), "v"(du.y), "v"(du.z), "v"(du.w));
                 }
+            } else if (EPI == 5) {
+                const int64_t e = (int64_t)(row_first + 4 * it) * p.ldc + col;
+                float m[4];
+                rng.mult4((uint32_t)(e >> 2), m);
+                *reinterpret_cast<float4*>(dst0 + it * step) = v;
+                *reinterpret_cast<float4*>(p.gate_out + e) = gate_resid4(v, pre_b[EPI == 5 ? (it & 7) : 0], pre_x[EPI == 5 ? (it & 7) : 0], m);
             } else if (EPI == 1) {
                 const int64_t e = (int64_t)pre_rc[EPI == 1 ? it : 0] * p.ldc + col;
                 float* dst = Cp + e;
@@ -1004,7 +1023,7 @@
                 *reinterpret_cast<float4*>(dst) = o;
             } else {
                 float* dst = dst0 + it * step;
-                if (EPI != 1 && EPI != 3 && amax_on)
+                if (EPI != 1 && EPI != 3 && EPI != 5 && amax_on)
                     asm("v_max3_f32 %0, %0, |%1|, |%2|\n\tv_max3_f32 %0, %0, |%3|, |%4|" : "+v"(cmax) : "v"(v.x), "v"(v.y), "v"(v.z), "v"(v.w));
                 if (EPI == 2) {
                     const float4 o4 = oth[EPI == 2 ? it : 0];
@@ -1025,7 +1044,7 @@
                 }
             }
         }
-        if (EPI != 1 && EPI != 3 && amax_on) {
+        if (EPI != 1 && EPI != 3 && EPI != 5 && amax_on) {
             uint32_t mw = __float_as_uint(cmax);
 #pragma unroll
             for (int o2 = 32; o2 > 0; o2 >>= 1) mw = max(mw, (uint32_t)__shfl_xor((int)mw, o2, 64));
@@ -1069,6 +1088,15 @@
                 if (GAMER_GEMM_CAMAX_BUILD && p.amax_c != nullptr) emax = fmaxf(emax, fmaxf(fabsf(dg), fabsf(du)));
                 return;
             }
+            if (EPI == 5) {
+                const int64_t e = (int64_t)row * p.ldc + col;
+                const DropoutRng rng(p.p_drop, p.seed);
+                float m[4];
+                rng.mult4((uint32_t)(e >> 2), m);
+                Cp[e] = v;
+                p.gate_out[e] = gate_resid_f(v, p.gate[e], p.resid[e], m[e & 3]);
+                return;
+            }
             if (GAMER_GEMM_CAMAX_BUILD && EPI != 1 && MODE == 0 && !ACCUM && p.amax_c != nullptr && col >= p.amax_c_col0) emax = fmaxf(emax, fabsf(v));
             if (EPI == 1) {
                 const int64_t rc = p.row_map ? p.row_map[row] : row;
@@ -1176,6 +1204,9 @@
     if (stamp && SPLIT == 6) return launch_gemm_t<A_KC, B_KC, MODE, false, true, 2, 0, SPLIT>(p, blocks, st, lds);
     if constexpr (SPLIT == 3 && MODE == 0 && A_KC) {
         if (p.sw_gu) return launch_gemm_t<A_KC, B_KC, MODE, false, false, 2, 4, SPLIT>(p, blocks, st, lds);
+    }
+    if constexpr (SPLIT == 3 && MODE == 0 && A_KC && B_KC) {
+        if (p.gate) return launch_gemm_t<A_KC, B_KC, MODE, false, false, 2, 5, SPLIT>(p, blocks, st, lds);
     }
     if (MODE == 0 && p.resid) return launch_gemm_t<A_KC, B_KC, MODE, false, false, 2, 1, SPLIT>(p, blocks, st, lds);
     if (MODE == 0 && p.rowdot_out) return launch_gemm_t<A_KC, B_KC, MODE, false, false, 2, 2, SPLIT>(p, blocks, st, lds);
@@ -1304,6 +1335,7 @@
     static EnvSwitch stamp("GAMER_GEMM_STAMP"), nbuf("GAMER_GEMM_NBUF");
     return stamp.is_set() || nbuf.is_set();
 }
+static std::atomic<long long> g_gate_epi_launches{0};
 static inline bool diag_pp_switch() { static EnvSwitch pp("GAMER_GEMM_PP"); return pp.is_set(); }
 static int gemm_entry(const gamer_gemm_desc* d, void* stream, int split) {
     GAMER_CHECK_ARG(d, "gamer_gemm_f32: null descriptor");
@@ -1344,6 +1376,7 @@
     p.wgrad_ws = nullptr;
     p.sw_gu = d->sw_gu; p.sw_ld = d->sw_ld;
     p.group_div = d->group_div > 1 ? d->group_div : 1; p.sw_tbl = d->sw_tbl;
+    p.gate = d->gate; p.gate_out = d->gate_out;
     GAMER_CHECK_ARG(d->group_div <= 1 || (d->group_mode == 0 && d->group_offsets && d->groups % d->group_div == 0),
                     "gamer_gemm_f32: group_div = %d needs group_mode 0, group_offsets and groups (%d) a multiple of it", d->group_div, d->groups);
     GAMER_CHECK_ARG(!d->sw_tbl || ((d->sw_gu || d->sw_hm) && aligned16(d->sw_tbl)),
@@ -1400,7 +1433,25 @@
                                      aligned16(d->bias_k) && aligned16(d->bias_v)),
                     "gamer_gemm_f32: the bias-row epilogue (bias_idx) needs a plain Linear-forward GEMM with one group, three tables and "
                     "N = bias_nq + 2 bias_nkv in multiples of 4 (N=%d)", d->N);
-    if (split == 3 && gemm_as_eligible(d, a_kc, b_kc, p.b_planes)) return launch_gemm_as(d, p.b_planes, b_kc, (hipStream_t)stream);
+    GAMER_CHECK_ARG(!d->gate || (d->resid && d->gate_out && !d->row_map && d->group_mode == 0 && d->groups == 1 && !d->group_offsets &&
+                                 a_kc && b_kc && !d->accumulate && !d->rowdot_out && !d->qk_q_rot && !d->sw_gu && !d->sw_hm && !d->norm_x &&
+                                 !d->bias_idx && !d->amax_c && d->alpha == 1.f && d->ldc == d->N && d->N % 4 == 0 && aligned16(d->gate) &&
+                                 aligned16(d->gate_out)),
+                    "gamer_gemm_f32: the gated residual epilogue (gate) needs resid and gate_out, a plain ungrouped Linear-forward GEMM without "
+                    "row_map or another epilogue, alpha = 1 and dense rows (ldc = %lld, N = %d)", (long long)d->ldc, d->N);
+    if (d->gate) {
+        static EnvSwitch gate_epi("GAMER_GEMM_GATE_EPI");
+        gamer_gemm_desc d2 = *d;
+        d2.gate = nullptr; d2.gate_out = nullptr; d2.resid = nullptr;
+        const bool fused = split == 3 && gate_epi.get(1) != 0 && d->N % BN == 0 && !diag_build_switches() && !diag_pp_switch() &&
+                           !gemm_as_eligible(&d2, a_kc, b_kc, p.b_planes) && !gemm_os_fwd_eligible(&d2, a_kc, b_kc);
+        if (fused) g_gate_epi_launches.fetch_add(1, std::memory_order_relaxed);
+        else {
+            GAMER_TRY(gemm_entry(&d2, stream, split));
+            return gamer_silu_gate_fwd(d->C, d->gate, (int64_t)d->M * d->N, d->gate_out, d->resid, d->p_drop, d->seed, stream);
+        }
+    }
+    if (split == 3 && !d->gate && gemm_as_eligible(d, a_kc, b_kc, p.b_planes)) return launch_gemm_as(d, p.b_planes, b_kc, (hipStream_t)stream);
     if (d->norm_x || d->bias_idx) {
         gamer_gemm_desc d2 = *d;
         if (d->norm_x) {
@@ -1423,7 +1474,7 @@
                          : gamer_swiglu_fwd_ld(d->C, d->ldc, d->M, d->N / 2, d->p_drop, d->seed, d->sw_hm, stream);
     }
     if (split == 3 && gemm_os_eligible(d, a_kc, b_kc, p.b_planes)) return launch_gemm_os(d, p.b_planes, g_split3_guard, (hipStream_t)stream);
-    if (split == 3 && gemm_os_fwd_eligible(d, a_kc, b_kc))
+    if (split == 3 && !d->gate && gemm_os_fwd_eligible(d, a_kc, b_kc))
         return launch_gemm_os(d, reinterpret_cast<const uint16_t*>(d->b_planes_t), g_split3_guard, (hipStream_t)stream, true);
     p.n_tiles = (d->N + BN - 1) / BN;
     hipStream_t st = (hipStream_t)stream;
@@ -1604,6 +1655,7 @@
 }
 
 extern "C" int gamer_gemm_f32(const gamer_gemm_desc* d, void* stream) { return gemm_entry(d, stream, 0); }
+extern "C" long long gamer_debug_gemm_gate_epi_launches(void) { return g_gate_epi_launches.load(std::memory_order_relaxed); }
 
 extern "C" int gamer_split3_guard(int on) {
     const int prev = g_split3_guard;
diff --git a/gamer_amd/csrc/qknorm_rope.hip b/gamer_amd/csrc/qknorm_rope.hip
--- a/gamer_amd/csrc/qknorm_rope.hip
+++ b/gamer_amd/csrc/qknorm_rope.hip
@@ -432,8 +432,157 @@
     }
 }
 
+__device__ __forceinline__ float group_scatter_sum(float v, int a) {
+    const uint32_t b = __float_as_uint(v);
+    const uint32_t c0 = a == 0 ? b : 0u, c1 = a == 1 ? b : 0u, c2 = a == 2 ? b : 0u, c3 = a == 3 ? b : 0u;
+    const auto s02 = __builtin_amdgcn_permlane32_swap(c0, c2, false, false);
+    const auto s13 = __builtin_amdgcn_permlane32_swap(c1, c3, false, false);
+    const float p = __uint_as_float(s02[0]) + __uint_as_float(s02[1]);
+    const float q = __uint_as_float(s13[0]) + __uint_as_float(s13[1]);
+    const auto r = __builtin_amdgcn_permlane16_swap(__float_as_uint(p), __float_as_uint(q), false, false);
+    return __uint_as_float(r[0]) + __uint_as_float(r[1]);
+}
+
+constexpr int QKX_QK = 9, QKX_V = 3, QKX_NB = 4, QKX_WAVES = 4096;
+__global__ void __launch_bounds__(EW_THREADS)
+qknorm_rope_bwd_tok_cross_kernel(const float* __restrict__ qkv, const float* __restrict__ dq_rot, const float* __restrict__ dk_rot,
+                                 int T, int S, int nq, int nkv, const float* __restrict__ wq, const float* __restrict__ wk, float eps,
+                                 const float* __restrict__ cos_t, const float* __restrict__ sin_t, const int32_t* __restrict__ act_idx,
+                                 int nb1, float* __restrict__ dqkv, float* __restrict__ partial, int n_waves,
+                                 const int32_t* __restrict__ pos_ids, uint32_t* __restrict__ amax_out) {
+    using L = RowLanes<float>;
+    constexpr int E = L::E, ROWS = 64 / L::LANES;
+    const int lane = threadIdx.x & 63;
+    const int g = lane % L::LANES, sub = lane / L::LANES;
+    const int wave = (int)(((int64_t)blockIdx.x * EW_THREADS + threadIdx.x) >> 6);
+    if (wave >= n_waves) return;
+    float am = 0.f;
+    const int nqk = nq + nkv, nall = nqk + nkv;
+    const int ldqkv = nall * 64;
+    float wqv[E], wkv[E], dwq[E], dwk[E], db[QKX_QK + QKX_V][E];
+    ld_f32(wq + E * g, wqv);
+    ld_f32(wk + E * g, wkv);
+#pragma unroll
+    for (int e = 0; e < E; ++e) { dwq[e] = 0.f; dwk[e] = 0.f; }
+#pragma unroll
+    for (int hd = 0; hd < QKX_QK + QKX_V; ++hd)
+#pragma unroll
+        for (int e = 0; e < E; ++e) db[hd][e] = 0.f;
+    const float sgn = g < L::LANES / 2 ? 1.f : -1.f;
+    for (int tb = wave * ROWS; tb < T; tb += n_waves * ROWS) {
+        const int t = tb + sub;
+        const bool live = t < T;
+        const int tc = live ? t : T - 1;
+        const int pos = pos_ids ? pos_ids[tc] : tc % S;
+        const int a_t = live ? act_idx[tc] : -1;
+        float cs[E], sn[E];
+        ld_f32(cos_t + pos * 64 + E * g, cs);
+        ld_f32(sin_t + pos * 64 + E * g, sn);
+        const float* xrow = qkv + (int64_t)tc * ldqkv + E * g;
+        const float* dqrow = dq_rot + (int64_t)tc * nq * 64 + E * g;
+        const float* dkrow = dk_rot + (int64_t)tc * nkv * 64 + E * g;
+        float dv[QKX_V][E];
+#pragma unroll
+        for (int hv = 0; hv < QKX_V; ++hv) L::ld(dqkv + (int64_t)tc * ldqkv + (nqk + min(hv, nkv - 1)) * 64 + E * g, dv[hv]);
+#pragma unroll
+        for (int h0 = 0; h0 < QKX_QK; h0 += 3) {
+            if (h0 >= nqk) break;
+            float xs[3][E], ds[3][E];
+#pragma unroll
+            for (int u = 0; u < 3; ++u) {
+                const int hd = min(h0 + u, nqk - 1);
+                L::ld(xrow + hd * 64, xs[u]);
+                L::ld(hd < nq ? dqrow + hd * 64 : dkrow + (hd - nq) * 64, ds[u]);
+            }
+#pragma unroll
+            for (int u = 0; u < 3; ++u) {
+                const int hd = h0 + u;
+                if (hd >= nqk) break;
+                const bool isq = hd < nq;
+                float dx[E], dwr[E];
+#pragma unroll
+                for (int e = 0; e < E; ++e) dwr[e] = -0.f;
+                bwd_row<float>(xs[u], ds[u], isq ? wqv : wkv, cs, sn, eps, sgn, true, live ? 1.f : 0.f, dx, dwr);
+#pragma unroll
+                for (int e = 0; e < E; ++e) {
+                    if (isq) dwq[e] = dwq[e] + dwr[e];
+                    else dwk[e] = dwk[e] + dwr[e];
+                    db[hd][e] += group_scatter_sum(dx[e], a_t);
+                }
+                if (live) {
+                    L::st(dqkv + (int64_t)t * ldqkv + hd * 64 + E * g, dx);
+                    am = amax_row(am, dx);
+                }
+            }
+        }
+#pragma unroll
+        for (int hv = 0; hv < QKX_V; ++hv) {
+            if (hv >= nkv) break;
+#pragma unroll
+            for (int e = 0; e < E; ++e) db[QKX_QK + hv][e] += group_scatter_sum(dv[hv][e], a_t);
+        }
+    }
+    bwd_amax_commit(am, amax_out, lane, (uint32_t)wave);
+    const int64_t row_len = 128 + (int64_t)nb1 * nall * 64;
+    float* prow = partial + (int64_t)wave * row_len + E * g;
+#pragma unroll
+    for (int e = 0; e < E; ++e) { dwq[e] = rows_sum<L>(dwq[e]); dwk[e] = rows_sum<L>(dwk[e]); }
+    if (sub == 0) {
+        st_f32(prow, dwq);
+        st_f32(prow + 64, dwk);
+    }
+    if (sub < nb1) {
+        float* brow = prow + 128 + (int64_t)sub * nall * 64;
+#pragma unroll
+        for (int hd = 0; hd < QKX_QK; ++hd)
+            if (hd < nqk) st_f32(brow + hd * 64, db[hd]);
+#pragma unroll
+        for (int hv = 0; hv < QKX_V; ++hv)
+            if (hv < nkv) st_f32(brow + (nqk + hv) * 64, db[QKX_QK + hv]);
+    }
+}
+
 constexpr int QKR_CW = 8;
 constexpr int QKR_RG = 1024 / QKR_CW;
+__global__ void __launch_bounds__(1024)
+qknorm_partial_reduce_tok_kernel(const float* __restrict__ partial, int n_rows, int nq, int nkv, int nb1, float* __restrict__ dwq,
+                                 float* __restrict__ dwk, float* __restrict__ dbias_q, float* __restrict__ dbias_k,
+                                 float* __restrict__ dbias_v) {
+    __shared__ float sh[16][QKR_CW];
+    const int cl = threadIdx.x & (QKR_CW - 1), rg = threadIdx.x / QKR_CW;
+    const int nqk = nq + nkv, nall = nqk + nkv;
+    const int64_t row_len = 128 + (int64_t)nb1 * nall * 64;
+    const int col = blockIdx.x * QKR_CW + cl;
+    float* dst;
+    if (col < 64) dst = dwq + col;
+    else if (col < 128) dst = dwk + (col - 64);
+    else {
+        const int b = col - 128;
+        const int a = b / (nall * 64), hd = (b / 64) % nall, c = b % 64;
+        if (hd < nq) dst = dbias_q + (int64_t)a * nq * 64 + hd * 64 + c;
+        else if (hd < nqk) dst = dbias_k + (int64_t)a * nkv * 64 + (hd - nq) * 64 + c;
+        else dst = dbias_v + (int64_t)a * nkv * 64 + (hd - nqk) * 64 + c;
+    }
+    float s0 = 0.f, s1 = 0.f, s2 = 0.f, s3 = 0.f;
+    auto at = [&](int64_t it) { return partial[it * row_len + col]; };
+    int64_t it = rg;
+    for (; it + 3 * QKR_RG < n_rows; it += 4 * QKR_RG) {
+        s0 += at(it); s1 += at(it + QKR_RG); s2 += at(it + 2 * QKR_RG); s3 += at(it + 3 * QKR_RG);
+    }
+    for (; it < n_rows; it += QKR_RG) s0 += at(it);
+    float t = (s0 + s1) + (s2 + s3);
+    t += __shfl_xor(t, 8, 64); t += __shfl_xor(t, 16, 64); t += __shfl_xor(t, 32, 64);
+    const int lane = threadIdx.x & 63, w = threadIdx.x >> 6;
+    if (lane < QKR_CW) sh[w][lane] = t;
+    __syncthreads();
+    if (threadIdx.x < QKR_CW) {
+        float tot = 0.f;
+#pragma unroll
+        for (int gi = 0; gi < 16; ++gi) tot += sh[gi][threadIdx.x];
+        *dst += tot;
+    }
+}
+
 __global__ void __launch_bounds__(1024)
 qknorm_partial_reduce_kernel(const float* __restrict__ partial, int n_rows, int nq, int nkv, int cross, int nb1,
                              float* __restrict__ dwq, float* __restrict__ dwk, float* __restrict__ dbias_q,
@@ -553,6 +702,21 @@
                                                     rcross, rnb1, dwq, dwk, dbias_q, dbias_k, dbias_v);
     };
     uint32_t* amax_out = nullptr;
+    if constexpr (F32) {
+        static EnvSwitch cross_tok("GAMER_QKNORM_CROSS_TOK");
+        const int64_t row_len = 128 + (int64_t)nb1 * (nq + 2 * nkv) * 64;
+        int x_waves = (T + ROWS - 1) / ROWS;
+        if (x_waves > QKX_WAVES) x_waves = QKX_WAVES;
+        if ((int64_t)x_waves * row_len > partial_numel) x_waves = (int)(partial_numel / row_len);
+        if (cross && !qknorm_row_major() && cross_tok.get(1) != 0 && nb1 <= QKX_NB && nq + nkv <= QKX_QK && nkv <= QKX_V && x_waves >= 1) {
+            amax_out = take_amax_sink().out[0];
+            GAMER_TRY(launch<qknorm_rope_bwd_tok_cross_kernel>(name, dim3((x_waves + EW_WAVES - 1) / EW_WAVES), dim3(EW_THREADS), 0, ST(stream),
+                                                               qkv, dq_rot, dk_rot, T, S, nq, nkv, wq, wk, eps, cos_t, sin_t, act_idx, nb1, dqkv,
+                                                               partial, x_waves, pos_ids, amax_out));
+            return launch<qknorm_partial_reduce_tok_kernel>(name, dim3((int)(row_len / QKR_CW)), dim3(1024), 0, ST(stream), (const float*)partial,
+                                                            x_waves, nq, nkv, nb1, dwq, dwk, dbias_q, dbias_k, dbias_v);
+        }
+    }
     if (!cross && !qknorm_row_major() && n_waves >= 1) {
         if constexpr (F32) amax_out = take_amax_sink().out[0];
         GAMER_TRY(launch<qknorm_rope_bwd_tok_kernel<TA>>(name, dim3((n_waves + EW_WAVES - 1) / EW_WAVES), dim3(EW_THREADS), 0, ST(stream), qkv,
diff --git a/gamer_amd/engine.py b/gamer_amd/engine.py
--- a/gamer_amd/engine.py
+++ b/gamer_amd/engine.py
@@ -621,12 +621,17 @@
                     attention(A["q_c"], k_x, qkv_x[:, NQ + NKV:], r["kl_cross"], r["ql_cross"], r["empty_cross"],
                               r["tile_empty_cross"], self._seed(l, 2), A["ao_c"], A["lse_c"], ws.cross_order, span_cross)
                 if x_cross_last is None:
-                    ops.linear_fwd(A["ao_c"], NQ, Cm["o"], NQ, A["op_c"], H, T, H, NQ)
                     ops.linear_fwd(A["h2"], H, Cm["gate"], H, A["gate_c"], H, T, H, H)
+                    if c.fuse_gate:
+                        ops.linear_fwd(A["ao_c"], NQ, Cm["o"], NQ, A["op_c"], H, T, H, NQ, resid=xs[1], p_drop=p_res,
+                                       seed=self._seed(l, 3), gate=A["gate_c"], gate_out=xs[2])
+                    else:
+                        ops.linear_fwd(A["ao_c"], NQ, Cm["o"], NQ, A["op_c"], H, T, H, NQ)
                 if h2_hold is not None:
                     h2_hold.__exit__(None, None, None)
                 if x_cross_last is None:
-                    ops.silu_gate_fwd(A["op_c"], A["gate_c"], xs[2], resid=xs[1], p=p_res, seed=self._seed(l, 3))
+                    if not c.fuse_gate:
+                        ops.silu_gate_fwd(A["op_c"], A["gate_c"], xs[2], resid=xs[1], p=p_res, seed=self._seed(l, 3))
                     xcur = xs[2]
             din = W.din
             if last_row_logits and l == cfg.num_hidden_layers - 1:
@@ -789,6 +794,7 @@
         c.fuse_swiglu_bwd = (c.bf16 or self.matmul == "split3") and self.fuse_swiglu_bwd
         c.fuse_norm = not c.bf16 and self.matmul == "split3" and os.environ.get("GAMER_GEMM_AS_NORM", "1") != "0"
         c.fuse_bias = not c.bf16 and self.matmul == "split3" and os.environ.get("GAMER_GEMM_AS_BIAS", "1") != "0"
+        c.fuse_gate = not c.bf16 and self.matmul == "split3" and os.environ.get("GAMER_GEMM_GATE_EPI", "1") != "0"
         return c
 
     def _prologue(self, input_ids, attention_mask, labels, train, dropout, dropout_rate, kv_dest, hidden_sink,
@@ -1012,10 +1018,13 @@
                 attention_bwd(A["q_c"], A["k_c"], A["qkv_c"][:, NQ + NKV:], A["ao_c"], A["lse_c"], r["kl_cross"],
                               r["ql_cross"], r["empty_cross"], r["tile_empty_cross"], self._seed(l, 2), ws.cross_order,
                               span_cross)
+                qk_need = ops.qknorm_partial_numel(NB1, nq + 2 * nkv)
+                qk_scratch = (ws.dao.view(-1)[:qk_need] if (not bf16 and ws.dao.numel() > ws.qk_partial.numel())
+                              else ws.qk_partial)
                 ops.qknorm_rope_bwd(A["qkv_c"], ws.dq, ws.dk, S, nq, nkv, C["qn"], C["kn"], eps, cos, sin, ws.dqkv,
                                     GC["qn"], GC["kn"], bias_q=C["bq"], bias_k=C["bk"], act_idx=r["act_idx"], nb1=NB1,
                                     dbias_q=GC["bq"], dbias_k=GC["bk"], dbias_v=GC["bv"], pos_ids=pos_ids,
-                                    partial=ws.qk_partial)
+                                    partial=qk_scratch)
                 with hold(ws.dqkv):
                     ops.linear_wgrad(ws.dqkv, QKV, A["h2"], H, GC["qkv"], H, T, QKV, H)
                     dgrad(ws.dqkv, QKV, C["qkv"], CT["qkv"], H, t3, H, QKV, H)
diff --git a/gamer_amd/ops.py b/gamer_amd/ops.py
--- a/gamer_amd/ops.py
+++ b/gamer_amd/ops.py
@@ -584,10 +584,12 @@
 
 def gemm(A, a_rs, a_ks, Bm, b_rs, b_ks, Cm, ldc, M, N, K, alpha=1.0, accumulate=False, groups=1, group_mode=0,
          group_offsets=None, strideB=0, strideC=0, kchunk=0, resid=None, row_map=None, p_drop=0.0, seed=0,
-         rowdot=None, qknorm=None, c_amax=None, swiglu_bwd=None, group_div=0, sw_tbl=None, swiglu_fwd=None, norm=None, bias=None):
+         rowdot=None, qknorm=None, c_amax=None, swiglu_bwd=None, group_div=0, sw_tbl=None, swiglu_fwd=None, norm=None, bias=None,
+         gate=None, gate_out=None):
     if A.dtype == torch.bfloat16:
-        if group_div > 1 or sw_tbl is not None or swiglu_fwd is not None or norm is not None or bias is not None:
-            raise RuntimeError("group_div / sw_tbl / swiglu_fwd / norm / bias are options of the fp32 GEMM")
+        if (group_div > 1 or sw_tbl is not None or swiglu_fwd is not None or norm is not None or bias is not None
+                or gate is not None):
+            raise RuntimeError("group_div / sw_tbl / swiglu_fwd / norm / bias / gate are options of the fp32 GEMM")
         return _gemm_bf16(A, a_rs, a_ks, Bm, b_rs, b_ks, Cm, ldc, M, N, K, alpha, accumulate, groups, group_mode,
                           group_offsets, strideB, strideC, kchunk, resid, row_map, p_drop, seed, rowdot, qknorm, swiglu_bwd)
     d = GemmDesc()
@@ -606,6 +608,10 @@
     d.row_map = ptr(row_map)
     d.p_drop = p_drop
     d.seed = seed
+    if gate is not None:
+        if resid is None or gate_out is None:
+            raise RuntimeError("gemm(gate=...): the gated residual epilogue takes resid and gate_out as well")
+        d.gate, d.gate_out = ptr(gate), ptr(gate_out)
     if rowdot is not None:
         d.rowdot_other, d.rowdot_out, d.rowdot_S = ptr(rowdot[0]), ptr(rowdot[1]), int(rowdot[2])
     if qknorm is not None:
@@ -887,8 +893,8 @@
          ptr(bias_q), ptr(bias_k), ptr(bias_v), ptr(act_idx), ptr(q_rot), ptr(k_rot), ptr(pos_ids), stream_ptr())
 
 
-def qknorm_partial_numel(nb1: int = 0) -> int:
-    return 8192 * (1 + nb1) * 64
+def qknorm_partial_numel(nb1: int = 0, heads: int = 0) -> int:
+    return max(8192 * (1 + nb1) * 64, 4096 * (128 + nb1 * heads * 64) if (nb1 and heads) else 0)
 
 
 def qknorm_rope_bwd(qkv, dq_rot, dk_rot, S, nq, nkv, wq, wk, eps, cos_t, sin_t, dqkv, dwq, dwk, bias_q=None,
diff --git a/include/gamer_hip.h b/include/gamer_hip.h
--- a/include/gamer_hip.h
+++ b/include/gamer_hip.h
@@ -151,6 +151,8 @@
     const int32_t* bias_idx;
     const float* bias_q; const float* bias_k; const float* bias_v;
     int bias_rows, bias_nq, bias_nkv;
+    const float* gate;
+    float* gate_out;
 } gamer_gemm_desc;
 
 int gamer_gemm_f32(const gamer_gemm_desc* d, void* stream);
```

Result: no change. 5193, median of 6 (+0.6%).
